# etzinis/sudo_rm_rf

Measured on AMD Instinct MI355X. Metric: separated-seconds/sec (4s@8kHz mixtures), Improved-U16/512, 1->8 MI355X, higher is better.
Workload: dtype f32 (1x1 convs: fp32 operands split into bf16 hi+lo, 3 bf16 MFMAs per product, fp32 accumulate)

## Files before the change

include/sudormrf_hip.h:

```cpp
#ifndef SUDORMRF_HIP_H
#define SUDORMRF_HIP_H

#include <stddef.h>

#ifdef __cplusplus
extern "C" {
#endif

#define SRF_ABI_VERSION 18

#define SRF_STAT_BUCKETS 64

#define SRF_OK 0
#define SRF_EINVAL (-1)
#define SRF_EHIP (-2)
#define SRF_EWORKSPACE (-3)

#define SRF_VARIANT_IMPROVED 0
#define SRF_VARIANT_GROUPCOMM 1
#define SRF_VARIANT_CAUSAL 2

typedef struct srf_config {
  int variant;
  int in_audio_channels;
  int out_channels;
  int in_channels;
  int num_blocks;
  int upsampling_depth;
  int enc_kernel_size;
  int enc_num_basis;
  int num_sources;
  int group_size;
} srf_config;

typedef struct srf_norm {
  const double* sums;
  const float* gamma;
  const float* beta;
  const float* prelu;
} srf_norm;

typedef struct srf_plan srf_plan;

int srf_abi_version(void);
const char* srf_last_error(void);

void srf_set_kernel_mode(int mode);
int srf_get_kernel_mode(void);
int srf_profile_begin(void* stream);
int srf_profile_end(void* stream, int* count);
int srf_profile_get(int i, const char** name, float* ms);
int srf_profile_timeline(int i, const char** name, float* t_ms, int* stream_index);

#ifdef SRF_DIAGNOSTICS
enum srf_debug_flag {
  SRF_DBG_NO_PAIRS = 1,
  SRF_DBG_GEMM_NO_MGROUPS = 2,
  SRF_DBG_NO_GEMM_256 = 4,
  SRF_DBG_NO_PACKED_WEIGHTS = 8,
  SRF_DBG_PYR_PER_LEVEL = 16,
  SRF_DBG_PYR_NO_LDS_TILES = 32,
  SRF_DBG_PYR_NO_REG = 64,
  SRF_DBG_PYR_PASS1_NONPERSISTENT = 128,
  SRF_DBG_GEMM_WHOLE_TAIL_TILES = 256,
  SRF_DBG_GEMM_QUARTER_TILES_LAST = 512,
  SRF_DBG_TAC_ONE_STEP_PER_LANE = 1024,
  SRF_DBG_GEMM_128_ONE_TILE_PER_BLOCK = 2048,
  SRF_DBG_WGRAD_NO_XCD_MAP = 4096,
  SRF_DBG_GEMM_256_SWAP_FORMS = 8192,
  SRF_DBG_TRAIN_BF16X3 = 16384,
  SRF_DBG_NO_FUSED_TAIL = 32768,
  SRF_DBG_BWD_NO_FUSED_HEAD = 1 << 16,
  SRF_DBG_PYR_PASS1_ROWS_PER_WAVE = 1 << 17,
  SRF_DBG_WGRAD_NO_WIDE_TILE = 1 << 18,
  SRF_DBG_WGRAD_128_MASKED = 1 << 19,
  SRF_DBG_WGRAD_SHORT_CHUNKS = 1 << 20,
  SRF_DBG_PAIR_PERSISTENT = 1 << 21,
  SRF_DBG_TAC_VALU = 1 << 22,
  SRF_DBG_PAIR_FULL_DRAIN = 1 << 23,
  SRF_DBG_TAC_GENERIC = 1 << 24,
  SRF_DBG_WGRAD_ONE_CHAIN_FOLD = 1 << 25,
  SRF_DBG_TAC_LANES_4TILES = 1 << 26,
  SRF_DBG_GEMM_128_POINTER_LOADS = 1 << 27,
  SRF_DBG_TRAIN_FWD_SPLIT_BF16 = 1 << 28,
  SRF_DBG_BWD_DW_CHUNKED = 1 << 29,
  SRF_DBG_BWD_GLN_SCALAR = 1 << 30,
  SRF_DBG_TRAIN_FWD_EXACT_MFMA = -2147483647 - 1
};
void srf_set_debug_flags(int flags);
#endif

int srf_plan_create(const srf_config* cfg, int batch, int T, srf_plan** out);
void srf_plan_destroy(srf_plan* plan);
size_t srf_plan_workspace_bytes(const srf_plan* plan);
int srf_plan_num_params(const srf_plan* plan);
int srf_plan_frames(const srf_plan* plan);
int srf_plan_padded_length(const srf_plan* plan);
int srf_plan_num_launches(const srf_plan* plan);

int srf_forward(const srf_plan* plan, const float* const* params, int num_params,
                const float* wav, float* out, void* workspace, size_t workspace_bytes, void* stream);

int srf_separate(const srf_plan* plan, const float* const* params, int num_params, const float* wav, float* out,
                 float* stats, int mixture_consistency, void* workspace, size_t workspace_bytes, void* stream);

int srf_plan_set_block_scales(srf_plan* plan, const float* alpha, const float* beta, int n);

int srf_debug_fetch(const srf_plan* plan, const void* workspace, int what, float* dst, size_t dst_floats,
                    void* stream);



int srf_encoder(const float* wav, const float* w, float* out, double* sums,
                int Bt, int A, int T, int N, int K, int L, void* stream);

int srf_gln_stats(const float* x, double* sums, int groups, long per_group, void* stream);
int srf_gln_apply(const float* x, float* y, const srf_norm* norm, int groups, int channels, int length,
                  void* stream);
int srf_gln_apply_add(const float* x, const float* q, float* y, const srf_norm* norm, int groups,
                      int channels, int length, void* stream);

int srf_pw_conv(const float* x, const float* w, const float* bias, float* y,
                int Bt, int Cin, int Cout, int L, const srf_norm* in_norm, const float* residual,
                double* out_sums, int epilogue_mask, const float* mul, int mul_channels, void* stream);

size_t srf_packed_pw_weight_bytes(int Cout, int Cin);
int srf_pack_pw_weights(const float* const* w, void* const* packed, const int* Cout, const int* Cin, int n,
                        void* stream);
int srf_pw_conv_packed(const float* x, const float* w, const void* w_packed, const float* bias, float* y,
                       int Bt, int Cin, int Cout, int L, const srf_norm* in_norm, const float* residual,
                       double* out_sums, int epilogue_mask, const float* mul, int mul_channels, void* stream);

int srf_pw_conv_pair_supported(int Bt, int Cin1, int Cmid, int Cout2, int L);
int srf_pw_conv_pair(const float* x, const void* w1_packed, const float* bias1, float* y, const srf_norm* in_norm,
                     const float* residual, const void* w2_packed, const float* bias2, float* y2, double* out_sums2,
                     int Bt, int Cin1, int Cmid, int Cout2, int L, void* stream);

size_t srf_packed3_pw_weight_bytes(int Cout, int Cin);
int srf_pack3_pw_weights(const float* const* w, void* const* packed, const int* Cout, const int* Cin, int n, void* stream);
void srf_pack3_forget(const void* packed);
int srf_pw_conv_packed3(const float* x, const float* w, const void* w_packed3, const float* bias, float* y, int Bt, int Cin,
                        int Cout, int L, const srf_norm* in_norm, const float* residual, double* out_sums, void* stream);
int srf_pw_conv_pair_packed3_supported(int Bt, int Cin1, int Cmid, int Cout2, int L);
int srf_pw_conv_pair_packed3(const float* x, const void* w1_packed3, const float* bias1, float* y, const srf_norm* in_norm,
                             const float* residual, const void* w2_packed3, const float* bias2, float* y2, double* out_sums2,
                             int Bt, int Cin1, int Cmid, int Cout2, int L, void* stream);

int srf_dwconv5(const float* x, const float* w, const float* bias, float* y,
                int Bt, int C, int Lin, int stride, const srf_norm* in_norm, double* out_sums,
                void* stream);

int srf_conv1d(const float* x, const float* w, const float* bias, float* y, int Bt, int Cin, int Cout, int Lin, int K,
               int stride, int padding, int dilation, int groups, double* out_sums, void* stream);

int srf_merge(const float* const* levels, const srf_norm* norms, int D, float* y,
              int Bt, int C, int L, double* out_sums, void* stream);

int srf_pyramid_supported(int C, int L, int D);
size_t srf_pyramid_scratch_bytes(int groups, int C, int L, int D);
int srf_pyramid(const float* y1, float* merged, const srf_norm* in_norm, const float* const* w,
                const float* const* bias, const float* const* gamma, const float* const* beta, int groups,
                int C, int L, int D, void* scratch, double* out_sums, void* stream);

int srf_causal_encoder(const float* wav, const float* w, float* out, int Bt, int A, int T, int N, int K, int L, void* stream);
int srf_causal_dwconv(const float* x, const float* w, const float* bias, const float* in_prelu, const float* out_prelu,
                      float* y, int Bt, int C, int Lin, int stride, void* stream);
int srf_causal_merge(const float* const* levels, int D, float* y, int Bt, int C, int L, void* stream);
int srf_causal_pyramid_supported(int C, int L, int D);
int srf_causal_pyramid(const float* y1, float* merged, const float* in_prelu, const float* const* w,
                       const float* const* bias, const float* const* prelu, int Bt, int C, int L, int D, void* stream);
int srf_causal_scale(const float* src, float* dst, long n, const float* dscale, float hscale, void* stream);
int srf_prelu_apply(const float* x, const float* slope, float* y, long n, void* stream);

typedef struct srf_stream srf_stream;
int srf_stream_create(const srf_config* cfg, int batch, int max_chunk_samples, srf_stream** out);
void srf_stream_destroy(srf_stream* s);
int srf_stream_granule(const srf_stream* s);
int srf_stream_delay(const srf_stream* s);
size_t srf_stream_state_bytes(const srf_stream* s);
size_t srf_stream_weights_bytes(const srf_stream* s);
size_t srf_stream_workspace_bytes(const srf_stream* s);
int srf_stream_num_launches(const srf_stream* s);
int srf_stream_set_block_scales(srf_stream* s, const float* alpha, const float* beta, int n);
int srf_stream_prepare(const srf_stream* s, const float* const* params, int num_params, void* weights_buf, void* stream);
int srf_stream_reset(const srf_stream* s, void* state, int row, void* stream);
int srf_stream_push(const srf_stream* s, const void* weights_buf, void* state, const float* wav, int n, float* out,
                    void* workspace, size_t workspace_bytes, void* stream);
int srf_stream_flush(const srf_stream* s, const void* state, float* out_tail, void* stream);
int srf_causal_stream_pyramid(const float* y1, float* merged, float* const* state, const float* in_prelu,
                              const float* const* w, const float* const* bias, const float* const* prelu, int Bt, int C, int Lc,
                              int D, void* stream);

size_t srf_decoder_scratch_floats(int Bt, int Ci, int Co, int K, int L);
int srf_decoder(const float* v, const float* w, float* out, int Bt, int Ci, int Co, int K, int L, int T,
                float* scratch, void* stream);

int srf_tac(const float* x, float* q, const float* const* params, int Bt, int G, int n, int H, int L,
            double* out_sums, void* stream);

int srf_mixture_consistency(const float* pr, const float* mix, float* out, int Bt, int S, int T,
                            void* stream);

int srf_mixture_consistency_magsq(const float* pr, const float* mix, float* out, int Bt, int S, int T, float* work,
                                  void* stream);

int srf_wav_normalize(const float* wav, float* out, float* stats, int rows, int T, void* stream);
int srf_wav_stats(const float* wav, float* stats, int rows, int T, void* stream);
int srf_wav_denormalize(const float* est, const float* stats, const float* mix_norm, float* out, int Bt, int S,
                        int T, void* stream);

size_t srf_pit_sisdr_work_bytes(int Bt, int S);
int srf_pit_sisdr_forward(const float* est, const float* tgt, int Bt, int S, int T, float clamp, void* work,
                          float* pw, float* loss, void* stream);
int srf_pit_sdr_forward(const float* est, const float* tgt, int Bt, int S, int T, float clamp, int sdr_type,
                        int zero_mean, int take_log, void* work, float* pw, float* loss, void* stream);
int srf_pit_sisdr_match(const void* work, int Bt, int S, int* match_out, void* stream);
int srf_pit_sisdr_backward(const float* est, const float* tgt, int Bt, int S, int T, float clamp, const void* work,
                           const float* loss, const float* upstream, float* grad_est, void* stream);

size_t srf_perm_inv_sisdr_work_bytes(int Bt, int S);
int srf_perm_inv_sisdr(const float* pr, const float* tgt, const float* mix, int Bt, int S, int T, int zero_mean,
                       double eps, void* work, float* best, int* best_perm, float* base, void* stream);

size_t srf_zeroref_snr_work_bytes(int Bt, int S, int T);
int srf_zeroref_snr_forward(const float* est, const float* tgt, int Bt, int S, int T, int zero_mean, float threshold_db,
                            float thresh, float eps, void* work, float* values, int* best_perm, float* loss, void* stream);
int srf_zeroref_snr_backward(const float* est, const float* tgt, int Bt, int S, int T, const void* work,
                             const float* upstream, int upstream_per_example, float* grad_est, void* stream);
size_t srf_stab_sisdr_work_bytes(int Bt, int T);
int srf_stab_sisdr(const float* pr, const float* tgt, int Bt, int pr_rows, int n_est, int n_act, int T, int zero_mean,
                   int improvement, double eps, void* work, float* values, int* best_perm, void* stream);
size_t srf_fuss_augment_scratch_bytes(int B, int T);
int srf_fuss_augment(const float* clean, const int* src_b, const int* src_s, const float* gain, int B, int S, int T, float eps,
                     float* out, float* mix, float* stats, void* scratch, void* stream);


size_t srf_pw_wgrad_scratch_bytes(int Bt, int Cout, int Cin, int L);
int srf_pw_wgrad(const float* g, const float* x, const srf_norm* in_norm, int Bt, int Cin, int Cout, int L, float* dw,
                 float* dbias, int accumulate, void* scratch, void* stream);
int srf_pw_wgrad_cols(const float* g, const float* x, const srf_norm* in_norm, int Bt, int Cin, int Cout, int L,
                      float* dw, int dw_cols, float* dbias, int accumulate, void* scratch, void* stream);
int srf_pw_wgrad_ld(const float* g, const float* x, const srf_norm* in_norm, int Bt, int Cin, int Cout, int L,
                    float* dw, int dw_cols, int dw_ld, float* dbias, int accumulate, void* scratch, void* stream);

size_t srf_tac_bwd_scratch_bytes(int Bt, int G, int n, int L);
int srf_tac_bwd(const float* x, const float* go, const float* const* params, float* const* grads, int Bt, int G, int n,
                int H, int L, float* gx, void* scratch, void* stream);

size_t srf_gln_bwd_scratch_bytes(int groups, int C);
int srf_gln_bwd(const float* gout, const float* gout2, const float* x, const srf_norm* norm, int groups, int C, int L,
                float* gx, int accumulate_gx, float* dgamma, float* dbeta, float* dslope, void* scratch, void* stream);

int srf_merge_bwd(const float* g_merged, float* const* g_levels, int D, long rows, int L, void* stream);

size_t srf_dwconv5_bwd_scratch_bytes(int groups, int C);
int srf_dwconv5_bwd(const float* gd, const float* xin, const srf_norm* in_norm, const float* w, int groups, int C,
                    int Lin, int stride, float* gin, float* dw, float* dbias, void* scratch, void* stream);

int srf_mask_apply(const float* m, const float* enc, float* v, int Bt, int SA, int N, int L, void* stream);
int srf_mask_bwd(const float* gv, const float* m, const float* enc, float* gm, float* genc, int accumulate_genc, int Bt,
                 int SA, int N, int L, void* stream);

int srf_prelu_bwd(const float* gout, const float* x, const float* slope, float* gx, float* dslope, long n, void* stream);

int srf_frames_gather(const float* src, float* out, int Bt, int R, int T, int K, int hop, int pad, int L, int rows_out,
                      void* stream);

size_t srf_train_saved_bytes(const srf_plan* plan);
size_t srf_train_scratch_bytes(const srf_plan* plan);
int srf_forward_train(const srf_plan* plan, const float* const* params, int num_params, const float* wav, float* out,
                      void* saved, size_t saved_bytes, void* scratch, size_t scratch_bytes, void* stream);
int srf_backward(const srf_plan* plan, const float* const* params, float* const* grads, int num_params,
                 const float* wav, const float* grad_out, const void* saved, size_t saved_bytes, void* scratch,
                 size_t scratch_bytes, void* stream);
int srf_backward_wav(const srf_plan* plan, const float* const* params, float* const* grads, int num_params,
                     const float* wav, const float* grad_out, const void* saved, size_t saved_bytes, void* scratch,
                     size_t scratch_bytes, float* grad_wav, void* stream);

size_t srf_online_remix_scratch_bytes(int B, int S);
int srf_online_remix(const float* clean, const int* src_b, const int* src_s, int B, int S, int T, float eps, float* mix,
                     float* out, void* scratch, void* stream);

int srf_opt_chunk_size(void);
int srf_clip_adam_step(const void* tensors, const void* chunks, int n_chunks, double* buckets, float max_norm, float lr,
                       float beta1, float beta2, float eps, int step, float* norm_out, void* stream);

typedef struct srf_feeder srf_feeder;
int srf_wav_info(const char* path, int* rate, int* channels, int* bits, long* frames);
int srf_wav_read(const char* path, long start, long n, float* dst, long* frames);
int srf_feeder_create(const char* const* paths, int n_items, int n_streams, int time_samples, int batch, int n_threads,
                      int augment, int shuffle, int drop_last, unsigned long long seed, srf_feeder** out);
int srf_feeder_create_sharded(const char* const* paths, int n_items, int n_streams, int time_samples, int batch,
                              int n_threads, int augment, int shuffle, int drop_last, unsigned long long seed, int normalize,
                              int rank, int world, srf_feeder** out);
void srf_feeder_destroy(srf_feeder* f);
long srf_feeder_epoch_items(srf_feeder* f, int* items, long capacity);
int srf_feeder_read_example(const char* const* paths, int n_streams, int time_samples, long start, int augment, int normalize,
                            float* wave, int* len, float* stat);
long srf_feeder_batches_per_epoch(const srf_feeder* f);
long srf_feeder_item_frames(const srf_feeder* f, int item);
int srf_feeder_start_epoch(srf_feeder* f, int epoch);
int srf_feeder_submit(srf_feeder* f, float* wave, int* len, float* stat);
int srf_feeder_wait(srf_feeder* f, float** wave, int** len, float** stat, int* n_valid);
int srf_feeder_normalize(const float* raw, const int* len, const float* stat, int B, int n_streams, int T, int normalize,
                         float eps, float* mix, float* src, void* stream);

#ifdef __cplusplus
}
#endif
#endif
```

sudo_rm_rf_amd/_lib.py:

```python
import ctypes as C
import os
import threading

import torch

_PKG = os.path.dirname(os.path.abspath(__file__))
LIB_PATH = os.environ.get("SRF_LIB") or os.path.join(_PKG, "libsudormrf_hip.so")
ABI_VERSION = 18
STAT_BUCKETS = 64

SRF_OK = 0
VARIANT_IMPROVED, VARIANT_GROUPCOMM, VARIANT_CAUSAL = 0, 1, 2


class SrfError(RuntimeError):
    pass


class srf_config(C.Structure):
    _fields_ = [(n, C.c_int) for n in (
        "variant", "in_audio_channels", "out_channels", "in_channels", "num_blocks",
        "upsampling_depth", "enc_kernel_size", "enc_num_basis", "num_sources", "group_size")]


class srf_norm(C.Structure):
    _fields_ = [("sums", C.c_void_p), ("gamma", C.c_void_p), ("beta", C.c_void_p), ("prelu", C.c_void_p)]


_vp, _i, _sz, _l = C.c_void_p, C.c_int, C.c_size_t, C.c_long
_PROTOS = {
    "srf_abi_version": (_i, []),
    "srf_last_error": (C.c_char_p, []),
    "srf_set_kernel_mode": (None, [_i]),
    "srf_get_kernel_mode": (_i, []),
    "srf_profile_begin": (_i, [_vp]),
    "srf_profile_end": (_i, [_vp, C.POINTER(_i)]),
    "srf_profile_get": (_i, [_i, C.POINTER(C.c_char_p), C.POINTER(C.c_float)]),
    "srf_profile_timeline": (_i, [_i, C.POINTER(C.c_char_p), C.POINTER(C.c_float), C.POINTER(_i)]),
    "srf_plan_create": (_i, [C.POINTER(srf_config), _i, _i, C.POINTER(_vp)]),
    "srf_plan_destroy": (None, [_vp]),
    "srf_plan_workspace_bytes": (_sz, [_vp]),
    "srf_plan_num_params": (_i, [_vp]),
    "srf_plan_frames": (_i, [_vp]),
    "srf_plan_padded_length": (_i, [_vp]),
    "srf_plan_num_launches": (_i, [_vp]),
    "srf_forward": (_i, [_vp, C.POINTER(_vp), _i, _vp, _vp, _vp, _sz, _vp]),
    "srf_debug_fetch": (_i, [_vp, _vp, _i, _vp, _sz, _vp]),
    "srf_encoder": (_i, [_vp, _vp, _vp, _vp, _i, _i, _i, _i, _i, _i, _vp]),
    "srf_gln_stats": (_i, [_vp, _vp, _i, _l, _vp]),
    "srf_gln_apply": (_i, [_vp, _vp, C.POINTER(srf_norm), _i, _i, _i, _vp]),
    "srf_gln_apply_add": (_i, [_vp, _vp, _vp, C.POINTER(srf_norm), _i, _i, _i, _vp]),
    "srf_pw_conv": (_i, [_vp, _vp, _vp, _vp, _i, _i, _i, _i, C.POINTER(srf_norm), _vp, _vp, _i, _vp, _i, _vp]),
    "srf_set_debug_flags": (None, [_i]),
    "srf_packed_pw_weight_bytes": (_sz, [_i, _i]),
    "srf_pack_pw_weights": (_i, [C.POINTER(_vp), C.POINTER(_vp), C.POINTER(_i), C.POINTER(_i), _i, _vp]),
    "srf_pw_conv_packed": (_i, [_vp, _vp, _vp, _vp, _vp, _i, _i, _i, _i, C.POINTER(srf_norm), _vp, _vp, _i, _vp, _i, _vp]),
    "srf_pw_conv_pair_supported": (_i, [_i, _i, _i, _i, _i]),
    "srf_pw_conv_pair": (_i, [_vp, _vp, _vp, _vp, C.POINTER(srf_norm), _vp, _vp, _vp, _vp, _vp, _i, _i, _i, _i, _i, _vp]),
    "srf_pw_conv_pair_packed3_supported": (_i, [_i, _i, _i, _i, _i]),
    "srf_pw_conv_pair_packed3": (_i, [_vp, _vp, _vp, _vp, C.POINTER(srf_norm), _vp, _vp, _vp, _vp, _vp, _i, _i, _i, _i, _i, _vp]),
    "srf_packed3_pw_weight_bytes": (_sz, [_i, _i]),
    "srf_pack3_pw_weights": (_i, [C.POINTER(_vp), C.POINTER(_vp), C.POINTER(_i), C.POINTER(_i), _i, _vp]),
    "srf_pack3_forget": (None, [_vp]),
    "srf_pw_conv_packed3": (_i, [_vp, _vp, _vp, _vp, _vp, _i, _i, _i, _i, C.POINTER(srf_norm), _vp, _vp, _vp]),
    "srf_pit_sisdr_work_bytes": (_sz, [_i, _i]),
    "srf_perm_inv_sisdr_work_bytes": (_sz, [_i, _i]),
    "srf_perm_inv_sisdr": (_i, [_vp, _vp, _vp, _i, _i, _i, _i, C.c_double, _vp, _vp, _vp, _vp, _vp]),
    "srf_pit_sisdr_forward": (_i, [_vp, _vp, _i, _i, _i, C.c_float, _vp, _vp, _vp, _vp]),
    "srf_pit_sdr_forward": (_i, [_vp, _vp, _i, _i, _i, C.c_float, _i, _i, _i, _vp, _vp, _vp, _vp]),
    "srf_pit_sisdr_match": (_i, [_vp, _i, _i, _vp, _vp]),
    "srf_pit_sisdr_backward": (_i, [_vp, _vp, _i, _i, _i, C.c_float, _vp, _vp, _vp, _vp, _vp]),
    "srf_zeroref_snr_work_bytes": (_sz, [_i, _i, _i]),
    "srf_zeroref_snr_forward": (_i, [_vp, _vp, _i, _i, _i, _i, C.c_float, C.c_float, C.c_float, _vp, _vp, _vp, _vp, _vp]),
    "srf_zeroref_snr_backward": (_i, [_vp, _vp, _i, _i, _i, _vp, _vp, _i, _vp, _vp]),
    "srf_stab_sisdr_work_bytes": (_sz, [_i, _i]),
    "srf_stab_sisdr": (_i, [_vp, _vp, _i, _i, _i, _i, _i, _i, _i, C.c_double, _vp, _vp, _vp, _vp]),
    "srf_fuss_augment_scratch_bytes": (_sz, [_i, _i]),
    "srf_fuss_augment": (_i, [_vp, _vp, _vp, _vp, _i, _i, _i, C.c_float, _vp, _vp, _vp, _vp, _vp]),
    "srf_pw_wgrad_scratch_bytes": (_sz, [_i, _i, _i, _i]),
    "srf_pw_wgrad_cols": (_i, [_vp, _vp, C.POINTER(srf_norm), _i, _i, _i, _i, _vp, _i, _vp, _i, _vp, _vp]),
    "srf_pw_wgrad_ld": (_i, [_vp, _vp, C.POINTER(srf_norm), _i, _i, _i, _i, _vp, _i, _i, _vp, _i, _vp, _vp]),
    "srf_pw_wgrad": (_i, [_vp, _vp, C.POINTER(srf_norm), _i, _i, _i, _i, _vp, _vp, _i, _vp, _vp]),
    "srf_gln_bwd_scratch_bytes": (_sz, [_i, _i]),
    "srf_gln_bwd": (_i, [_vp, _vp, _vp, C.POINTER(srf_norm), _i, _i, _i, _vp, _i, _vp, _vp, _vp, _vp, _vp]),
    "srf_merge_bwd": (_i, [_vp, C.POINTER(_vp), _i, C.c_long, _i, _vp]),
    "srf_dwconv5_bwd_scratch_bytes": (_sz, [_i, _i]),
    "srf_dwconv5_bwd": (_i, [_vp, _vp, C.POINTER(srf_norm), _vp, _i, _i, _i, _i, _vp, _vp, _vp, _vp, _vp]),
    "srf_mask_apply": (_i, [_vp, _vp, _vp, _i, _i, _i, _i, _vp]),
    "srf_mask_bwd": (_i, [_vp, _vp, _vp, _vp, _vp, _i, _i, _i, _i, _i, _vp]),
    "srf_prelu_bwd": (_i, [_vp, _vp, _vp, _vp, _vp, C.c_long, _vp]),
    "srf_frames_gather": (_i, [_vp, _vp, _i, _i, _i, _i, _i, _i, _i, _i, _vp]),
    "srf_train_saved_bytes": (_sz, [_vp]),
    "srf_train_scratch_bytes": (_sz, [_vp]),
    "srf_forward_train": (_i, [_vp, C.POINTER(_vp), _i, _vp, _vp, _vp, _sz, _vp, _sz, _vp]),
    "srf_backward": (_i, [_vp, C.POINTER(_vp), C.POINTER(_vp), _i, _vp, _vp, _vp, _sz, _vp, _sz, _vp]),
    "srf_backward_wav": (_i, [_vp, C.POINTER(_vp), C.POINTER(_vp), _i, _vp, _vp, _vp, _sz, _vp, _sz, _vp, _vp]),
    "srf_tac_bwd_scratch_bytes": (_sz, [_i, _i, _i, _i]),
    "srf_tac_bwd": (_i, [_vp, _vp, C.POINTER(_vp), C.POINTER(_vp), _i, _i, _i, _i, _i, _vp, _vp, _vp]),
    "srf_online_remix_scratch_bytes": (_sz, [_i, _i]),
    "srf_online_remix": (_i, [_vp, _vp, _vp, _i, _i, _i, C.c_float, _vp, _vp, _vp, _vp]),
    "srf_opt_chunk_size": (_i, []),
    "srf_clip_adam_step": (_i, [_vp, _vp, _i, _vp, C.c_float, C.c_float, C.c_float, C.c_float, C.c_float, _i, _vp, _vp]),
    "srf_wav_normalize": (_i, [_vp, _vp, _vp, _i, _i, _vp]),
    "srf_wav_stats": (_i, [_vp, _vp, _i, _i, _vp]),
    "srf_separate": (_i, [_vp, C.POINTER(_vp), _i, _vp, _vp, _vp, _i, _vp, _sz, _vp]),
    "srf_wav_denormalize": (_i, [_vp, _vp, _vp, _vp, _i, _i, _i, _vp]),
    "srf_dwconv5": (_i, [_vp, _vp, _vp, _vp, _i, _i, _i, _i, C.POINTER(srf_norm), _vp, _vp]),
    "srf_conv1d": (_i, [_vp, _vp, _vp, _vp, _i, _i, _i, _i, _i, _i, _i, _i, _i, _vp, _vp]),
    "srf_pyramid_supported": (_i, [_i, _i, _i]),
    "srf_pyramid_scratch_bytes": (_sz, [_i, _i, _i, _i]),
    "srf_pyramid": (_i, [_vp, _vp, C.POINTER(srf_norm), C.POINTER(_vp), C.POINTER(_vp), C.POINTER(_vp),
                        C.POINTER(_vp), _i, _i, _i, _i, _vp, _vp, _vp]),
    "srf_merge": (_i, [C.POINTER(_vp), C.POINTER(srf_norm), _i, _vp, _i, _i, _i, _vp, _vp]),
    "srf_decoder_scratch_floats": (_sz, [_i, _i, _i, _i, _i]),
    "srf_decoder": (_i, [_vp, _vp, _vp, _i, _i, _i, _i, _i, _i, _vp, _vp]),
    "srf_tac": (_i, [_vp, _vp, C.POINTER(_vp), _i, _i, _i, _i, _i, _vp, _vp]),
    "srf_mixture_consistency": (_i, [_vp, _vp, _vp, _i, _i, _i, _vp]),
    "srf_mixture_consistency_magsq": (_i, [_vp, _vp, _vp, _i, _i, _i, _vp, _vp]),
    "srf_wav_info": (_i, [C.c_char_p, C.POINTER(_i), C.POINTER(_i), C.POINTER(_i), C.POINTER(_l)]),
    "srf_wav_read": (_i, [C.c_char_p, _l, _l, _vp, C.POINTER(_l)]),
    "srf_feeder_create": (_i, [C.POINTER(C.c_char_p), _i, _i, _i, _i, _i, _i, _i, _i, C.c_ulonglong, C.POINTER(_vp)]),
    "srf_feeder_create_sharded": (_i, [C.POINTER(C.c_char_p), _i, _i, _i, _i, _i, _i, _i, _i, C.c_ulonglong, _i, _i, _i,
                                       C.POINTER(_vp)]),
    "srf_feeder_destroy": (None, [_vp]),
    "srf_feeder_epoch_items": (_l, [_vp, _vp, _l]),
    "srf_feeder_read_example": (_i, [C.POINTER(C.c_char_p), _i, _i, _l, _i, _i, _vp, _vp, _vp]),
    "srf_feeder_batches_per_epoch": (_l, [_vp]),
    "srf_feeder_item_frames": (_l, [_vp, _i]),
    "srf_feeder_start_epoch": (_i, [_vp, _i]),
    "srf_feeder_submit": (_i, [_vp, _vp, _vp, _vp]),
    "srf_feeder_wait": (_i, [_vp, C.POINTER(_vp), C.POINTER(_vp), C.POINTER(_vp), C.POINTER(_i)]),
    "srf_feeder_normalize": (_i, [_vp, _vp, _vp, _i, _i, _i, _i, C.c_float, _vp, _vp, _vp]),
    "srf_plan_set_block_scales": (_i, [_vp, C.POINTER(C.c_float), C.POINTER(C.c_float), _i]),
    "srf_causal_encoder": (_i, [_vp, _vp, _vp, _i, _i, _i, _i, _i, _i, _vp]),
    "srf_causal_dwconv": (_i, [_vp, _vp, _vp, _vp, _vp, _vp, _i, _i, _i, _i, _vp]),
    "srf_causal_merge": (_i, [C.POINTER(_vp), _i, _vp, _i, _i, _i, _vp]),
    "srf_causal_pyramid_supported": (_i, [_i, _i, _i]),
    "srf_causal_pyramid": (_i, [_vp, _vp, _vp, C.POINTER(_vp), C.POINTER(_vp), C.POINTER(_vp), _i, _i, _i, _i, _vp]),
    "srf_causal_scale": (_i, [_vp, _vp, _l, _vp, C.c_float, _vp]),
    "srf_prelu_apply": (_i, [_vp, _vp, _vp, _l, _vp]),
    "srf_stream_create": (_i, [C.POINTER(srf_config), _i, _i, C.POINTER(_vp)]),
    "srf_stream_destroy": (None, [_vp]),
    "srf_stream_granule": (_i, [_vp]),
    "srf_stream_delay": (_i, [_vp]),
    "srf_stream_state_bytes": (_sz, [_vp]),
    "srf_stream_weights_bytes": (_sz, [_vp]),
    "srf_stream_workspace_bytes": (_sz, [_vp]),
    "srf_stream_num_launches": (_i, [_vp]),
    "srf_stream_set_block_scales": (_i, [_vp, C.POINTER(C.c_float), C.POINTER(C.c_float), _i]),
    "srf_stream_prepare": (_i, [_vp, C.POINTER(_vp), _i, _vp, _vp]),
    "srf_stream_reset": (_i, [_vp, _vp, _i, _vp]),
    "srf_stream_push": (_i, [_vp, _vp, _vp, _vp, _i, _vp, _vp, _sz, _vp]),
    "srf_stream_flush": (_i, [_vp, _vp, _vp, _vp]),
    "srf_causal_stream_pyramid": (_i, [_vp, _vp, C.POINTER(_vp), _vp, C.POINTER(_vp), C.POINTER(_vp), C.POINTER(_vp), _i, _i, _i,
                                       _i, _vp]),
}
EXPORTED_SYMBOLS = tuple(_PROTOS)

_lib = None
_lock = threading.Lock()


def load():
    global _lib
    if _lib is not None:
        return _lib
    with _lock:
        if _lib is not None:
            return _lib
        if not os.path.exists(LIB_PATH):
            raise SrfError(
                "libsudormrf_hip.so not found at %s -- build it with `python -m sudo_rm_rf_amd.build` "
                "(or __graft_entry__.build()).  There is no CPU / PyTorch fallback." % LIB_PATH)
        lib = C.CDLL(LIB_PATH)
        for name, (res, args) in _PROTOS.items():
            try:
                fn = getattr(lib, name)
            except AttributeError as e:
                raise SrfError("libsudormrf_hip.so lacks symbol %s (stale build?)" % name) from e
            fn.restype = res
            fn.argtypes = args
        if lib.srf_abi_version() != ABI_VERSION:
            raise SrfError("libsudormrf_hip.so ABI version %d != expected %d" %
                           (lib.srf_abi_version(), ABI_VERSION))
        _lib = lib
    return _lib


def check(rc, what="libsudormrf_hip"):
    if rc != SRF_OK:
        msg = load().srf_last_error()
        raise SrfError("%s failed (%d): %s" % (what, rc, msg.decode() if msg else "?"))


def ptr(t):
    return None if t is None else C.c_void_p(t.data_ptr())


def current_stream(device):
    return C.c_void_p(torch.cuda.current_stream(device).cuda_stream)


def make_norm(sums=None, gamma=None, beta=None, prelu=None):
    n = srf_norm()
    n.sums = sums.data_ptr() if sums is not None else None
    n.gamma = gamma.data_ptr() if gamma is not None else None
    n.beta = beta.data_ptr() if beta is not None else None
    n.prelu = prelu.data_ptr() if prelu is not None else None
    return n
```

sudo_rm_rf_amd/build.py:

```python
import hashlib
import os
import re
import shutil
import subprocess
import sys
from concurrent.futures import ThreadPoolExecutor

PKG = os.path.dirname(os.path.abspath(__file__))
CSRC = os.path.join(PKG, "csrc")
OBJ = os.path.join(CSRC, "build")
LIB = os.path.join(PKG, "libsudormrf_hip.so")
SOURCES = ["srf_api.hip", "srf_encoder.hip", "srf_elementwise.hip", "srf_dwconv.hip", "srf_pyramid.hip", "srf_pyramid_reg.hip", "srf_pwconv.hip", "srf_pwconv_bf16x3.hip", "srf_pwconv_x3w.hip", "srf_pwconv_x3p.hip", "srf_pwconv_x3f.hip", "srf_pwconv_w4.hip", "srf_pwconv_small.hip",
           "srf_tac.hip", "srf_loss.hip", "srf_pwconv_wgrad.hip", "srf_backward.hip", "srf_train.hip", "srf_augment.hip", "srf_optim.hip", "srf_feeder.hip",
           "srf_causal.hip", "srf_causal_stream.hip", "srf_loss_fuss.hip"]
HEADERS = [os.path.join(CSRC, "srf_common.h"), os.path.join(CSRC, "srf_internal.h"), os.path.join(CSRC, "srf_pw.h"), os.path.join(CSRC, "srf_plan.h"), os.path.join(CSRC, "srf_pyr.h"),
           os.path.join(os.path.dirname(PKG), "include", "sudormrf_hip.h")]
FLAGS = ["-O3", "-std=c++17", "--offload-arch=gfx950", "-fPIC", "-munsafe-fp-atomics",
         "-Wall", "-Wno-unused-function"]
FILE_FLAGS = {
    "srf_pwconv_bf16x3.hip": ["-fno-slp-vectorize"],
    "srf_pwconv_x3w.hip": ["-fno-slp-vectorize"],
    "srf_pwconv_x3p.hip": ["-fno-slp-vectorize"],
    "srf_pwconv_x3f.hip": ["-fno-slp-vectorize"],
    "srf_pwconv_w4.hip": ["-fno-slp-vectorize"],
    "srf_pwconv_wgrad.hip": ["-fno-slp-vectorize"],
    "srf_pwconv.hip": ["-fno-slp-vectorize"],
    "srf_pyramid_reg.hip": ["-fno-slp-vectorize"],
}

_HAZARD = re.compile(r"^\s*(v_pk_\w+)\s.*op_sel:\[[01],1[,\]]", re.M)


def isa_lint(asm_path):
    hits = []
    with open(asm_path, errors="replace") as f:
        for i, line in enumerate(f, 1):
            if _HAZARD.match(line):
                hits.append((i, line.strip()))
    return hits


def hipcc():
    for c in (os.environ.get("HIPCC"), shutil.which("hipcc"), "/opt/rocm/bin/hipcc"):
        if c and os.path.exists(c):
            return c
    raise RuntimeError("hipcc not found (set HIPCC=...)")


def _digest(paths, extra=""):
    h = hashlib.sha1(extra.encode())
    for p in paths:
        with open(p, "rb") as f:
            h.update(f.read())
    return h.hexdigest()


def _compile(cc, src, extra_flags):
    path = os.path.join(CSRC, src)
    obj = os.path.join(OBJ, os.path.basename(src).replace(".hip", ".o"))
    stamp = obj + ".sha1"
    flags = FLAGS + FILE_FLAGS.get(src, []) + extra_flags
    dig = _digest([path, os.path.abspath(__file__)] + HEADERS, " ".join(flags))
    if os.path.exists(obj) and os.path.exists(stamp) and open(stamp).read() == dig:
        return obj, False
    cmd = [cc] + flags + ["-save-temps=obj", "-c", path, "-o", obj]
    r = subprocess.run(cmd, capture_output=True, text=True)
    if r.returncode != 0:
        raise RuntimeError("hipcc failed: %s\n%s\n%s" % (" ".join(cmd), r.stdout, r.stderr))
    warn = "\n".join(l for l in r.stderr.splitlines() if "argument unused during compilation" not in l)
    if warn.strip():
        sys.stderr.write(warn + "\n")
    base = os.path.basename(src).replace(".hip", "")
    asm = os.path.join(OBJ, base + "-hip-amdgcn-amd-amdhsa-gfx950.s")
    if not os.path.exists(asm):
        raise RuntimeError("ISA lint: device assembly %s was not produced" % asm)
    hits = isa_lint(asm)
    for f in os.listdir(OBJ):
        if f.startswith(base + "-h") or f.startswith(base + ".hip-"):
            os.remove(os.path.join(OBJ, f))
    if hits:
        os.remove(obj)
        raise RuntimeError(
            "ISA lint: %s contains %d packed-fp32 instruction(s) with op_sel = 1 on src1 (wrong low result in lanes 48..63 "
            "next to another wavefront's bf16 MFMA on gfx950, see build.py); first: line %d: %s"
            % (src, len(hits), hits[0][0], hits[0][1]))
    with open(stamp, "w") as f:
        f.write(dig)
    return obj, True


def build(force=False, verbose=True, extra_flags=()):
    cc = hipcc()
    os.makedirs(OBJ, exist_ok=True)
    extra_flags = list(extra_flags)
    if force:
        for f in os.listdir(OBJ):
            os.remove(os.path.join(OBJ, f))
    sources = SOURCES
    with ThreadPoolExecutor(max_workers=min(len(sources), os.cpu_count() or 4)) as ex:
        res = list(ex.map(lambda s: _compile(cc, s, extra_flags), sources))
    objs = [o for o, _ in res]
    changed = any(c for _, c in res)
    if changed or not os.path.exists(LIB):
        cmd = [cc, "-shared", "-fPIC", "--offload-arch=gfx950", "-o", LIB] + objs
        r = subprocess.run(cmd, capture_output=True, text=True)
        if r.returncode != 0:
            raise RuntimeError("link failed: %s\n%s\n%s" % (" ".join(cmd), r.stdout, r.stderr))
        if verbose:
            print("built", LIB)
    elif verbose:
        print("up to date:", LIB)
    return LIB


if __name__ == "__main__":
    build(force="--force" in sys.argv)
```

sudo_rm_rf_amd/csrc/srf_api.hip:

```cpp
#include <string.h>

#include <atomic>
#include <mutex>
#include <new>
#include <vector>

#include "srf_plan.h"

static thread_local char g_err[512] = "";
static std::atomic<int> g_kernel_mode{0};

void srf_set_error(const char* fmt, ...) {
  va_list ap;
  va_start(ap, fmt);
  vsnprintf(g_err, sizeof(g_err), fmt, ap);
  va_end(ap);
}
static thread_local int g_kernel_mode_override = -1;
int srf_kernel_mode() { return g_kernel_mode_override >= 0 ? g_kernel_mode_override : g_kernel_mode.load(std::memory_order_relaxed); }
int srf_kernel_mode_override(int mode) {
  const int prev = g_kernel_mode_override;
  g_kernel_mode_override = mode;
  return prev;
}
static std::atomic<int> g_debug_flags{0};
int srf_debug_flags() { return g_debug_flags.load(std::memory_order_relaxed); }
extern "C" void srf_set_debug_flags(int f) { g_debug_flags.store(f, std::memory_order_relaxed); }

static std::mutex g_dev_mu;
static int g_dev_cus[SRF_MAX_DEVICES];
static long g_dev_occ[SRF_MAX_DEVICES][SRF_OCC_SLOTS];
static bool g_dev_occ_set[SRF_MAX_DEVICES][SRF_OCC_SLOTS];

int srf_current_device() {
  int dev = 0;
  return hipGetDevice(&dev) == hipSuccess ? dev : -1;
}
int srf_device_cus() {
  const int dev = srf_current_device();
  if (dev < 0 || dev >= SRF_MAX_DEVICES) return 256;
  std::lock_guard<std::mutex> lk(g_dev_mu);
  if (!g_dev_cus[dev]) {
    hipDeviceProp_t prop;
    g_dev_cus[dev] = hipGetDeviceProperties(&prop, dev) == hipSuccess ? prop.multiProcessorCount : 256;
  }
  return g_dev_cus[dev];
}
long srf_device_cached(int slot, long (*compute)(void*), void* arg) {
  const int dev = srf_current_device();
  if (dev < 0 || dev >= SRF_MAX_DEVICES || slot < 0 || slot >= SRF_OCC_SLOTS) return compute(arg);
  {
    std::lock_guard<std::mutex> lk(g_dev_mu);
    if (g_dev_occ_set[dev][slot]) return g_dev_occ[dev][slot];
  }
  const long v = compute(arg);
  std::lock_guard<std::mutex> lk(g_dev_mu);
  g_dev_occ[dev][slot] = v;
  g_dev_occ_set[dev][slot] = true;
  return v;
}

struct ProfMark {
  const char* name;
  hipEvent_t ev;
  hipStream_t st;
};
static bool g_prof = false;
static std::vector<ProfMark> g_marks;
static std::vector<hipEvent_t> g_pool;
static std::vector<float> g_ms;

static thread_local int g_prof_hold = 0;
bool srf_profiling() { return g_prof && g_prof_hold == 0; }
void srf_prof_hold(int delta) { g_prof_hold += delta; }
void srf_prof_mark(const char* name, hipStream_t st) {
  hipEvent_t ev;
  if (!g_pool.empty()) {
    ev = g_pool.back();
    g_pool.pop_back();
  } else if (hipEventCreate(&ev) != hipSuccess) {
    return;
  }
  (void)hipEventRecord(ev, st);
  g_marks.push_back(ProfMark{name, ev, st});
}

extern "C" int srf_profile_begin(void* stream) {
  for (auto& m : g_marks) g_pool.push_back(m.ev);
  g_marks.clear();
  g_ms.clear();
  g_prof = true;
  srf_prof_mark("begin", (hipStream_t)stream);
  return SRF_OK;
}

extern "C" int srf_profile_end(void* stream, int* count) {
  g_prof = false;
  SRF_CHECK_HIP(hipStreamSynchronize((hipStream_t)stream));
  g_ms.assign(g_marks.size(), 0.f);
  for (size_t i = 1; i < g_marks.size(); ++i) {
    float ms = 0.f;
    SRF_CHECK_HIP(hipEventElapsedTime(&ms, g_marks[i - 1].ev, g_marks[i].ev));
    g_ms[i] = ms;
  }
  if (count) *count = g_marks.empty() ? 0 : (int)g_marks.size() - 1;
  return SRF_OK;
}

extern "C" int srf_profile_timeline(int i, const char** name, float* t_ms, int* stream_index) {
  SRF_CHECK_ARG(i >= 0 && (size_t)(i + 1) < g_marks.size() && name && t_ms && stream_index, "srf_profile_timeline: bad index %d", i);
  float ms = 0.f;
  SRF_CHECK_HIP(hipEventElapsedTime(&ms, g_marks[0].ev, g_marks[i + 1].ev));
  int idx = 0;
  std::vector<hipStream_t> seen;
  for (size_t j = 1; j <= (size_t)(i + 1); ++j) {
    bool known = false;
    for (size_t k = 0; k < seen.size(); ++k)
      if (seen[k] == g_marks[j].st) {
        known = true;
        if (j == (size_t)(i + 1)) idx = (int)k;
      }
    if (!known) {
      if (j == (size_t)(i + 1)) idx = (int)seen.size();
      seen.push_back(g_marks[j].st);
    }
  }
  *name = g_marks[i + 1].name;
  *t_ms = ms;
  *stream_index = idx;
  return SRF_OK;
}

extern "C" int srf_profile_get(int i, const char** name, float* ms) {
  SRF_CHECK_ARG(i >= 0 && (size_t)(i + 1) < g_marks.size() && name && ms, "srf_profile_get: bad index %d", i);
  *name = g_marks[i + 1].name;
  *ms = g_ms[i + 1];
  return SRF_OK;
}

extern "C" const char* srf_last_error(void) { return g_err; }
extern "C" int srf_abi_version(void) { return SRF_ABI_VERSION; }
extern "C" void srf_set_kernel_mode(int mode) { g_kernel_mode.store((mode == 1 || mode == 2) ? mode : 0, std::memory_order_relaxed); }
extern "C" int srf_get_kernel_mode(void) { return g_kernel_mode.load(std::memory_order_relaxed); }

__global__ __launch_bounds__(256) void srf_zero_kernel(uint4* __restrict__ p, size_t n16) {
  for (size_t i = (size_t)blockIdx.x * 256 + threadIdx.x; i < n16; i += (size_t)gridDim.x * 256) p[i] = make_uint4(0, 0, 0, 0);
}
static int srf_zero_launch(void* p, size_t bytes, hipStream_t st) {
  SRF_CHECK_ARG(srf_aligned16(p) && bytes % 16 == 0, "internal: zero fill needs 16-byte granules");
  const size_t n16 = bytes / 16;
  if (!n16) return SRF_OK;
  const size_t blocks = (n16 + 255) / 256;
  hipLaunchKernelGGL(srf_zero_kernel, dim3((unsigned)(blocks < 2048 ? blocks : 2048)), dim3(256), 0, st, (uint4*)p, n16);
  SRF_CHECK_LAUNCH("zero_fill", st);
  return SRF_OK;
}

extern "C" size_t srf_decoder_scratch_floats(int Bt, int Ci, int Co, int K, int L) {
  const size_t M = (size_t)Co * K;
  return srf_align_up(M * Ci, 64) + srf_align_up(M, 64) + srf_align_up((size_t)Bt * M * L, 64);
}

static int srf_decoder_impl(const float* v, const float* w, float* out, int Bt, int Ci, int Co, int K, int L, int T,
                            float* scratch, const float* post_stats, const float* post_wav, int post_mc, void* stream,
                            const float* in_prelu = nullptr);
extern "C" int srf_decoder(const float* v, const float* w, float* out, int Bt, int Ci, int Co, int K,
                           int L, int T, float* scratch, void* stream) {
  return srf_decoder_impl(v, w, out, Bt, Ci, Co, K, L, T, scratch, nullptr, nullptr, 0, stream);
}
static int srf_decoder_impl(const float* v, const float* w, float* out, int Bt, int Ci, int Co, int K, int L, int T,
                            float* scratch, const float* post_stats, const float* post_wav, int post_mc, void* stream,
                            const float* in_prelu) {
  SRF_CHECK_ARG(v && w && out && scratch, "srf_decoder: null pointer");
  SRF_CHECK_ARG(Bt > 0 && Ci > 0 && Co > 0 && L > 0 && T > 0, "srf_decoder: bad sizes");
  SRF_CHECK_ARG(K >= 3 && (K & 1), "srf_decoder: kernel size must be odd (got %d)", K);
  SRF_CHECK_ARG(T <= (K / 2) * L, "srf_decoder: T=%d exceeds hop*L=%d", T, (K / 2) * L);
  SRF_CHECK_ARG(Co <= 65535 && Bt <= 65535, "srf_decoder: too many channels / batch");
  SRF_CHECK_ALIGNED16("srf_decoder", {"scratch", scratch});
  hipStream_t st = (hipStream_t)stream;
  const int M = Co * K;
  float* wt = scratch;
  float* zb = wt + srf_align_up((size_t)M * Ci, 64);
  float* z = zb + srf_align_up((size_t)M, 64);
  int rc = srf_transpose_launch(w, wt, Ci, M, st);
  if (rc) return rc;
  rc = srf_zero_launch(zb, sizeof(float) * srf_align_up((size_t)M, 64), st);
  if (rc) return rc;
  const srf_norm act{nullptr, nullptr, nullptr, in_prelu};
  rc = srf_pw_conv(v, wt, zb, z, Bt, Ci, M, L, in_prelu ? &act : nullptr, nullptr, nullptr, 0, nullptr, 0, stream);
  if (rc) return rc;
  return srf_overlap_add_launch(z, out, Bt, Co, K, L, T, 1, post_stats, post_wav, post_mc, st);
}

static long plan_padded_length(int T, int h, int D) {
  const long nls = (long)h << D;
  return (T < nls) ? nls : ((T / nls) + (T % nls ? 1 : 0)) * nls;
}
static void plan_add_pack(srf_plan* p, size_t* off, int param, int cout, int cin) {
  const size_t bytes = srf_packed_pw_weight_bytes(cout, cin);
  if (!bytes) return;
  const size_t o = *off;
  *off = srf_align_up(*off + bytes, 256);
  p->pk_param.push_back(param);
  p->pk_cout.push_back(cout);
  p->pk_cin.push_back(cin);
  p->pk_off.push_back(o);
  p->pk_of_param[param] = o;
}

static int plan_fail(srf_plan* p, int rc) {
  delete p;
  return rc;
}

static int causal_plan_create(const srf_config* c, int batch, int T, srf_plan** out);
extern "C" int srf_plan_create(const srf_config* c, int batch, int T, srf_plan** out) {
  SRF_CHECK_ARG(c && out, "srf_plan_create: null pointer");
  *out = nullptr;
  SRF_CHECK_ARG(c->variant == SRF_VARIANT_IMPROVED || c->variant == SRF_VARIANT_GROUPCOMM || c->variant == SRF_VARIANT_CAUSAL,
                "srf_plan_create: unknown variant %d", c->variant);
  if (c->variant == SRF_VARIANT_CAUSAL) return causal_plan_create(c, batch, T, out);
  SRF_CHECK_ARG(batch > 0 && T > 0, "srf_plan_create: batch and T must be positive");
  SRF_CHECK_ARG(c->out_channels > 0 && c->in_channels > 0 && c->num_blocks > 0 && c->enc_num_basis > 0 &&
                    c->num_sources > 0,
                "srf_plan_create: non-positive model dimension");
  SRF_CHECK_ARG(c->upsampling_depth >= 1 && c->upsampling_depth <= SRF_MAX_DEPTH,
                "srf_plan_create: upsampling_depth %d unsupported (1..%d)", c->upsampling_depth,
                SRF_MAX_DEPTH);
  SRF_CHECK_ARG(c->enc_kernel_size >= 3 && (c->enc_kernel_size & 1),
                "srf_plan_create: enc_kernel_size must be odd (the reference's mask multiply breaks "
                "for even sizes)");
  srf_plan* p = new (std::nothrow) srf_plan();
  SRF_CHECK_ARG(p != nullptr, "srf_plan_create: out of host memory");
  p->cfg = *c;
  const bool gc = c->variant == SRF_VARIANT_GROUPCOMM;
  const int G = gc ? c->group_size : 1;
  p->A = gc ? c->in_audio_channels : 1;
  if (G <= 0 || p->A <= 0) {
    srf_set_error("srf_plan_create: group_size / in_audio_channels must be positive");
    return plan_fail(p, SRF_EINVAL);
  }
  if (gc && (c->out_channels % G || c->in_channels % G)) {
    srf_set_error("srf_plan_create: channels (%d,%d) not divisible by group_size %d", c->out_channels,
                  c->in_channels, G);
    return plan_fail(p, SRF_EINVAL);
  }
  if (gc) {
    const int n = c->out_channels / G;
    if (!(n == 2 || n == 4 || n == 8 || n == 16 || n == 32)) {
      srf_set_error("srf_plan_create: out_channels/group_size = %d unsupported (2,4,8,16,32)", n);
      return plan_fail(p, SRF_EINVAL);
    }
  }
  const int D = c->upsampling_depth, U = c->num_blocks, K = c->enc_kernel_size;
  const int h = K / 2;
  const long Tp = plan_padded_length(T, h, D);
  p->Bt = batch;
  p->T = T;
  p->Tp = (int)Tp;
  p->L = (int)((Tp + 2 * h - K) / h + 1);
  p->SA = c->num_sources * p->A;
  p->Bg = batch * G;
  p->nB = c->out_channels / G;
  p->nC = c->in_channels / G;
  if (p->L % (1 << (D - 1)) != 0) {
    srf_set_error("srf_plan_create: internal: L=%d not divisible by 2^(D-1)", p->L);
    return plan_fail(p, SRF_EINVAL);
  }
  if ((long)p->Bg > 65535) {
    srf_set_error("srf_plan_create: batch*group_size=%d too large (max 65535 per call)", p->Bg);
    return plan_fail(p, SRF_EINVAL);
  }
  const int ublock_params = 10 + 4 * D;
  p->p_block0 = 5;
  p->p_ublock_off = gc ? 11 : 0;
  p->p_block_stride = ublock_params + p->p_ublock_off;
  p->p_tail = 5 + U * p->p_block_stride;
  p->n_params = p->p_tail + 4;
  p->slots_per_block = D + 2 + (gc ? 1 : 0);
  p->n_slots = 1 + U * p->slots_per_block;
  const size_t F = sizeof(float);
  const size_t L = p->L;
  size_t off = 0;
  auto take = [&](size_t bytes) {
    const size_t o = off;
    off = srf_align_up(off + bytes, 256);
    return o;
  };
  p->stats_bytes = (size_t)p->n_slots * p->Bg * SRF_STAT_BUCKETS * 2 * sizeof(double);
  p->off_stats = take(p->stats_bytes);
  p->off_enc = take(F * batch * c->enc_num_basis * L);
  p->off_xa = take(F * batch * c->out_channels * L);
  p->off_xb = take(F * batch * c->out_channels * L);
  p->off_xq = gc ? take(F * batch * c->out_channels * L) : 0;
  p->off_xu = gc ? take(F * batch * c->out_channels * L) : 0;
  p->off_y1 = take(F * batch * c->in_channels * L);
  for (int k = 0; k < D; ++k) p->off_lv[k] = take(F * batch * c->in_channels * (L >> k));
  p->off_masked = take(F * batch * p->SA * c->enc_num_basis * L);
  p->off_dec = take(F * srf_decoder_scratch_floats(batch, p->SA * c->enc_num_basis, p->SA, K, p->L));
  p->fused_pyramid = srf_pyramid_supported(p->nC, p->L, D);
  p->off_pyr = p->fused_pyramid ? take(srf_pyramid_scratch_bytes(p->Bg, p->nC, p->L, D)) : 0;
  p->pk_of_param.assign(p->n_params, 0);
  plan_add_pack(p, &off, 3, c->out_channels, c->enc_num_basis);
  for (int i = 0; i < U; ++i) {
    const int pu = p->p_block0 + i * p->p_block_stride + p->p_ublock_off;
    plan_add_pack(p, &off, pu + 0, p->nC, p->nB);
    plan_add_pack(p, &off, pu + 5 + 4 * D + 3, p->nB, p->nC);
  }
  plan_add_pack(p, &off, p->p_tail + 1, p->SA * c->enc_num_basis, c->out_channels);
  p->off_wdpack = (p->SA * K <= 64 && p->pk_of_param[p->p_tail + 1]) ? take(srf_mask_decode_pack_bytes(p->SA * c->enc_num_basis)) : 0;
  p->total_bytes = off;
  p->n_launches = 1  + 2 + U * (D + 3 + (gc ? 2 : 0)) + 1 + 4;
  *out = p;
  return SRF_OK;
}

static int causal_plan_create(const srf_config* c, int batch, int T, srf_plan** out) {
  SRF_CHECK_ARG(batch > 0 && T > 0, "srf_plan_create: batch and T must be positive");
  SRF_CHECK_ARG(c->in_audio_channels > 0 && c->out_channels > 0 && c->in_channels > 0 && c->num_blocks > 0 &&
                    c->enc_num_basis > 0 && c->num_sources > 0,
                "srf_plan_create: non-positive model dimension (causal variant)");
  SRF_CHECK_ARG(c->group_size == 1, "srf_plan_create: the causal variant has no groups (group_size must be 1, got %d)",
                c->group_size);
  SRF_CHECK_ARG(c->upsampling_depth >= 1 && c->upsampling_depth <= SRF_MAX_DEPTH,
                "srf_plan_create: upsampling_depth %d unsupported (1..%d)", c->upsampling_depth, SRF_MAX_DEPTH);
  SRF_CHECK_ARG(c->enc_kernel_size >= 3 && (c->enc_kernel_size & 1),
                "srf_plan_create: enc_kernel_size must be odd for the causal variant (got %d)", c->enc_kernel_size);
  srf_plan* p = new (std::nothrow) srf_plan();
  SRF_CHECK_ARG(p != nullptr, "srf_plan_create: out of host memory");
  p->cfg = *c;
// ... 447 lines not shown
```

sudo_rm_rf_amd/csrc/srf_common.h:

```cpp
#pragma once
#include <hip/hip_runtime.h>
#include <stdarg.h>
#include <stdio.h>
#include <initializer_list>
#define SRF_DIAGNOSTICS 1
#include "../../include/sudormrf_hip.h"

#define SRF_WAVE 64
#define SRF_MAX_DEPTH 8

void srf_set_error(const char* fmt, ...);
int srf_kernel_mode();
int srf_kernel_mode_override(int mode);
int srf_debug_flags();
static inline bool srf_dbg(int mask) { return (srf_debug_flags() & mask) != 0; }
bool srf_profiling();
void srf_prof_hold(int delta);
void srf_prof_mark(const char* name, hipStream_t st);
#define SRF_MAX_DEVICES 64
int srf_current_device();
int srf_device_cus();
#define SRF_OCC_SLOTS 16
long srf_device_cached(int slot, long (*compute)(void*), void* arg);

#define SRF_CHECK_ARG(cond, ...)          \
  do {                                    \
    if (!(cond)) {                        \
      srf_set_error(__VA_ARGS__);         \
      return SRF_EINVAL;                  \
    }                                     \
  } while (0)

#define SRF_CHECK_LAUNCH(name, st)                                                    \
  do {                                                                                \
    hipError_t e__ = hipGetLastError();                                               \
    if (e__ != hipSuccess) {                                                          \
      srf_set_error("%s: kernel launch failed: %s", name, hipGetErrorString(e__));    \
      return SRF_EHIP;                                                                \
    }                                                                                 \
    if (srf_profiling()) srf_prof_mark(name, (hipStream_t)(st));                      \
  } while (0)

#define SRF_CHECK_HIP(expr)                                                            \
  do {                                                                                \
    hipError_t e__ = (expr);                                                          \
    if (e__ != hipSuccess) {                                                          \
      srf_set_error("%s failed: %s", #expr, hipGetErrorString(e__));                  \
      return SRF_EHIP;                                                                \
    }                                                                                 \
  } while (0)

static inline bool srf_aligned16(const void* p) { return (((size_t)p) & 15) == 0; }
static inline size_t srf_align_up(size_t v, size_t a) { return (v + a - 1) / a * a; }

struct SrfNamedPtr {
  const char* name;
  const void* p;
};
static inline const char* srf_first_unaligned16(std::initializer_list<SrfNamedPtr> ops) {
  for (const SrfNamedPtr& o : ops)
    if (o.p && !srf_aligned16(o.p)) return o.name;
  return nullptr;
}
#define SRF_CHECK_ALIGNED16(fn, ...)                                                                        \
  do {                                                                                                      \
    if (const char* u__ = srf_first_unaligned16({__VA_ARGS__})) {                                           \
      srf_set_error("%s: operand '%s' is not 16-byte aligned (this entry point has no unaligned form)", fn, u__); \
      return SRF_EINVAL;                                                                                    \
    }                                                                                                       \
  } while (0)

struct SrfNormDev {
  const double* sums;
  const float* gamma;
  const float* beta;
  const float* prelu;
};

static inline SrfNormDev srf_norm_dev(const srf_norm* n) {
  SrfNormDev d{nullptr, nullptr, nullptr, nullptr};
  if (n) {
    d.sums = n->sums;
    d.gamma = n->gamma;
    d.beta = n->beta;
    d.prelu = n->prelu;
  }
  return d;
}

__device__ __forceinline__ double srf_wave_sum(double v);
__device__ __forceinline__ void srf_finalize_stats(const double* sums, long g, double inv_count,
                                                   float& mean, float& rstd) {
  const double2 bk =
      reinterpret_cast<const double2*>(sums)[g * SRF_STAT_BUCKETS + (threadIdx.x & (SRF_STAT_BUCKETS - 1))];
  const double s = srf_wave_sum(bk.x), q = srf_wave_sum(bk.y);
  const double m = s * inv_count;
  double v = q * inv_count - m * m;
  v = v < 0.0 ? 0.0 : v;
  mean = (float)m;
  rstd = (float)(1.0 / sqrt(v + 1e-8));
}

__device__ __forceinline__ double srf_wave_sum(double v) {
#pragma unroll
  for (int o = 32; o > 0; o >>= 1) v += __shfl_xor(v, o, 64);
  return v;
}

__device__ __forceinline__ double* srf_stat_slot(double* sums, long g, long bucket) {
  return sums + 2 * (g * SRF_STAT_BUCKETS + (bucket & (SRF_STAT_BUCKETS - 1)));
}

template <int NWAVES>
__device__ __forceinline__ void srf_block_stats_atomic(double s, double q, double* dst, double* sh) {
  s = srf_wave_sum(s);
  q = srf_wave_sum(q);
  const int lane = threadIdx.x & 63, w = threadIdx.x >> 6;
  if (lane == 0) {
    sh[w] = s;
    sh[NWAVES + w] = q;
  }
  __syncthreads();
  if (threadIdx.x == 0) {
    double a = 0.0, b = 0.0;
#pragma unroll
    for (int i = 0; i < NWAVES; ++i) {
      a += sh[i];
      b += sh[NWAVES + i];
    }
    atomicAdd(dst, a);
    atomicAdd(dst + 1, b);
  }
}

__device__ __forceinline__ float srf_lane_up(float v) {
  return __int_as_float(__builtin_amdgcn_update_dpp(0, __float_as_int(v), 0x138, 0xf, 0xf, true));
}
__device__ __forceinline__ float srf_lane_down(float v) {
  return __int_as_float(__builtin_amdgcn_update_dpp(0, __float_as_int(v), 0x130, 0xf, 0xf, true));
}

__device__ __forceinline__ float srf_dpp_wave_sum(float v) {
  auto dpp = [](float x, int ctrl_id) {
    const int xi = __float_as_int(x);
    int r;
    switch (ctrl_id) {
      case 0: r = __builtin_amdgcn_update_dpp(0, xi, 0x111, 0xf, 0xf, true); break;
      case 1: r = __builtin_amdgcn_update_dpp(0, xi, 0x112, 0xf, 0xf, true); break;
      case 2: r = __builtin_amdgcn_update_dpp(0, xi, 0x114, 0xf, 0xf, true); break;
      case 3: r = __builtin_amdgcn_update_dpp(0, xi, 0x118, 0xf, 0xf, true); break;
      case 4: r = __builtin_amdgcn_update_dpp(0, xi, 0x142, 0xa, 0xf, true); break;
      default: r = __builtin_amdgcn_update_dpp(0, xi, 0x143, 0xc, 0xf, true); break;
    }
    return __int_as_float(r);
  };
  v += dpp(v, 0);
  v += dpp(v, 1);
  v += dpp(v, 2);
  v += dpp(v, 3);
  v += dpp(v, 4);
  v += dpp(v, 5);
  return v;
}

__device__ __forceinline__ double srf_dpp_wave_sum(double v) {
  auto step = [](double x, auto ctrl_tag) {
    constexpr int CTRL = decltype(ctrl_tag)::ctrl, RMASK = decltype(ctrl_tag)::rmask;
    const long long xi = __double_as_longlong(x);
    const int lo = __builtin_amdgcn_update_dpp(0, (int)(xi & 0xffffffffLL), CTRL, RMASK, 0xf, true);
    const int hi = __builtin_amdgcn_update_dpp(0, (int)(xi >> 32), CTRL, RMASK, 0xf, true);
    return __longlong_as_double(((long long)hi << 32) | (unsigned int)lo);
  };
  struct T1 { enum { ctrl = 0x111, rmask = 0xf }; };
  struct T2 { enum { ctrl = 0x112, rmask = 0xf }; };
  struct T4 { enum { ctrl = 0x114, rmask = 0xf }; };
  struct T8 { enum { ctrl = 0x118, rmask = 0xf }; };
  struct B15 { enum { ctrl = 0x142, rmask = 0xa }; };
  struct B31 { enum { ctrl = 0x143, rmask = 0xc }; };
  v += step(v, T1{});
  v += step(v, T2{});
  v += step(v, T4{});
  v += step(v, T8{});
  v += step(v, B15{});
  v += step(v, B31{});
  return v;
}

__device__ __forceinline__ void srf_finalize_stats_dpp(const double* sums, long g, double inv_count, float& mean,
                                                       float& rstd) {
  const double2 bk = reinterpret_cast<const double2*>(sums)[g * SRF_STAT_BUCKETS + (threadIdx.x & (SRF_STAT_BUCKETS - 1))];
  auto bcast63 = [](double x) {
    const long long xi = __double_as_longlong(x);
    const int lo = __builtin_amdgcn_readlane((int)(xi & 0xffffffffLL), 63);
    const int hi = __builtin_amdgcn_readlane((int)(xi >> 32), 63);
    return __longlong_as_double(((long long)hi << 32) | (unsigned int)lo);
  };
  const double s = bcast63(srf_dpp_wave_sum(bk.x)), q = bcast63(srf_dpp_wave_sum(bk.y));
  const double m = s * inv_count;
  double v = q * inv_count - m * m;
  v = v < 0.0 ? 0.0 : v;
  mean = (float)m;
  rstd = (float)(1.0 / sqrt(v + 1e-8));
}

template <bool NT>
__device__ __forceinline__ float4 srf_ld4(const float* p) {
  if constexpr (NT) {
    typedef float srf_f4v __attribute__((ext_vector_type(4)));
    const srf_f4v t = __builtin_nontemporal_load(reinterpret_cast<const srf_f4v*>(p));
    return make_float4(t[0], t[1], t[2], t[3]);
  } else {
    return *reinterpret_cast<const float4*>(p);
  }
}
template <bool NT>
__device__ __forceinline__ float2 srf_ld2(const float* p) {
  if constexpr (NT) {
    typedef float srf_f2v __attribute__((ext_vector_type(2)));
    const srf_f2v t = __builtin_nontemporal_load(reinterpret_cast<const srf_f2v*>(p));
    return make_float2(t[0], t[1]);
  } else {
    return *reinterpret_cast<const float2*>(p);
  }
}

__device__ __forceinline__ float srf_prelu(float x, float a) {
  return __builtin_amdgcn_fmed3f(x, a * x, a <= 1.f ? __builtin_inff() : -__builtin_inff());
}
```

sudo_rm_rf_amd/csrc/srf_pyr.h:

```cpp
#pragma once
#include "srf_internal.h"

struct PyrRegArgs {
  const float* y1;
  float* d0;
  float* merged;
  SrfNormDev in_norm;
  const float* in_mr;
  double in_inv_count;
  const float* w[SRF_MAX_DEPTH];
  const float* bias[SRF_MAX_DEPTH];
  const float* gamma[SRF_MAX_DEPTH];
  const float* beta[SRF_MAX_DEPTH];
  const float* lvl;
  double* mom;
  double* out_sums;
  int rows;
  int rpw;
  int C, L, D, tiles, own;
  float* lv_out[SRF_MAX_DEPTH];
  int save = 0;
};

int srf_pyramid_reg_launch(PyrRegArgs a, bool moments, long rows, hipStream_t st);
```

sudo_rm_rf_amd/csrc/srf_pyramid.hip:

```cpp
#include "srf_pyr.h"

struct PyrArgs {
  const float* y1;
  float* merged;
  SrfNormDev in_norm;
  double in_inv_count;
  const float* w[SRF_MAX_DEPTH];
  const float* bias[SRF_MAX_DEPTH];
  const float* gamma[SRF_MAX_DEPTH];
  const float* beta[SRF_MAX_DEPTH];
  const float* lvl;
  const float* in_mr;
  float* d0;
  double* mom;
  double* out_sums;
  long rows;
  int C, L, D;
};

__device__ __forceinline__ float srf_dot5(const float* w, float x0, float x1, float x2, float x3, float x4,
                                          float init) {
  return fmaf(w[4], x4, fmaf(w[3], x3, fmaf(w[2], x2, fmaf(w[1], x1, fmaf(w[0], x0, init)))));
}

// ... 231 lines not shown
    }
    if (a.out_sums) srf_block_stats_atomic<4>(ms, mq, srf_stat_slot(a.out_sums, g, row), red);
  }
  __syncthreads();
  }
}

struct PyrTile {
  int TS, tiles;
  int h[SRF_MAX_DEPTH];
  int wave_floats;
  long tasks;
};

template <bool MOMENTS>
__global__ __launch_bounds__(256) void srf_pyramid_tile_kernel(PyrArgs a, PyrTile t) {
  extern __shared__ __attribute__((aligned(16))) float lds[];
  const int L = a.L, D = a.D, C = a.C;
  const int lane = threadIdx.x & 63;
  const int wave = __builtin_amdgcn_readfirstlane(threadIdx.x >> 6);
  const long task = (long)blockIdx.x * 4 + wave;
  if (task >= t.tasks) return;
  const long row = task / t.tiles;
  const int tile = (int)(task - row * t.tiles);
  const int c = (int)(row % C);
  const long g = row / C;
  const int j0 = tile * t.TS;

  float* bufB = lds + wave * t.wave_floats;
  const int len0 = t.TS + 2 * t.h[0] + 8;
  float* bufA = bufB + len0;
  int offA[SRF_MAX_DEPTH];
  {
    int o = 0;
    offA[0] = 0;
#pragma unroll
    for (int k = 1; k < SRF_MAX_DEPTH; ++k) {
      offA[k] = o;
      if (k < D) o += (t.TS >> k) + 2 * t.h[k] + 8;
    }
  }

  float* coef = bufB + t.wave_floats - 8 * SRF_MAX_DEPTH;
  {
    const int k = lane >> 3, j = lane & 7;
    float v = 0.f;
    if (k < D) {
      if (j < 5) {
        v = a.w[k][c * 5 + j];
      } else if (j == 5) {
        v = (MOMENTS && k > 0) ? 0.f : a.bias[k][c];
      } else if (MOMENTS) {
        v = (j == 6) ? 1.f : 0.f;
      } else {
        const float m = a.lvl[(g * D + k) * 2 + 0], r = a.lvl[(g * D + k) * 2 + 1];
        const float aa = a.gamma[k][c] * r;
        v = (j == 6) ? aa : (a.beta[k][c] - m * aa);
      }
    }
    coef[lane] = v;
  }
  __builtin_amdgcn_fence(__ATOMIC_RELEASE, "wavefront");
  __builtin_amdgcn_wave_barrier();
  __builtin_amdgcn_fence(__ATOMIC_ACQUIRE, "wavefront");
  float sc = 1.f, sh = 0.f;
  if (a.in_norm.sums) {
    const float mean = a.in_mr[2 * g], rstd = a.in_mr[2 * g + 1];
    sc = a.in_norm.gamma[c] * rstd;
    sh = a.in_norm.beta[c] - mean * sc;
  }
  const bool act = a.in_norm.prelu != nullptr;
  const float slope = act ? a.in_norm.prelu[0] : 1.f;
  struct Lv {
    float w[5], b, a, c;
  };
  auto level_coef = [&](int k) {
    const float4 c0 = *reinterpret_cast<const float4*>(coef + 8 * k);
    const float4 c1 = *reinterpret_cast<const float4*>(coef + 8 * k + 4);
    Lv lv;
    lv.w[0] = c0.x;
    lv.w[1] = c0.y;
    lv.w[2] = c0.z;
    lv.w[3] = c0.w;
    lv.w[4] = c1.x;
    lv.b = c1.y;
    lv.a = c1.z;
    lv.c = c1.w;
    return lv;
  };
  auto wave_sync = [&]() {
    __builtin_amdgcn_fence(__ATOMIC_RELEASE, "wavefront");
    __builtin_amdgcn_wave_barrier();
    __builtin_amdgcn_fence(__ATOMIC_ACQUIRE, "wavefront");
  };

  const int lo0 = j0 - t.h[0];
  const int n4 = L >> 2;
  float s1[SRF_MAX_DEPTH], s2[SRF_MAX_DEPTH];
#pragma unroll
  for (int k = 0; k < SRF_MAX_DEPTH; ++k) s1[k] = s2[k] = 0.f;

  if (MOMENTS) {
    const float4* yrow = reinterpret_cast<const float4*>(a.y1 + (size_t)row * L);
    for (int q = lane; q < (len0 >> 2); q += 64) {
      const int p4 = ((lo0 - 4) >> 2) + q;
      const bool ok = p4 >= 0 && p4 < n4;
      float4 v = yrow[min(max(p4, 0), n4 - 1)];
      v.x = fmaf(v.x, sc, sh);
      v.y = fmaf(v.y, sc, sh);
      v.z = fmaf(v.z, sc, sh);
      v.w = fmaf(v.w, sc, sh);
      if (act) {
        v.x = srf_prelu(v.x, slope);
        v.y = srf_prelu(v.y, slope);
        v.z = srf_prelu(v.z, slope);
        v.w = srf_prelu(v.w, slope);
      }
      if (!ok) v = make_float4(0.f, 0.f, 0.f, 0.f);
      *reinterpret_cast<float4*>(bufA + 4 * q) = v;
    }
    wave_sync();
    const Lv l0 = level_coef(0);
    float4* drow = reinterpret_cast<float4*>(a.d0 + (size_t)row * L);
    const int nq = (t.TS + 2 * t.h[0]) >> 2;
    for (int q = lane; q < nq; q += 64) {
      const float* p = bufA + 4 + 4 * q;
      const float2 lo = *reinterpret_cast<const float2*>(p - 2);
      const float4 mi = *reinterpret_cast<const float4*>(p);
      const float2 hi = *reinterpret_cast<const float2*>(p + 4);
      float4 d;
      d.x = srf_dot5(l0.w, lo.x, lo.y, mi.x, mi.y, mi.z, l0.b);
      d.y = srf_dot5(l0.w, lo.y, mi.x, mi.y, mi.z, mi.w, l0.b);
      d.z = srf_dot5(l0.w, mi.x, mi.y, mi.z, mi.w, hi.x, l0.b);
      d.w = srf_dot5(l0.w, mi.y, mi.z, mi.w, hi.x, hi.y, l0.b);
      const int pos = lo0 + 4 * q;
      if (pos >= j0 && pos < j0 + t.TS) {
        drow[pos >> 2] = d;
        s1[0] += (d.x + d.y) + (d.z + d.w);
        s2[0] += fmaf(d.x, d.x, fmaf(d.y, d.y, fmaf(d.z, d.z, d.w * d.w)));
        if (pos == 0) {
          a.mom[(row * D + 0) * 5 + 2] = (double)d.x;
          a.mom[(row * D + 0) * 5 + 3] = (double)d.y;
        }
        if (pos == L - 4) a.mom[(row * D + 0) * 5 + 4] = (double)d.w;
      }
      if (pos < 0 || pos >= L) d = make_float4(0.f, 0.f, 0.f, 0.f);
      *reinterpret_cast<float4*>(bufB + 4 + 4 * q) = d;
    }
  } else {
    const Lv l0 = level_coef(0);
    const float4* drow = reinterpret_cast<const float4*>(a.d0 + (size_t)row * L);
    const int nq = (t.TS + 2 * t.h[0]) >> 2;
    for (int q = lane; q < nq; q += 64) {
      const int p4 = (lo0 >> 2) + q;
      const bool ok = p4 >= 0 && p4 < n4;
      float4 d = drow[min(max(p4, 0), n4 - 1)];
      d.x = fmaf(d.x, l0.a, l0.c);
      d.y = fmaf(d.y, l0.a, l0.c);
      d.z = fmaf(d.z, l0.a, l0.c);
      d.w = fmaf(d.w, l0.a, l0.c);
      if (!ok) d = make_float4(0.f, 0.f, 0.f, 0.f);
      *reinterpret_cast<float4*>(bufB + 4 + 4 * q) = d;
    }
  }
  wave_sync();

#pragma unroll
  for (int k = 1; k < SRF_MAX_DEPTH; ++k) {
    if (k < D) {
      const int Lk = L >> k;
      const Lv lk = level_coef(k);
      const float* src = (k == 1) ? bufB : (bufA + offA[k - 1]);
      float* dst = bufA + offA[k];
      const int own_lo = j0 >> k, own_len = t.TS >> k;
      const int lo = own_lo - t.h[k];
      const int nq = (own_len + 2 * t.h[k]) >> 2;
      for (int q = lane; q < nq; q += 64) {
        const float* p = src + 8 + 8 * q;
        const float2 l2 = *reinterpret_cast<const float2*>(p - 2);
        const float4 A = *reinterpret_cast<const float4*>(p);
        const float4 B = *reinterpret_cast<const float4*>(p + 4);
        const float r = p[8];
        float4 d;
        d.x = srf_dot5(lk.w, l2.x, l2.y, A.x, A.y, A.z, lk.b);
        d.y = srf_dot5(lk.w, A.x, A.y, A.z, A.w, B.x, lk.b);
        d.z = srf_dot5(lk.w, A.z, A.w, B.x, B.y, B.z, lk.b);
        d.w = srf_dot5(lk.w, B.x, B.y, B.z, B.w, r, lk.b);
        const int pos = lo + 4 * q;
        if (MOMENTS) {
          if (pos >= own_lo && pos < own_lo + own_len) {
            s1[k] += (d.x + d.y) + (d.z + d.w);
            s2[k] += fmaf(d.x, d.x, fmaf(d.y, d.y, fmaf(d.z, d.z, d.w * d.w)));
            if (pos == 0) {
              a.mom[(row * D + k) * 5 + 2] = (double)d.x;
              a.mom[(row * D + k) * 5 + 3] = (double)d.y;
            }
            if (pos == Lk - 4) a.mom[(row * D + k) * 5 + 4] = (double)d.w;
          }
        } else {
          d.x = fmaf(d.x, lk.a, lk.c);
          d.y = fmaf(d.y, lk.a, lk.c);
          d.z = fmaf(d.z, lk.a, lk.c);
          d.w = fmaf(d.w, lk.a, lk.c);
        }
        if (pos < 0 || pos >= Lk) d = make_float4(0.f, 0.f, 0.f, 0.f);
        *reinterpret_cast<float4*>(dst + 4 + 4 * q) = d;
      }
      wave_sync();
    }
  }

  if (MOMENTS) {
#pragma unroll
    for (int k = 0; k < SRF_MAX_DEPTH; ++k) {
      if (k < D) {
        float r1 = s1[k], r2 = s2[k];
#pragma unroll
        for (int o = 32; o > 0; o >>= 1) {
          r1 += __shfl_xor(r1, o, 64);
          r2 += __shfl_xor(r2, o, 64);
        }
        if (lane == 0) {
          atomicAdd(&a.mom[(row * D + k) * 5 + 0], (double)r1);
          atomicAdd(&a.mom[(row * D + k) * 5 + 1], (double)r2);
        }
      }
    }
  } else {
    float4* mrow = reinterpret_cast<float4*>(a.merged + (size_t)row * L + j0);
    float ms = 0.f, mq = 0.f;
    for (int q = lane; q < (t.TS >> 2); q += 64) {
      float tt = 0.f;
      bool have = false;
#pragma unroll
      for (int k = SRF_MAX_DEPTH - 1; k >= 2; --k) {
        if (k < D) {
          const float nk = bufA[offA[k] + 4 + t.h[k] + ((4 * q) >> k)];
          tt = have ? nk + tt : nk;
          have = true;
        }
      }
      float4 o = *reinterpret_cast<const float4*>(bufB + 4 + t.h[0] + 4 * q);
      if (D > 1) {
        const float2 e = *reinterpret_cast<const float2*>(bufA + offA[1] + 4 + t.h[1] + 2 * q);
        const float ta = have ? e.x + tt : e.x, tb = have ? e.y + tt : e.y;
        o.x += ta;
        o.y += ta;
        o.z += tb;
        o.w += tb;
      }
      mrow[q] = o;
      ms += (o.x + o.y) + (o.z + o.w);
      mq += fmaf(o.x, o.x, fmaf(o.y, o.y, fmaf(o.z, o.z, o.w * o.w)));
    }
    if (a.out_sums) {
      const double ds = srf_wave_sum((double)ms), dq = srf_wave_sum((double)mq);
      if (lane == 0) {
        double* dst = srf_stat_slot(a.out_sums, g, task);
        atomicAdd(dst, ds);
        atomicAdd(dst + 1, dq);
      }
    }
  }
}

__global__ __launch_bounds__(64) void srf_stats_finalize_kernel(const double* sums, double inv_count,
                                                                float* out) {
  float mean, rstd;
  srf_finalize_stats(sums, blockIdx.x, inv_count, mean, rstd);
  if (threadIdx.x == 0) {
    out[2 * blockIdx.x] = mean;
    out[2 * blockIdx.x + 1] = rstd;
  }
}

struct PyrFinArgs {
  const double* mom;
  const float* w[SRF_MAX_DEPTH];
  const float* bias[SRF_MAX_DEPTH];
  const float* gamma[SRF_MAX_DEPTH];
  const float* beta[SRF_MAX_DEPTH];
  float* lvl;
  const double* in_sums;
  double in_inv_count;
  float* in_mr;
  int C, L, D;
  double* lv_sums[SRF_MAX_DEPTH];
};

#define SRF_FIN_CPT 8
template <int CPT>
__global__ __launch_bounds__(256) void srf_pyramid_finalize_kernel(PyrFinArgs a) {
  __shared__ double red[16];
  const long g = blockIdx.x;
  const int tid = threadIdx.x, C = a.C, D = a.D;
  if (a.in_sums && tid < 64) {
    float m, r;
    srf_finalize_stats(a.in_sums, g, a.in_inv_count, m, r);
    if (tid == 0) {
      a.in_mr[2 * g] = m;
      a.in_mr[2 * g + 1] = r;
    }
  }
  double alpha[CPT], kap[CPT], g0[CPT], g1[CPT], gl[CPT];
#pragma unroll
  for (int i = 0; i < CPT; ++i) {
    alpha[i] = 1.0;
    kap[i] = g0[i] = g1[i] = gl[i] = 0.0;
  }
  constexpr bool PRE = CPT <= 2;
  double mo[PRE ? SRF_MAX_DEPTH : 1][CPT][5];
  auto load_level = [&](int slot, int k) {
#pragma unroll
    for (int i = 0; i < CPT; ++i) {
      const int c = min(tid + 256 * i, C - 1);
      const double* m = a.mom + ((g * C + c) * D + k) * 5;
#pragma unroll
      for (int e = 0; e < 5; ++e) mo[slot][i][e] = m[e];
    }
  };
  if (PRE) {
#pragma unroll
    for (int k = 0; k < SRF_MAX_DEPTH; ++k) load_level(PRE ? k : 0, k < D ? k : 0);
  }
#pragma unroll
  for (int k = 0; k < SRF_MAX_DEPTH; ++k) {
    if (k >= D) break;
    const int Lk = a.L >> k;
    const int slot = PRE ? k : 0;
    if (!PRE) load_level(0, k);
    float gam_[CPT], bet_[CPT], w_[CPT][5], bias_[CPT];
    if (k + 1 < D) {
#pragma unroll
      for (int i = 0; i < CPT; ++i) {
        const int c = min(tid + 256 * i, C - 1);
        gam_[i] = a.gamma[k][c];
        bet_[i] = a.beta[k][c];
        bias_[i] = a.bias[k + 1][c];
#pragma unroll
        for (int t = 0; t < 5; ++t) w_[i][t] = a.w[k + 1][c * 5 + t];
      }
    }
    double s = 0.0, q = 0.0;
#pragma unroll
    for (int i = 0; i < CPT; ++i) {
      const int c = tid + 256 * i;
      if (c < C) {
        const double S1 = mo[slot][i][0], S2 = mo[slot][i][1], e0 = mo[slot][i][2], e1 = mo[slot][i][3], el = mo[slot][i][4];
        s += alpha[i] * S1 + (Lk - 3) * kap[i] + g0[i] + g1[i] + gl[i];
        q += alpha[i] * alpha[i] * S2 +
             2.0 * alpha[i] * (kap[i] * (S1 - e0 - e1 - el) + g0[i] * e0 + g1[i] * e1 + gl[i] * el) +
             (Lk - 3) * kap[i] * kap[i] + g0[i] * g0[i] + g1[i] * g1[i] + gl[i] * gl[i];
      }
    }
    s = srf_dpp_wave_sum(s);
    q = srf_dpp_wave_sum(q);
    if ((tid & 63) == 63) {
      red[(tid >> 6) * 2] = s;
      red[(tid >> 6) * 2 + 1] = q;
    }
    __syncthreads();
    float mean_f, rstd_f;
    {
      double ts = 0.0, tq = 0.0;
      for (int w = 0; w < 4; ++w) {
        ts += red[2 * w];
        tq += red[2 * w + 1];
      }
      const double n = (double)C * (double)Lk;
      const double mean = ts / n;
      double var = tq / n - mean * mean;
      var = var < 0.0 ? 0.0 : var;
      mean_f = (float)mean;
      rstd_f = (float)(1.0 / sqrt(var + 1e-8));
      if (tid == 0) {
        a.lvl[(g * D + k) * 2 + 0] = mean_f;
        a.lvl[(g * D + k) * 2 + 1] = rstd_f;
        if (a.lv_sums[k]) {
          double* dst = a.lv_sums[k] + (size_t)g * SRF_STAT_BUCKETS * 2;
          dst[0] = ts;
          dst[1] = tq;
        }
      }
    }
    if (k + 1 < D) {
#pragma unroll
      for (int i = 0; i < CPT; ++i) {
        const int c = tid + 256 * i;
        if (c < C) {
          const float af = gam_[i] * rstd_f;
          const float bf = bet_[i] - mean_f * af;
          const double A = (double)af, B = (double)bf;
          const double w0 = w_[i][0], w1 = w_[i][1], w2 = w_[i][2], w3 = w_[i][3], w4 = w_[i][4];
          const double bs = (double)bias_[i];
          const double sw = w0 + w1 + w2 + w3 + w4;
          const double nk = bs + A * kap[i] * sw + B * sw;
          const double n0 = bs + A * (w2 * g0[i] + w3 * g1[i] + w4 * kap[i]) + B * (w2 + w3 + w4);
          const double n1 = bs + A * (w0 * g0[i] + w1 * g1[i] + (w2 + w3 + w4) * kap[i]) + B * sw;
          const double nl = bs + A * ((w0 + w1 + w2) * kap[i] + w3 * gl[i]) + B * (w0 + w1 + w2 + w3);
          kap[i] = nk;
          g0[i] = n0;
          g1[i] = n1;
          gl[i] = nl;
          alpha[i] *= A;
        }
      }
    }
    __syncthreads();
  }
}

static size_t pyr_lds_bytes(int L, int D) {
  size_t sizeA = (size_t)L + 8, lv = 0;
  for (int k = 1; k < D; ++k) lv += (size_t)(L >> k) + 8;
  if (lv > sizeA) sizeA = lv;
  sizeA = (sizeA + 3) & ~(size_t)3;
  return sizeof(float) * ((size_t)L + 8 + sizeA) + sizeof(double) * (4 * SRF_MAX_DEPTH * 2 + 8);
}

static void srf_pyramid_finalize_launch(const PyrFinArgs& f, int groups, int C, hipStream_t st) {
  if (C <= 512)
    hipLaunchKernelGGL(srf_pyramid_finalize_kernel<2>, dim3((unsigned)groups), dim3(256), 0, st, f);
  else
    hipLaunchKernelGGL((srf_pyramid_finalize_kernel<SRF_FIN_CPT>), dim3((unsigned)groups), dim3(256), 0, st, f);
}

extern "C" int srf_pyramid_supported(int C, int L, int D) {
  if (D < 1 || D > SRF_MAX_DEPTH || C > 256 * SRF_FIN_CPT) return 0;
  if ((L >> (D - 1)) < 8 || (L % (1 << (D - 1))) != 0) return 0;
  if (!srf_dbg(SRF_DBG_PYR_NO_REG) && srf_pyramid_reg_supported(L, D)) return 1;
  if (L % (4 << (D - 1)) != 0) return 0;
  return pyr_lds_bytes(L, D) <= 160 * 1024 - 1024;
}

static size_t pyr_small_bytes(int groups, int C, int D) {
  const size_t b = sizeof(double) * (size_t)groups * C * D * 5 + sizeof(float) * (size_t)groups * (D * 2 + 2);
  return (b + 255) & ~(size_t)255;
}
extern "C" size_t srf_pyramid_scratch_bytes(int groups, int C, int L, int D) {
  return pyr_small_bytes(groups, C, D) + sizeof(float) * (size_t)groups * C * L;
}

static bool pyr_pick_tile(int L, int D, PyrTile* t) {
  const int unit = 4 << (D - 1);
  const int m = L / unit;
  int best = 0;
  for (int q = 1; q <= m; ++q) {
    if (m % q) continue;
    const int ts = q * unit;
    if (ts >= 384 && ts <= 1024) {
      if (!best || abs(ts - 640) < abs(best - 640)) best = ts;
    }
  }
  if (!best || best == L) return false;
  t->TS = best;
  t->tiles = L / best;
  int h = 0;
  for (int k = SRF_MAX_DEPTH - 1; k >= 0; --k) {
    if (k >= D) {
      t->h[k] = 0;
      continue;
    }
    t->h[k] = (k == D - 1) ? 0 : 2 * h + 4;
    h = t->h[k];
  }
  const int len0 = best + 2 * t->h[0] + 8;
  int lv = 0;
  for (int k = 1; k < D; ++k) lv += (best >> k) + 2 * t->h[k] + 8;
  const int lenA = lv > len0 ? lv : len0;
  t->wave_floats = len0 + ((lenA + 3) & ~3) + 8 * SRF_MAX_DEPTH;
  return (size_t)t->wave_floats * 4 * sizeof(float) <= 64 * 1024;
}


int srf_pyramid_impl(const float* y1, float* merged, const srf_norm* in_norm, const float* const* w,
                     const float* const* bias, const float* const* gamma, const float* const* beta, int groups, int C,
                     int L, int D, void* scratch, double* out_sums, float* const* lv_out, double* const* lv_sums,
                     void* stream);

extern "C" int srf_pyramid(const float* y1, float* merged, const srf_norm* in_norm,
                           const float* const* w, const float* const* bias, const float* const* gamma,
                           const float* const* beta, int groups, int C, int L, int D, void* scratch,
                           double* out_sums, void* stream) {
  return srf_pyramid_impl(y1, merged, in_norm, w, bias, gamma, beta, groups, C, L, D, scratch, out_sums, nullptr, nullptr,
                          stream);
}

int srf_pyramid_impl(const float* y1, float* merged, const srf_norm* in_norm, const float* const* w,
                     const float* const* bias, const float* const* gamma, const float* const* beta, int groups, int C,
                     int L, int D, void* scratch, double* out_sums, float* const* lv_out, double* const* lv_sums,
                     void* stream) {
  SRF_CHECK_ARG((lv_out == nullptr) == (lv_sums == nullptr), "srf_pyramid: level outputs and level sums come together");
  SRF_CHECK_ARG(y1 && merged && w && bias && gamma && beta && scratch, "srf_pyramid: null pointer");
  SRF_CHECK_ARG(groups > 0 && C > 0 && L > 0, "srf_pyramid: bad sizes");
  SRF_CHECK_ARG(srf_pyramid_supported(C, L, D), "srf_pyramid: unsupported shape C=%d L=%d D=%d", C, L, D);
  SRF_CHECK_ALIGNED16("srf_pyramid", {"in_norm.sums", in_norm ? in_norm->sums : nullptr}, {"y1", y1}, {"merged", merged}, {"scratch", scratch});
  hipStream_t st = (hipStream_t)stream;
  const long rows = (long)groups * C;
  SRF_CHECK_ARG(rows < (1L << 31), "srf_pyramid: too many rows");
  double* mom = reinterpret_cast<double*>(scratch);
  float* lvl = reinterpret_cast<float*>(mom + (size_t)rows * D * 5);
  PyrArgs a;
  PyrFinArgs f;
  a.y1 = y1;
  a.merged = merged;
  a.in_norm = srf_norm_dev(in_norm);
  a.in_inv_count = 1.0 / ((double)C * (double)L);
  for (int k = 0; k < SRF_MAX_DEPTH; ++k) {
    const int kk = k < D ? k : 0;
    SRF_CHECK_ARG(w[kk] && bias[kk] && gamma[kk] && beta[kk], "srf_pyramid: null level parameter %d", kk);
    a.w[k] = f.w[k] = w[kk];
    a.bias[k] = f.bias[k] = bias[kk];
    a.gamma[k] = f.gamma[k] = gamma[kk];
    a.beta[k] = f.beta[k] = beta[kk];
  }
  a.lvl = lvl;
  a.in_mr = lvl + (size_t)groups * D * 2;
  a.d0 = reinterpret_cast<float*>(reinterpret_cast<char*>(scratch) + pyr_small_bytes(groups, C, D));
  a.mom = mom;
  a.out_sums = out_sums;
  a.rows = rows;
  a.C = C;
  a.L = L;
  a.D = D;
  f.mom = mom;
  f.lvl = lvl;
  f.in_sums = nullptr;
  f.in_inv_count = a.in_inv_count;
  f.in_mr = const_cast<float*>(a.in_mr);
  f.C = C;
  f.L = L;
  f.D = D;
  for (int k = 0; k < SRF_MAX_DEPTH; ++k) f.lv_sums[k] = (lv_sums && k < D) ? lv_sums[k] : nullptr;
  SRF_CHECK_ARG(!lv_out || (!srf_dbg(SRF_DBG_PYR_NO_REG | SRF_DBG_PYR_PASS1_NONPERSISTENT) && srf_pyramid_reg_supported(L, D)),
                "srf_pyramid: level outputs need the register-resident kernels");
  if (!srf_dbg(SRF_DBG_PYR_NO_REG) && srf_pyramid_reg_supported(L, D)) {
    PyrRegArgs r;
    for (int k = 0; k < SRF_MAX_DEPTH; ++k) r.lv_out[k] = (lv_out && k < D) ? lv_out[k] : nullptr;
    r.save = lv_out != nullptr;
    r.y1 = y1;
    r.d0 = a.d0;
    r.merged = merged;
    r.in_norm = a.in_norm;
    r.in_mr = a.in_mr;
    r.in_inv_count = a.in_inv_count;
    for (int k = 0; k < SRF_MAX_DEPTH; ++k) {
      r.w[k] = a.w[k];
      r.bias[k] = a.bias[k];
      r.gamma[k] = a.gamma[k];
      r.beta[k] = a.beta[k];
    }
    r.lvl = lvl;
    r.mom = mom;
    r.out_sums = out_sums;
    r.C = C;
    r.L = L;
    r.D = D;
    r.rows = r.rpw = 0;
    r.tiles = r.own = 0;
    if (srf_dbg(SRF_DBG_PYR_PASS1_NONPERSISTENT)) {
      SRF_CHECK_HIP(hipMemsetAsync(mom, 0, sizeof(double) * (size_t)rows * D * 5, st));
      if (a.in_norm.sums) {
        hipLaunchKernelGGL(srf_stats_finalize_kernel, dim3((unsigned)groups), dim3(64), 0, st, a.in_norm.sums,
                           a.in_inv_count, const_cast<float*>(a.in_mr));
        SRF_CHECK_LAUNCH("stats_finalize", st);
      }
    }
    SRF_CHECK_ARG(merged != y1, "srf_pyramid: merged must not alias y1 (pass 2 re-reads y1 with halos)");
    int rc = srf_pyramid_reg_launch(r, true, rows, st);
    if (rc) return rc;
    if (!srf_dbg(SRF_DBG_PYR_PASS1_NONPERSISTENT)) f.in_sums = a.in_norm.sums;
    srf_pyramid_finalize_launch(f, groups, C, st);
    SRF_CHECK_LAUNCH("pyramid_finalize", st);
    return srf_pyramid_reg_launch(r, false, rows, st);
  }
  PyrTile tile;
  if (!srf_dbg(SRF_DBG_PYR_NO_LDS_TILES) && pyr_pick_tile(L, D, &tile)) {
    tile.tasks = rows * tile.tiles;
    const size_t tl = (size_t)tile.wave_floats * 4 * sizeof(float);
    const unsigned nb = (unsigned)((tile.tasks + 3) / 4);
    SRF_CHECK_HIP(hipMemsetAsync(mom, 0, sizeof(double) * (size_t)rows * D * 5, st));
    if (a.in_norm.sums) {
      hipLaunchKernelGGL(srf_stats_finalize_kernel, dim3((unsigned)groups), dim3(64), 0, st, a.in_norm.sums,
                         a.in_inv_count, const_cast<float*>(a.in_mr));
      SRF_CHECK_LAUNCH("stats_finalize", st);
    }
    hipLaunchKernelGGL(srf_pyramid_tile_kernel<true>, dim3(nb), dim3(256), tl, st, a, tile);
    SRF_CHECK_LAUNCH("pyramid_moments", st);
    srf_pyramid_finalize_launch(f, groups, C, st);
    SRF_CHECK_LAUNCH("pyramid_finalize", st);
    hipLaunchKernelGGL(srf_pyramid_tile_kernel<false>, dim3(nb), dim3(256), tl, st, a, tile);
    SRF_CHECK_LAUNCH("pyramid_merge", st);
    return SRF_OK;
  }
  const size_t ldsb = pyr_lds_bytes(L, D);
  if (ldsb > 64 * 1024) {
    SRF_CHECK_HIP(hipFuncSetAttribute(reinterpret_cast<const void*>(&srf_pyramid_kernel<true>),
                                      hipFuncAttributeMaxDynamicSharedMemorySize, 160 * 1024));
    SRF_CHECK_HIP(hipFuncSetAttribute(reinterpret_cast<const void*>(&srf_pyramid_kernel<false>),
                                      hipFuncAttributeMaxDynamicSharedMemorySize, 160 * 1024));
  }
  auto resident_blocks = [&](const void* fn) -> long {
    int per_cu = 0;
    if (hipOccupancyMaxActiveBlocksPerMultiprocessor(&per_cu, fn, 256, ldsb) != hipSuccess || per_cu < 1)
      per_cu = 1;
    const long n = (long)per_cu * srf_device_cus();
    return n < rows ? n : rows;
  };
  const long nblk1 = resident_blocks(reinterpret_cast<const void*>(&srf_pyramid_kernel<true>));
  const long nblk2 = resident_blocks(reinterpret_cast<const void*>(&srf_pyramid_kernel<false>));
  hipLaunchKernelGGL(srf_pyramid_kernel<true>, dim3((unsigned)nblk1), dim3(256), ldsb, st, a);
  SRF_CHECK_LAUNCH("pyramid_moments", st);
  srf_pyramid_finalize_launch(f, groups, C, st);
  SRF_CHECK_LAUNCH("pyramid_finalize", st);
  hipLaunchKernelGGL(srf_pyramid_kernel<false>, dim3((unsigned)nblk2), dim3(256), ldsb, st, a);
  SRF_CHECK_LAUNCH("pyramid_merge", st);
  return SRF_OK;
}
```

sudo_rm_rf_amd/csrc/srf_pyramid_reg.hip:

```cpp
#include "srf_pyr.h"


template <int N>
__device__ __forceinline__ void srf_zero(float (&v)[N]) {
#pragma unroll
  for (int i = 0; i < N; ++i) v[i] = 0.f;
}

template <int N>
__device__ __forceinline__ void srf_conv_s1(const float (&x)[N], float (&out)[N], const float* w, float b) {
  const float l2 = srf_lane_up(x[N - 2]), l1 = srf_lane_up(x[N - 1]);
  const float r0 = srf_lane_down(x[0]), r1 = srf_lane_down(x[1]);
  float e[N + 4];
  e[0] = l2;
  e[1] = l1;
#pragma unroll
  for (int i = 0; i < N; ++i) e[i + 2] = x[i];
  e[N + 2] = r0;
  e[N + 3] = r1;
#pragma unroll
  for (int i = 0; i < N; ++i)
    out[i] = fmaf(w[4], e[i + 4], fmaf(w[3], e[i + 3], fmaf(w[2], e[i + 2], fmaf(w[1], e[i + 1], fmaf(w[0], e[i], b)))));
}

template <int N>
__device__ __forceinline__ void srf_conv_s2(const float (&x)[N], float (&out)[N / 2], const float* w, float b) {
  const float l2 = srf_lane_up(x[N - 2]), l1 = srf_lane_up(x[N - 1]);
  const float r0 = srf_lane_down(x[0]);
  float e[N + 3];
  e[0] = l2;
  e[1] = l1;
#pragma unroll
  for (int i = 0; i < N; ++i) e[i + 2] = x[i];
  e[N + 2] = r0;
#pragma unroll
  for (int j = 0; j < N / 2; ++j)
    out[j] = fmaf(w[4], e[2 * j + 4],
                  fmaf(w[3], e[2 * j + 3], fmaf(w[2], e[2 * j + 2], fmaf(w[1], e[2 * j + 1], fmaf(w[0], e[2 * j], b)))));
}

template <int N>
__device__ __forceinline__ void srf_affine_mask(float (&v)[N], float a, float c, bool valid) {
  const float am = valid ? a : 0.f, cm = valid ? c : 0.f;
#pragma unroll
  for (int i = 0; i < N; ++i) v[i] = fmaf(v[i], am, cm);
}

template <int N>
__device__ __forceinline__ void srf_acc_moments(const float (&v)[N], float& s, float& q) {
#pragma unroll
  for (int i = 0; i < N; ++i) {
    s += v[i];
    q = fmaf(v[i], v[i], q);
  }
}

struct LvCoef {
  float w[5], b, a, c;
};

template <int N>
__device__ __forceinline__ void srf_pyr_edges(double* m5, const float (&v)[N], int ci, int nchunks) {
  if (ci == 0) {
    m5[2] = (double)v[0];
    if (N >= 2) m5[3] = (double)v[N >= 2 ? 1 : 0];
  }
  if (N == 1 && ci == 1) m5[3] = (double)v[0];
  if (ci == nchunks - 1) m5[4] = (double)v[N - 1];
}

template <int CH>
__device__ __forceinline__ void srf_pyr_store_chunks(float4* strip, const float (&v)[CH], bool own, float* row_base,
                                                     int first_chunk, int cnt, int lane) {
  constexpr int NF = CH / 4, PF = NF + 1;
  const int j = lane - 2;
  if (own) {
#pragma unroll
    for (int i = 0; i < NF; ++i) strip[j * PF + i] = make_float4(v[4 * i], v[4 * i + 1], v[4 * i + 2], v[4 * i + 3]);
  }
  __builtin_amdgcn_fence(__ATOMIC_RELEASE, "wavefront");
  __builtin_amdgcn_wave_barrier();
  __builtin_amdgcn_fence(__ATOMIC_ACQUIRE, "wavefront");
  float4* dst = reinterpret_cast<float4*>(row_base + (size_t)first_chunk * CH);
#pragma unroll
  for (int it = 0; it < (60 * NF + 63) / 64; ++it) {
    const int f = it * 64 + lane;
    if (f < cnt * NF) dst[f] = strip[(f / NF) * PF + (f % NF)];
  }
  __builtin_amdgcn_fence(__ATOMIC_RELEASE, "wavefront");
  __builtin_amdgcn_wave_barrier();
  __builtin_amdgcn_fence(__ATOMIC_ACQUIRE, "wavefront");
}

template <int N>
__device__ __forceinline__ void srf_pyr_store_level(float* dst, const float (&v)[N]) {
  if constexpr (N >= 4) {
#pragma unroll
    for (int i = 0; i < N / 4; ++i)
      reinterpret_cast<float4*>(dst)[i] = make_float4(v[4 * i], v[4 * i + 1], v[4 * i + 2], v[4 * i + 3]);
  } else if constexpr (N == 2) {
    *reinterpret_cast<float2*>(dst) = make_float2(v[0], v[1]);
  } else {
    dst[0] = v[0];
  }
}

template <bool MOMENTS, int CH, bool PERSIST = MOMENTS, bool SAVE = false>
__global__ __launch_bounds__(256) void srf_pyramid_reg_kernel(PyrRegArgs a) {
  __shared__ float4 pyr_strip[MOMENTS ? 1 : 4 * 60 * (CH / 4 + 1)];
  const int lane = threadIdx.x & 63;
  const int L = a.L, D = a.D, C = a.C;
  const int nchunks = L / CH;
  const int wave = __builtin_amdgcn_readfirstlane(threadIdx.x >> 6);
  int row, row_end, tile, g, c;
  if (PERSIST) {
    row = (blockIdx.x * 4 + wave) * a.rpw;
    if (row >= a.rows) return;
    row_end = min(row + a.rpw, a.rows);
    g = row / C;
    c = row - g * C;
    tile = 0;
  } else {
    c = blockIdx.x;
    g = blockIdx.z;
    row = g * C + c;
    row_end = row + 1;
    tile = blockIdx.y * 4 + wave;
    if (tile >= a.tiles) return;
  }
  const float* in_base = a.y1;
  auto chunk_src = [&](int row_, int tile_) {
    const int ci_ = min(max(tile_ * a.own - 2 + lane, 0), nchunks - 1);
    return reinterpret_cast<const float4*>(in_base + (size_t)row_ * L + ci_ * CH);
  };
  float s1[6], s2[6];
  int cur_g = -1;
  float in_mean = 0.f, in_rstd = 1.f;
  float4 pre[CH / 4];
  {
    const float4* src = chunk_src(row, tile);
#pragma unroll
    for (int i = 0; i < CH / 4; ++i) pre[i] = src[i];
  }
  for (;;) {
  int nrow = row, ntile = tile + 1;
  if (ntile == a.tiles) {
    ntile = 0;
    nrow = row + 1;
  }
  const bool last_task = !PERSIST || nrow >= row_end;
  const int ci = tile * a.own - 2 + lane;
  const bool valid = ci >= 0 && ci < nchunks;
  const bool own = valid && lane >= 2 && lane < 2 + a.own;

  LvCoef lc[SRF_MAX_DEPTH];
#pragma unroll
  for (int k = 0; k < SRF_MAX_DEPTH; ++k) {
    if (k < D && (CH >> k) >= 1) {
#pragma unroll
      for (int t = 0; t < 5; ++t) lc[k].w[t] = a.w[k][c * 5 + t];
      lc[k].b = (MOMENTS && k > 0) ? 0.f : a.bias[k][c];
      if (MOMENTS) {
        lc[k].a = 1.f;
        lc[k].c = 0.f;
      } else {
        const float m = a.lvl[(g * D + k) * 2 + 0], r = a.lvl[(g * D + k) * 2 + 1];
        lc[k].a = a.gamma[k][c] * r;
        lc[k].c = a.beta[k][c] - m * lc[k].a;
      }
    }
  }

  float x0[CH];
  {
    float sc = 1.f, sh = 0.f;
    if (a.in_norm.sums) {
      if (PERSIST) {
        if (g != cur_g) {
          srf_finalize_stats(a.in_norm.sums, g, a.in_inv_count, in_mean, in_rstd);
          cur_g = g;
        }
      } else {
        in_mean = a.in_mr[2 * g];
        in_rstd = a.in_mr[2 * g + 1];
      }
      sc = a.in_norm.gamma[c] * in_rstd;
      sh = a.in_norm.beta[c] - in_mean * sc;
    }
    const bool act = a.in_norm.prelu != nullptr;
    const float slope = act ? a.in_norm.prelu[0] : 1.f;
    float o[CH];
#pragma unroll
    for (int i = 0; i < CH / 4; ++i) {
      const float4 v = pre[i];
      o[4 * i + 0] = v.x;
      o[4 * i + 1] = v.y;
      o[4 * i + 2] = v.z;
      o[4 * i + 3] = v.w;
    }
    const float scm = valid ? sc : 0.f, shm = valid ? sh : 0.f;
#pragma unroll
    for (int i = 0; i < CH; ++i) {
      float v = fmaf(o[i], scm, shm);
      if (act) v = srf_prelu(v, slope);
      o[i] = v;
    }
    srf_conv_s1<CH>(o, x0, lc[0].w, lc[0].b);
    if (SAVE && a.lv_out[0])
      srf_pyr_store_chunks<CH>(pyr_strip + (threadIdx.x >> 6) * (60 * (CH / 4 + 1)), x0, own, a.lv_out[0] + (size_t)row * L,
                               tile * a.own, min(a.own, nchunks - tile * a.own), lane);
    const float vmask = valid ? 1.f : 0.f;
    if (MOMENTS) {
#pragma unroll
      for (int i = 0; i < CH; ++i) x0[i] *= vmask;
    } else {
      srf_affine_mask<CH>(x0, lc[0].a, lc[0].c, valid);
    }
  }

  if (PERSIST) {
    const float4* src = chunk_src(last_task ? row : nrow, last_task ? tile : ntile);
#pragma unroll
    for (int i = 0; i < CH / 4; ++i) pre[i] = src[i];
  }

  float x1[CH / 2], x2[CH / 4], x3[CH / 8], x4[CH / 16], x5[CH / 32 > 0 ? CH / 32 : 1];
  srf_zero(x1);
  srf_zero(x2);
  srf_zero(x3);
  srf_zero(x4);
  srf_zero(x5);
  if (!PERSIST || tile == 0) {
#pragma unroll
    for (int k = 0; k < 6; ++k) s1[k] = s2[k] = 0.f;
  }
  double* mrow = a.mom + (size_t)row * D * 5;
  if (MOMENTS && own) {
    srf_acc_moments<CH>(x0, s1[0], s2[0]);
    srf_pyr_edges<CH>(mrow, x0, ci, nchunks);
  }
  if (D > 1) {
    srf_conv_s2<CH>(x0, x1, lc[1].w, lc[1].b);
    if (SAVE && own) srf_pyr_store_level<CH / 2>(a.lv_out[1] + (size_t)row * (L >> 1) + (size_t)ci * (CH / 2), x1);
    srf_affine_mask<CH / 2>(x1, lc[1].a, lc[1].c, valid);
    if (MOMENTS && own) {
      srf_acc_moments<CH / 2>(x1, s1[1], s2[1]);
      srf_pyr_edges<CH / 2>(mrow + 5, x1, ci, nchunks);
    }
  }
  if (D > 2) {
    srf_conv_s2<CH / 2>(x1, x2, lc[2].w, lc[2].b);
    if (SAVE && own) srf_pyr_store_level<CH / 4>(a.lv_out[2] + (size_t)row * (L >> 2) + (size_t)ci * (CH / 4), x2);
    srf_affine_mask<CH / 4>(x2, lc[2].a, lc[2].c, valid);
    if (MOMENTS && own) {
      srf_acc_moments<CH / 4>(x2, s1[2], s2[2]);
      srf_pyr_edges<CH / 4>(mrow + 10, x2, ci, nchunks);
    }
  }
  if (D > 3) {
    srf_conv_s2<CH / 4>(x2, x3, lc[3].w, lc[3].b);
    if (SAVE && own) srf_pyr_store_level<CH / 8>(a.lv_out[3] + (size_t)row * (L >> 3) + (size_t)ci * (CH / 8), x3);
    srf_affine_mask<CH / 8>(x3, lc[3].a, lc[3].c, valid);
    if (MOMENTS && own) {
      srf_acc_moments<CH / 8>(x3, s1[3], s2[3]);
      srf_pyr_edges<CH / 8>(mrow + 15, x3, ci, nchunks);
    }
  }
  if (D > 4) {
    srf_conv_s2<CH / 8>(x3, x4, lc[4].w, lc[4].b);
    if (SAVE && own) srf_pyr_store_level<CH / 16>(a.lv_out[4] + (size_t)row * (L >> 4) + (size_t)ci * (CH / 16), x4);
    srf_affine_mask<CH / 16>(x4, lc[4].a, lc[4].c, valid);
    if (MOMENTS && own) {
      srf_acc_moments<CH / 16>(x4, s1[4], s2[4]);
      srf_pyr_edges<CH / 16>(mrow + 20, x4, ci, nchunks);
    }
  }
  if constexpr (CH >= 32) {
    if (D > 5) {
      srf_conv_s2<CH / 16>(x4, x5, lc[5].w, lc[5].b);
      if (SAVE && own) srf_pyr_store_level<CH / 32>(a.lv_out[5] + (size_t)row * (L >> 5) + (size_t)ci * (CH / 32), x5);
      srf_affine_mask<CH / 32>(x5, lc[5].a, lc[5].c, valid);
      if (MOMENTS && own) {
        srf_acc_moments<CH / 32>(x5, s1[5], s2[5]);
        srf_pyr_edges<CH / 32>(mrow + 25, x5, ci, nchunks);
      }
    }
  }

  if (MOMENTS) {
#pragma unroll
    for (int k = 0; k < 6; ++k) {
      if (PERSIST && tile != a.tiles - 1) break;
      if (k < D) {
        const float r1 = srf_dpp_wave_sum(s1[k]);
        const float r2 = srf_dpp_wave_sum(s2[k]);
        if (lane == 63) {
          if (PERSIST) {
            mrow[k * 5 + 0] = (double)r1;
            mrow[k * 5 + 1] = (double)r2;
          } else {
            atomicAdd(&mrow[k * 5 + 0], (double)r1);
            atomicAdd(&mrow[k * 5 + 1], (double)r2);
          }
        }
      }
    }
  } else {
    float ms = 0.f, mq = 0.f;
    float outv[CH];
#pragma unroll
    for (int i = 0; i < CH; ++i) {
      float t = 0.f;
      bool have = false;
      if (D > 5 && CH >= 32) {
        t = x5[i >> 5];
        have = true;
      }
      if (D > 4) {
        const float v = x4[i >> 4];
        t = have ? v + t : v;
        have = true;
      }
      if (D > 3) {
        const float v = x3[i >> 3];
        t = have ? v + t : v;
        have = true;
      }
      if (D > 2) {
        const float v = x2[i >> 2];
        t = have ? v + t : v;
        have = true;
      }
      if (D > 1) {
        const float v = x1[i >> 1];
        t = have ? v + t : v;
        have = true;
      }
      const float v = have ? x0[i] + t : x0[i];
      outv[i] = v;
      ms += v;
      mq = fmaf(v, v, mq);
    }
    if (!own) {
      ms = 0.f;
      mq = 0.f;
    }
    srf_pyr_store_chunks<CH>(pyr_strip + wave * (60 * (CH / 4 + 1)), outv, own, a.merged + (size_t)row * L, tile * a.own,
                             min(a.own, nchunks - tile * a.own), lane);
    if (a.out_sums) {
      const double ds = srf_dpp_wave_sum((double)ms), dq = srf_dpp_wave_sum((double)mq);
      if (lane == 63) {
        double* dst = srf_stat_slot(a.out_sums, g, c * a.tiles + tile);
        atomicAdd(dst, ds);
        atomicAdd(dst + 1, dq);
      }
    }
  }
  if (last_task) break;
  if (ntile == 0 && ++c == C) {
    c = 0;
    ++g;
  }
  row = nrow;
  tile = ntile;
  }
}

bool srf_pyramid_reg_supported(int L, int D) {
  if (D <= 5) return L % 16 == 0 && L / 16 >= 4;
  if (D == 6) return L % 32 == 0 && L / 32 >= 4;
  return false;
}

int srf_pyramid_reg_launch(PyrRegArgs a, bool moments, long rows, hipStream_t st) {
  const int CH = a.D <= 5 ? 16 : 32;
  const int nchunks = a.L / CH;
  a.tiles = (nchunks + 59) / 60;
  a.own = (nchunks + a.tiles - 1) / a.tiles;
  SRF_CHECK_ARG(rows * a.tiles < (1L << 31) && rows / a.C <= 65535, "srf_pyramid: too many rows");
  a.rows = (int)rows;
  const bool persist = moments && !srf_dbg(SRF_DBG_PYR_PASS1_NONPERSISTENT);
  long cw = 0;
  if (persist) {
    struct Q { int ch; } q{CH};
    cw = srf_device_cached(CH == 16 ? 0 : 1, [](void* p) -> long {
      const int ch = static_cast<Q*>(p)->ch;
      int per_cu = 0;
      const void* fn = ch == 16 ? (const void*)&srf_pyramid_reg_kernel<true, 16, true>
                                : (const void*)&srf_pyramid_reg_kernel<true, 32, true>;
      if (hipOccupancyMaxActiveBlocksPerMultiprocessor(&per_cu, fn, 256, 0) != hipSuccess || per_cu < 1) per_cu = 2;
      return (long)srf_device_cus() * per_cu * 4;
    }, &q);
  }
  dim3 grid;
  if (persist) {
    long nwaves = cw < rows ? cw : rows;
    a.rpw = srf_dbg(SRF_DBG_PYR_PASS1_ROWS_PER_WAVE) ? (int)((rows + nwaves - 1) / nwaves) : 1;
    nwaves = (rows + a.rpw - 1) / a.rpw;
    grid = dim3((unsigned)((nwaves + 3) / 4));
  } else {
    a.rpw = 1;
    grid = dim3((unsigned)a.C, (unsigned)((a.tiles + 3) / 4), (unsigned)(rows / a.C));
  }
  const bool save = !moments && a.save != 0;
  if (save)
    for (int k = 0; k < a.D; ++k)
      SRF_CHECK_ARG((a.lv_out[k] || (k == 0 && a.D > 1)) && srf_aligned16(a.lv_out[k]), "srf_pyramid: level output %d missing / unaligned", k);
  if (CH == 16) {
    if (moments && persist)
      hipLaunchKernelGGL((srf_pyramid_reg_kernel<true, 16, true>), grid, dim3(256), 0, st, a);
    else if (moments)
      hipLaunchKernelGGL((srf_pyramid_reg_kernel<true, 16, false>), grid, dim3(256), 0, st, a);
    else if (save)
      hipLaunchKernelGGL((srf_pyramid_reg_kernel<false, 16, false, true>), grid, dim3(256), 0, st, a);
    else
      hipLaunchKernelGGL((srf_pyramid_reg_kernel<false, 16, false>), grid, dim3(256), 0, st, a);
  } else {
    if (moments && persist)
      hipLaunchKernelGGL((srf_pyramid_reg_kernel<true, 32, true>), grid, dim3(256), 0, st, a);
    else if (moments)
      hipLaunchKernelGGL((srf_pyramid_reg_kernel<true, 32, false>), grid, dim3(256), 0, st, a);
    else if (save)
      hipLaunchKernelGGL((srf_pyramid_reg_kernel<false, 32, false, true>), grid, dim3(256), 0, st, a);
    else
      hipLaunchKernelGGL((srf_pyramid_reg_kernel<false, 32, false>), grid, dim3(256), 0, st, a);
  }
  SRF_CHECK_LAUNCH(moments ? "pyramid_moments" : (save ? "pyramid_merge_save" : "pyramid_merge"), st);
  return SRF_OK;
}
```

sudo_rm_rf_amd/ops.py:

```python
import contextlib
import ctypes as C
import enum
import weakref

import torch

from . import _lib


def _chk(*ts):
    dev = None
    for t in ts:
        if t is None:
            continue
        if t.device.type != "cuda":
            raise _lib.SrfError("sudo_rm_rf_amd ops need CUDA (ROCm) tensors; got %s" % t.device)
        if not t.is_contiguous():
            raise _lib.SrfError("tensor must be contiguous")
        dev = t.device
    return dev


def new_sums(groups, device):
    return torch.zeros((groups, _lib.STAT_BUCKETS, 2), dtype=torch.float64, device=device)


def _norm(sums, gamma, beta, prelu):
    if sums is None and gamma is None and beta is None and prelu is None:
        return None
    return C.byref(_lib.make_norm(sums, gamma, beta, prelu))


def encoder(wav, weight, L, sums=None):
    dev = _chk(wav, weight, sums)
    Bt, A, T = wav.shape
    N, A2, K = weight.shape
    assert A == A2
    out = torch.empty((Bt, N, L), dtype=torch.float32, device=dev)
    _lib.check(_lib.load().srf_encoder(_lib.ptr(wav), _lib.ptr(weight), _lib.ptr(out), _lib.ptr(sums),
                                       Bt, A, T, N, K, L, _lib.current_stream(dev)), "srf_encoder")
    return out


def gln_stats(x, groups):
    dev = _chk(x)
    sums = new_sums(groups, dev)
    per_group = x.numel() // groups
    _lib.check(_lib.load().srf_gln_stats(_lib.ptr(x), _lib.ptr(sums), groups, per_group,
                                         _lib.current_stream(dev)), "srf_gln_stats")
    return sums


def gln_apply(x, sums, gamma, beta, prelu=None, residual=None):
    dev = _chk(x, sums, gamma, beta, prelu, residual)
    groups, channels = x.shape[0], x.shape[1]
    length = x.numel() // (groups * channels)
    y = torch.empty_like(x)
    n = _lib.make_norm(sums, gamma, beta, prelu)
    lib = _lib.load()
    if residual is None:
        rc = lib.srf_gln_apply(_lib.ptr(x), _lib.ptr(y), C.byref(n), groups, channels, length,
                               _lib.current_stream(dev))
    else:
        rc = lib.srf_gln_apply_add(_lib.ptr(residual), _lib.ptr(x), _lib.ptr(y), C.byref(n), groups,
                                   channels, length, _lib.current_stream(dev))
    _lib.check(rc, "srf_gln_apply")
    return y


def glob_ln(x, gamma, beta):
    x = x.contiguous()
    return gln_apply(x, gln_stats(x, x.shape[0]), gamma, beta)


def pack_pw_weight(weight):
    dev = _chk(weight)
    Cout = weight.shape[0]
    Cin = weight.numel() // Cout
    lib = _lib.load()
    nbytes = lib.srf_packed_pw_weight_bytes(Cout, Cin)
    if not nbytes:
        return None
    packed = torch.empty(nbytes, dtype=torch.uint8, device=dev)
    _lib.check(lib.srf_pack_pw_weights((C.c_void_p * 1)(weight.data_ptr()), (C.c_void_p * 1)(packed.data_ptr()),
                                       (C.c_int * 1)(Cout), (C.c_int * 1)(Cin), 1, _lib.current_stream(dev)),
               "srf_pack_pw_weights")
    return packed


def pack3_pw_weight(weight):
    dev = _chk(weight)
    Cout = weight.shape[0]
    Cin = weight.numel() // Cout
    lib = _lib.load()
    nbytes = lib.srf_packed3_pw_weight_bytes(Cout, Cin)
    if not nbytes:
        return None
    packed = torch.empty(nbytes, dtype=torch.uint8, device=dev)
    _lib.check(lib.srf_pack3_pw_weights((C.c_void_p * 1)(weight.data_ptr()), (C.c_void_p * 1)(packed.data_ptr()),
                                        (C.c_int * 1)(Cout), (C.c_int * 1)(Cin), 1, _lib.current_stream(dev)),
               "srf_pack3_pw_weights")
    weakref.finalize(packed, lib.srf_pack3_forget, packed.data_ptr())
    return packed


def pw_conv3(x, weight, bias, packed3, in_sums=None, in_gamma=None, in_beta=None, in_prelu=None, residual=None, out_sums=None):
    dev = _chk(x, weight, bias, in_sums, in_gamma, in_beta, in_prelu, residual, out_sums)
    Bt, Cin, L = x.shape
    Cout = weight.shape[0]
    y = torch.empty((Bt, Cout, L), dtype=torch.float32, device=dev)
    rc = _lib.load().srf_pw_conv_packed3(_lib.ptr(x), _lib.ptr(weight), _lib.ptr(packed3), _lib.ptr(bias), _lib.ptr(y), Bt, Cin,
                                         Cout, L, _norm(in_sums, in_gamma, in_beta, in_prelu), _lib.ptr(residual),
                                         _lib.ptr(out_sums), _lib.current_stream(dev))
    _lib.check(rc, "srf_pw_conv_packed3")
    return y


def pw_conv(x, weight, bias, in_sums=None, in_gamma=None, in_beta=None, in_prelu=None, residual=None,
            out_sums=None, mask_mul=None, packed=None):
    dev = _chk(x, weight, bias, in_sums, in_gamma, in_beta, in_prelu, residual, out_sums, mask_mul)
    Bt, Cin, L = x.shape
    Cout = weight.shape[0]
    assert weight.numel() == Cout * Cin
    y = torch.empty((Bt, Cout, L), dtype=torch.float32, device=dev)
    lib = _lib.load()
    rc = lib.srf_pw_conv_packed(
        _lib.ptr(x), _lib.ptr(weight), _lib.ptr(packed), _lib.ptr(bias), _lib.ptr(y), Bt, Cin, Cout, L,
        _norm(in_sums, in_gamma, in_beta, in_prelu), _lib.ptr(residual), _lib.ptr(out_sums),
        1 if mask_mul is not None else 0, _lib.ptr(mask_mul),
        mask_mul.shape[1] if mask_mul is not None else 0, _lib.current_stream(dev))
    _lib.check(rc, "srf_pw_conv")
    return y


def pw_conv_pair_supported(Bt, Cin1, Cmid, Cout2, L):
    return bool(_lib.load().srf_pw_conv_pair_supported(Bt, Cin1, Cmid, Cout2, L))


def pw_conv_pair(x, packed1, bias1, in_sums, in_gamma, in_beta, in_prelu, residual, packed2, bias2, Cmid, Cout2, out_sums2=None):
    dev = _chk(x, packed1, bias1, in_sums, in_gamma, in_beta, in_prelu, residual, packed2, bias2, out_sums2)
    Bt, Cin1, L = x.shape
    y = torch.empty((Bt, Cmid, L), dtype=torch.float32, device=dev)
    y2 = torch.empty((Bt, Cout2, L), dtype=torch.float32, device=dev)
    rc = _lib.load().srf_pw_conv_pair(_lib.ptr(x), _lib.ptr(packed1), _lib.ptr(bias1), _lib.ptr(y),
                                      _norm(in_sums, in_gamma, in_beta, in_prelu), _lib.ptr(residual), _lib.ptr(packed2),
                                      _lib.ptr(bias2), _lib.ptr(y2), _lib.ptr(out_sums2), Bt, Cin1, Cmid, Cout2, L,
                                      _lib.current_stream(dev))
    _lib.check(rc, "srf_pw_conv_pair")
    return y, y2


def pw_conv_pair3_supported(Bt, Cin1, Cmid, Cout2, L):
    return bool(_lib.load().srf_pw_conv_pair_packed3_supported(Bt, Cin1, Cmid, Cout2, L))


def pw_conv_pair3(x, packed3_1, bias1, in_sums, in_gamma, in_beta, in_prelu, residual, packed3_2, bias2, Cmid, Cout2, out_sums2=None):
    dev = _chk(x, packed3_1, bias1, in_sums, in_gamma, in_beta, in_prelu, residual, packed3_2, bias2, out_sums2)
    Bt, Cin1, L = x.shape
    y = torch.empty((Bt, Cmid, L), dtype=torch.float32, device=dev)
    y2 = torch.empty((Bt, Cout2, L), dtype=torch.float32, device=dev)
    rc = _lib.load().srf_pw_conv_pair_packed3(_lib.ptr(x), _lib.ptr(packed3_1), _lib.ptr(bias1), _lib.ptr(y),
                                              _norm(in_sums, in_gamma, in_beta, in_prelu), _lib.ptr(residual), _lib.ptr(packed3_2),
                                              _lib.ptr(bias2), _lib.ptr(y2), _lib.ptr(out_sums2), Bt, Cin1, Cmid, Cout2, L,
                                              _lib.current_stream(dev))
    _lib.check(rc, "srf_pw_conv_pair_packed3")
    return y, y2


def dwconv5(x, weight, bias, stride, in_sums=None, in_gamma=None, in_beta=None, in_prelu=None,
            out_sums=None):
    dev = _chk(x, weight, bias, in_sums, in_gamma, in_beta, in_prelu, out_sums)
    Bt, Cc, Lin = x.shape
    Lout = (Lin - 1) // stride + 1
    y = torch.empty((Bt, Cc, Lout), dtype=torch.float32, device=dev)
    rc = _lib.load().srf_dwconv5(_lib.ptr(x), _lib.ptr(weight), _lib.ptr(bias), _lib.ptr(y), Bt, Cc, Lin,
                                 stride, _norm(in_sums, in_gamma, in_beta, in_prelu), _lib.ptr(out_sums),
                                 _lib.current_stream(dev))
    _lib.check(rc, "srf_dwconv5")
    return y


def conv1d(x, weight, bias, stride=1, padding=0, dilation=1, groups=1, out_sums=None):
    dev = _chk(x, weight, bias, out_sums)
    Bt, Cin, Lin = x.shape
    Cout, cpg, K = weight.shape
    if cpg * groups != Cin:
        raise RuntimeError("weight %s does not match %d input channels in %d groups" % (tuple(weight.shape), Cin, groups))
    Lout = (Lin + 2 * padding - dilation * (K - 1) - 1) // stride + 1
    if Lout <= 0:
        raise RuntimeError("kernel size %d (dilation %d) exceeds the padded input length %d" % (K, dilation, Lin + 2 * padding))
    y = torch.empty((Bt, Cout, Lout), dtype=torch.float32, device=dev)
    rc = _lib.load().srf_conv1d(_lib.ptr(x), _lib.ptr(weight), _lib.ptr(bias), _lib.ptr(y), Bt, Cin, Cout, Lin, K, stride,
                                padding, dilation, groups, _lib.ptr(out_sums), _lib.current_stream(dev))
    _lib.check(rc, "srf_conv1d")
    return y


def merge(levels, sums, gammas, betas, out_sums=None):
    dev = _chk(*levels, *sums, *gammas, *betas, out_sums)
    D = len(levels)
    Bt, Cc, L = levels[0].shape
    y = torch.empty((Bt, Cc, L), dtype=torch.float32, device=dev)
    lv = (C.c_void_p * D)(*[t.data_ptr() for t in levels])
    norms = (_lib.srf_norm * D)(*[_lib.make_norm(s, g, b, None) for s, g, b in zip(sums, gammas, betas)])
    rc = _lib.load().srf_merge(lv, norms, D, _lib.ptr(y), Bt, Cc, L, _lib.ptr(out_sums),
                               _lib.current_stream(dev))
    _lib.check(rc, "srf_merge")
    return y


def pyramid(y1, in_sums, in_gamma, in_beta, in_prelu, weights, biases, gammas, betas, out_sums=None):
    dev = _chk(y1, in_sums, in_gamma, in_beta, in_prelu, *weights, *biases, *gammas, *betas, out_sums)
    groups, Cc, L = y1.shape
    D = len(weights)
    lib = _lib.load()
    if not lib.srf_pyramid_supported(Cc, L, D):
        raise _lib.SrfError("srf_pyramid: unsupported shape C=%d L=%d D=%d" % (Cc, L, D))
    merged = torch.empty_like(y1)
    scratch = torch.empty(lib.srf_pyramid_scratch_bytes(groups, Cc, L, D), dtype=torch.uint8, device=dev)
    arr = lambda ts: (C.c_void_p * D)(*[t.data_ptr() for t in ts])
    n = _lib.make_norm(in_sums, in_gamma, in_beta, in_prelu)
    rc = lib.srf_pyramid(_lib.ptr(y1), _lib.ptr(merged), C.byref(n), arr(weights), arr(biases), arr(gammas),
                         arr(betas), groups, Cc, L, D, _lib.ptr(scratch), _lib.ptr(out_sums),
                         _lib.current_stream(dev))
    _lib.check(rc, "srf_pyramid")
    return merged


def decoder(v, weight, T):
    dev = _chk(v, weight)
    Bt, Ci, L = v.shape
    Ci2, Co, K = weight.shape
    assert Ci == Ci2
    lib = _lib.load()
    scratch = torch.empty(lib.srf_decoder_scratch_floats(Bt, Ci, Co, K, L), dtype=torch.float32, device=dev)
    out = torch.empty((Bt, Co, T), dtype=torch.float32, device=dev)
    rc = lib.srf_decoder(_lib.ptr(v), _lib.ptr(weight), _lib.ptr(out), Bt, Ci, Co, K, L, T,
                         _lib.ptr(scratch), _lib.current_stream(dev))
    _lib.check(rc, "srf_decoder")
    return out


def tac(x4, params, out_sums=None):
    dev = _chk(x4, *params, out_sums)
    Bt, G, n, L = x4.shape
    H = params[0].shape[0]
    q = torch.empty_like(x4)
    pp = (C.c_void_p * 9)(*[p.data_ptr() for p in params])
    rc = _lib.load().srf_tac(_lib.ptr(x4), _lib.ptr(q), pp, Bt, G, n, H, L, _lib.ptr(out_sums),
                             _lib.current_stream(dev))
    _lib.check(rc, "srf_tac")
    return q


def mixture_consistency(pr_batch, input_mixture, mix_weights_type="uniform"):
    dev = _chk(pr_batch, input_mixture)
    Bt, S, T = pr_batch.shape
    out = torch.empty_like(pr_batch)
    if mix_weights_type == "magsq":
        work = torch.empty(Bt * S, dtype=torch.float32, device=pr_batch.device)
        rc = _lib.load().srf_mixture_consistency_magsq(_lib.ptr(pr_batch), _lib.ptr(input_mixture), _lib.ptr(out),
                                                       Bt, S, T, _lib.ptr(work), _lib.current_stream(dev))
        _lib.check(rc, "srf_mixture_consistency_magsq")
        return out
    rc = _lib.load().srf_mixture_consistency(_lib.ptr(pr_batch), _lib.ptr(input_mixture), _lib.ptr(out),
                                             Bt, S, T, _lib.current_stream(dev))
    _lib.check(rc, "srf_mixture_consistency")
    return out


def pw_wgrad(g, x, in_sums=None, in_gamma=None, in_beta=None, in_prelu=None, dw=None, dbias=None, want_bias=True):
    dev = _chk(g, x, in_sums, in_gamma, in_beta, in_prelu, dw, dbias)
    Bt, Cout, L = g.shape
    Cin = x.shape[1]
    assert x.shape == (Bt, Cin, L)
    lib = _lib.load()
    acc = dw is not None
    if dw is None:
        dw = torch.empty((Cout, Cin), dtype=torch.float32, device=dev)
    if dbias is None and want_bias:
        assert not acc
        dbias = torch.empty((Cout,), dtype=torch.float32, device=dev)
    scratch = torch.empty(lib.srf_pw_wgrad_scratch_bytes(Bt, Cout, Cin, L), dtype=torch.uint8, device=dev)
    rc = lib.srf_pw_wgrad(_lib.ptr(g), _lib.ptr(x), _norm(in_sums, in_gamma, in_beta, in_prelu), Bt, Cin, Cout, L,
                          _lib.ptr(dw), _lib.ptr(dbias), 1 if acc else 0, _lib.ptr(scratch),
                          _lib.current_stream(dev))
    _lib.check(rc, "srf_pw_wgrad")
    return dw, dbias


def gln_bwd(gout, x, sums, gamma, beta, prelu=None, gout2=None, gx=None, dgamma=None, dbeta=None, dslope=None):
    dev = _chk(gout, x, sums, gamma, beta, prelu, gout2, gx, dgamma, dbeta, dslope)
    groups, Cc, L = x.shape
    lib = _lib.load()
    acc = gx is not None
    if gx is None:
        gx = torch.empty_like(x)
    dgamma = torch.zeros(Cc, dtype=torch.float32, device=dev) if dgamma is None else dgamma
    dbeta = torch.zeros(Cc, dtype=torch.float32, device=dev) if dbeta is None else dbeta
    if prelu is not None and dslope is None:
        dslope = torch.zeros(1, dtype=torch.float32, device=dev)
    scratch = torch.empty(lib.srf_gln_bwd_scratch_bytes(groups, Cc), dtype=torch.uint8, device=dev)
    n = _norm(sums, gamma, beta, prelu)
    rc = lib.srf_gln_bwd(_lib.ptr(gout), _lib.ptr(gout2), _lib.ptr(x), n, groups, Cc, L, _lib.ptr(gx),
                         1 if acc else 0, _lib.ptr(dgamma), _lib.ptr(dbeta), _lib.ptr(dslope), _lib.ptr(scratch),
                         _lib.current_stream(dev))
    _lib.check(rc, "srf_gln_bwd")
    return gx, dgamma, dbeta, dslope


def merge_bwd(g_merged, D):
    dev = _chk(g_merged)
    groups, Cc, L = g_merged.shape
    outs = [g_merged] + [torch.empty((groups, Cc, L >> k), dtype=torch.float32, device=dev) for k in range(1, D)]
    arr = (C.c_void_p * D)(*[t.data_ptr() for t in outs])
    rc = _lib.load().srf_merge_bwd(_lib.ptr(g_merged), arr, D, groups * Cc, L, _lib.current_stream(dev))
    _lib.check(rc, "srf_merge_bwd")
    return outs


def dwconv5_bwd(gd, xin, weight, stride, in_sums=None, in_gamma=None, in_beta=None, in_prelu=None, dw=None,
                dbias=None, want_gin=True):
    dev = _chk(gd, xin, weight, in_sums, in_gamma, in_beta, in_prelu, dw, dbias)
    groups, Cc, Lin = xin.shape
    lib = _lib.load()
    gin = torch.empty_like(xin) if want_gin else None
    dw = torch.zeros((Cc, 1, 5), dtype=torch.float32, device=dev) if dw is None else dw
    dbias = torch.zeros((Cc,), dtype=torch.float32, device=dev) if dbias is None else dbias
    scratch = torch.empty(lib.srf_dwconv5_bwd_scratch_bytes(groups, Cc), dtype=torch.uint8, device=dev)
    rc = lib.srf_dwconv5_bwd(_lib.ptr(gd), _lib.ptr(xin), _norm(in_sums, in_gamma, in_beta, in_prelu), _lib.ptr(weight),
                             groups, Cc, Lin, stride, _lib.ptr(gin), _lib.ptr(dw), _lib.ptr(dbias), _lib.ptr(scratch),
                             _lib.current_stream(dev))
    _lib.check(rc, "srf_dwconv5_bwd")
    return gin, dw, dbias


def mask_apply(m, enc):
    dev = _chk(m, enc)
    Bt, SN, L = m.shape
    N = enc.shape[1]
    v = torch.empty_like(m)
    _lib.check(_lib.load().srf_mask_apply(_lib.ptr(m), _lib.ptr(enc), _lib.ptr(v), Bt, SN // N, N, L,
                                          _lib.current_stream(dev)), "srf_mask_apply")
    return v


def mask_bwd(gv, m, enc, genc=None):
    dev = _chk(gv, m, enc, genc)
    Bt, SN, L = m.shape
    N = enc.shape[1]
    acc = genc is not None
    genc = torch.empty_like(enc) if genc is None else genc
    gm = torch.empty_like(gv)
    _lib.check(_lib.load().srf_mask_bwd(_lib.ptr(gv), _lib.ptr(m), _lib.ptr(enc), _lib.ptr(gm), _lib.ptr(genc),
                                        1 if acc else 0, Bt, SN // N, N, L, _lib.current_stream(dev)), "srf_mask_bwd")
    return gm, genc


def prelu_bwd(gout, x, slope, dslope=None):
    dev = _chk(gout, x, slope, dslope)
    gx = torch.empty_like(gout)
    dslope = torch.zeros(1, dtype=torch.float32, device=dev) if dslope is None else dslope
    _lib.check(_lib.load().srf_prelu_bwd(_lib.ptr(gout), _lib.ptr(x), _lib.ptr(slope), _lib.ptr(gx), _lib.ptr(dslope),
                                         gout.numel(), _lib.current_stream(dev)), "srf_prelu_bwd")
    return gx, dslope


def frames_gather(src, K, hop, pad, L, rows_out=None):
    dev = _chk(src)
    Bt, R, T = src.shape
    rows_out = R * K if rows_out is None else rows_out
    out = torch.empty((Bt, rows_out, L), dtype=torch.float32, device=dev)
    _lib.check(_lib.load().srf_frames_gather(_lib.ptr(src), _lib.ptr(out), Bt, R, T, K, hop, pad, L, rows_out,
                                             _lib.current_stream(dev)), "srf_frames_gather")
    return out


def tac_bwd(x, go, params, grads=None):
    dev = _chk(x, go, *params)
    Bt, G, n, L = x.shape
    lib = _lib.load()
    if grads is None:
        grads = [torch.zeros_like(p) for p in params]
    gx = torch.empty_like(x)
    scratch = torch.empty(lib.srf_tac_bwd_scratch_bytes(Bt, G, n, L), dtype=torch.uint8, device=dev)
    parr = (C.c_void_p * 9)(*[p.data_ptr() for p in params])
    garr = (C.c_void_p * 9)(*[g.data_ptr() for g in grads])
    rc = lib.srf_tac_bwd(_lib.ptr(x), _lib.ptr(go), parr, garr, Bt, G, n, 3 * n, L, _lib.ptr(gx), _lib.ptr(scratch),
                         _lib.current_stream(dev))
    _lib.check(rc, "srf_tac_bwd")
    return gx, grads


def wav_normalize(wav):
    dev = _chk(wav)
    T = wav.shape[-1]
    rows = wav.numel() // T
    out = torch.empty_like(wav)
    stats = torch.empty((rows, 2), dtype=torch.float32, device=dev)
    rc = _lib.load().srf_wav_normalize(_lib.ptr(wav), _lib.ptr(out), _lib.ptr(stats), rows, T,
                                       _lib.current_stream(dev))
    _lib.check(rc, "srf_wav_normalize")
    return out, stats


def wav_denormalize(est, stats, mix_norm=None):
    dev = _chk(est, stats, mix_norm)
    Bt, S, T = est.shape
    assert stats.shape == (Bt, 2)
    out = torch.empty_like(est)
    rc = _lib.load().srf_wav_denormalize(_lib.ptr(est), _lib.ptr(stats), _lib.ptr(mix_norm), _lib.ptr(out),
                                         Bt, S, T, _lib.current_stream(dev))
    _lib.check(rc, "srf_wav_denormalize")
    return out


def causal_encoder(wav, weight, L):
    dev = _chk(wav, weight)
    Bt, A, T = wav.shape
    N, A2, KW = weight.shape
    if A != A2 or KW % 2 == 0:
        raise _lib.SrfError("causal_encoder: weight %s does not fit input %s" % (tuple(weight.shape), tuple(wav.shape)))
    K = (KW + 1) // 2
    out = torch.empty((Bt, N, L), dtype=torch.float32, device=dev)
    _lib.check(_lib.load().srf_causal_encoder(_lib.ptr(wav), _lib.ptr(weight), _lib.ptr(out), Bt, A, T, N, K, L,
                                              _lib.current_stream(dev)), "srf_causal_encoder")
    return out


def causal_dwconv(x, weight, bias, stride, in_prelu=None, out_prelu=None):
    dev = _chk(x, weight, bias, in_prelu, out_prelu)
    Bt, Cc, Lin = x.shape
    if weight.shape != (Cc, 1, 21):
        raise _lib.SrfError("causal_dwconv: weight must be [%d, 1, 21], got %s" % (Cc, tuple(weight.shape)))
    y = torch.empty((Bt, Cc, (Lin - 1) // stride + 1), dtype=torch.float32, device=dev)
    rc = _lib.load().srf_causal_dwconv(_lib.ptr(x), _lib.ptr(weight), _lib.ptr(bias), _lib.ptr(in_prelu), _lib.ptr(out_prelu),
                                       _lib.ptr(y), Bt, Cc, Lin, stride, _lib.current_stream(dev))
    _lib.check(rc, "srf_causal_dwconv")
    return y


def causal_merge(levels):
    dev = _chk(*levels)
    Bt, Cc, L = levels[0].shape
    D = len(levels)
    y = torch.empty_like(levels[0])
    arr = (C.c_void_p * D)(*[t.data_ptr() for t in levels])
    _lib.check(_lib.load().srf_causal_merge(arr, D, _lib.ptr(y), Bt, Cc, L, _lib.current_stream(dev)), "srf_causal_merge")
    return y


def causal_pyramid_supported(C_, L, D):
    return bool(_lib.load().srf_causal_pyramid_supported(C_, L, D))


def causal_pyramid(y1, in_prelu, weights, biases, prelus):
    dev = _chk(y1, in_prelu, *weights, *biases, *prelus)
    Bt, Cc, L = y1.shape
    D = len(weights)
    lib = _lib.load()
    if not lib.srf_causal_pyramid_supported(Cc, L, D):
        raise _lib.SrfError("srf_causal_pyramid: unsupported shape C=%d L=%d D=%d" % (Cc, L, D))
    merged = torch.empty_like(y1)
    arr = lambda ts: (C.c_void_p * D)(*[t.data_ptr() for t in ts])
    rc = lib.srf_causal_pyramid(_lib.ptr(y1), _lib.ptr(merged), _lib.ptr(in_prelu), arr(weights), arr(biases), arr(prelus),
                                Bt, Cc, L, D, _lib.current_stream(dev))
    _lib.check(rc, "srf_causal_pyramid")
    return merged


def causal_stream_pyramid(y1, state, in_prelu, weights, biases, prelus):
    dev = _chk(y1, in_prelu, *state, *weights, *biases, *prelus)
    Bt, Cc, Lc = y1.shape
    D = len(weights)
    if len(state) != D or any(tuple(s.shape) != (Bt, Cc, 10) for s in state):
        raise _lib.SrfError("causal_stream_pyramid: state must be %d tensors of shape [%d, %d, 10]" % (D, Bt, Cc))
    merged = torch.empty_like(y1)
    arr = lambda ts: (C.c_void_p * D)(*[t.data_ptr() for t in ts])
    rc = _lib.load().srf_causal_stream_pyramid(_lib.ptr(y1), _lib.ptr(merged), arr(state), _lib.ptr(in_prelu), arr(weights),
                                               arr(biases), arr(prelus), Bt, Cc, Lc, D, _lib.current_stream(dev))
    _lib.check(rc, "srf_causal_stream_pyramid")
    return merged


def causal_scale(src, dscale=None, hscale=1.0):
    dev = _chk(src, dscale)
    dst = torch.empty_like(src)
    rc = _lib.load().srf_causal_scale(_lib.ptr(src), _lib.ptr(dst), src.numel(), _lib.ptr(dscale), float(hscale),
                                      _lib.current_stream(dev))
    _lib.check(rc, "srf_causal_scale")
    return dst


def prelu(x, slope):
    dev = _chk(x, slope)
    y = torch.empty_like(x)
    _lib.check(_lib.load().srf_prelu_apply(_lib.ptr(x), _lib.ptr(slope), _lib.ptr(y), x.numel(), _lib.current_stream(dev)),
               "srf_prelu_apply")
    return y


class DebugFlag(enum.IntFlag):
    NO_PAIRS = 1
    GEMM_NO_MGROUPS = 2
    NO_GEMM_256 = 4
    NO_PACKED_WEIGHTS = 8
    PYR_PER_LEVEL = 16
    PYR_NO_LDS_TILES = 32
    PYR_NO_REG = 64
    PYR_PASS1_NONPERSISTENT = 128
    GEMM_WHOLE_TAIL_TILES = 256
    GEMM_QUARTER_TILES_LAST = 512
    TAC_ONE_STEP_PER_LANE = 1024
    GEMM_128_ONE_TILE_PER_BLOCK = 2048
    WGRAD_NO_XCD_MAP = 4096
    GEMM_256_SWAP_FORMS = 8192
    TRAIN_BF16X3 = 16384
    NO_FUSED_TAIL = 32768
    BWD_NO_FUSED_HEAD = 1 << 16
    PYR_PASS1_ROWS_PER_WAVE = 1 << 17
    WGRAD_NO_WIDE_TILE = 1 << 18
    WGRAD_128_MASKED = 1 << 19
    WGRAD_SHORT_CHUNKS = 1 << 20
    PAIR_PERSISTENT = 1 << 21
    TAC_VALU = 1 << 22
    PAIR_FULL_DRAIN = 1 << 23
    TAC_GENERIC = 1 << 24
    WGRAD_ONE_CHAIN_FOLD = 1 << 25
    TAC_LANES_4TILES = 1 << 26
    GEMM_128_POINTER_LOADS = 1 << 27
    TRAIN_FWD_SPLIT_BF16 = 1 << 28
    BWD_DW_CHUNKED = 1 << 29
    BWD_GLN_SCALAR = 1 << 30
    TRAIN_FWD_EXACT_MFMA = 1 << 31


_debug_flags = 0


def set_debug_flags(flags):
    global _debug_flags
    bits = int(flags) & 0xFFFFFFFF
    _lib.load().srf_set_debug_flags(bits - (1 << 32) if bits >> 31 else bits)
    _debug_flags = bits


@contextlib.contextmanager
def debug_flags(flags):
    prev = _debug_flags
    set_debug_flags(flags)
    try:
        yield
    finally:
        set_debug_flags(prev)


def set_kernel_mode(mode):
    _lib.load().srf_set_kernel_mode(int(mode))


def get_kernel_mode():
    return int(_lib.load().srf_get_kernel_mode())


class kernel_trace:

    def __init__(self, device):
        self.device = torch.device(device)
        self.launches, self.names = [], set()

    def __enter__(self):
        self._stream = _lib.current_stream(self.device)
        _lib.check(_lib.load().srf_profile_begin(self._stream), "srf_profile_begin")
        return self

    def __exit__(self, *exc):
        lib = _lib.load()
        cnt = C.c_int(0)
        _lib.check(lib.srf_profile_end(self._stream, C.byref(cnt)), "srf_profile_end")
        name, ms = C.c_char_p(), C.c_float()
        for i in range(cnt.value):
            lib.srf_profile_get(i, C.byref(name), C.byref(ms))
            if not name.value.startswith(b"("):
                self.launches.append((name.value.decode(), ms.value))
        self.names = {n for n, _ in self.launches}
        return False
```

Baseline: 22420.

## Fuse pyramid moments, finalize and merge into one persistent kernel launch

```diff
diff --git a/include/sudormrf_hip.h b/include/sudormrf_hip.h
--- a/include/sudormrf_hip.h
+++ b/include/sudormrf_hip.h
@@ -7,7 +7,7 @@
 extern "C" {
 #endif
 
-#define SRF_ABI_VERSION 18
+#define SRF_ABI_VERSION 19
 
 #define SRF_STAT_BUCKETS 64
 
@@ -88,6 +88,17 @@
   SRF_DBG_TRAIN_FWD_EXACT_MFMA = -2147483647 - 1
 };
 void srf_set_debug_flags(int flags);
+enum srf_debug_flag2 {
+  SRF_DBG2_PYR_THREE_LAUNCHES = 1,
+  SRF_DBG2_PYR_ASCENDING = 2,
+  SRF_DBG2_PROFILE_KEEPS_FUSED = 4,
+  SRF_DBG2_PYR_PREREAD_HANDOFF = 8,
+  SRF_DBG2_PYR_ONE_LAUNCH = 16,
+  SRF_DBG2_PYR_LAG_SHIFT = 8,
+  SRF_DBG2_PYR_LAG_MASK = 0xff00
+};
+void srf_set_debug_flags2(int flags);
+int srf_debug_flags2(void);
 #endif
 
 int srf_plan_create(const srf_config* cfg, int batch, int T, srf_plan** out);
diff --git a/sudo_rm_rf_amd/_diag.py b/sudo_rm_rf_amd/_diag.py
--- /dev/null
+++ b/sudo_rm_rf_amd/_diag.py
@@ -0,0 +1,32 @@
+import contextlib
+import enum
+
+from . import _lib
+
+
+class DebugFlag2(enum.IntFlag):
+    PYR_THREE_LAUNCHES = 1
+    PYR_ASCENDING = 2
+    PROFILE_KEEPS_FUSED = 4
+    PYR_PREREAD_HANDOFF = 8
+    PYR_ONE_LAUNCH = 16
+
+    @staticmethod
+    def pyr_lag(k):
+        if not 0 <= int(k) <= 255:
+            raise ValueError("lag %r outside 0..255" % (k,))
+        return int(k) << 8
+
+
+def set_debug_flags2(flags):
+    _lib.load().srf_set_debug_flags2(int(flags))
+
+
+@contextlib.contextmanager
+def debug_flags2(flags):
+    prev = _lib.load().srf_debug_flags2()
+    set_debug_flags2(flags)
+    try:
+        yield
+    finally:
+        set_debug_flags2(prev)
diff --git a/sudo_rm_rf_amd/_lib.py b/sudo_rm_rf_amd/_lib.py
--- a/sudo_rm_rf_amd/_lib.py
+++ b/sudo_rm_rf_amd/_lib.py
@@ -6,7 +6,7 @@
 
 _PKG = os.path.dirname(os.path.abspath(__file__))
 LIB_PATH = os.environ.get("SRF_LIB") or os.path.join(_PKG, "libsudormrf_hip.so")
-ABI_VERSION = 18
+ABI_VERSION = 19
 STAT_BUCKETS = 64
 
 SRF_OK = 0
@@ -52,6 +52,8 @@
     "srf_gln_apply_add": (_i, [_vp, _vp, _vp, C.POINTER(srf_norm), _i, _i, _i, _vp]),
     "srf_pw_conv": (_i, [_vp, _vp, _vp, _vp, _i, _i, _i, _i, C.POINTER(srf_norm), _vp, _vp, _i, _vp, _i, _vp]),
     "srf_set_debug_flags": (None, [_i]),
+    "srf_set_debug_flags2": (None, [_i]),
+    "srf_debug_flags2": (_i, []),
     "srf_packed_pw_weight_bytes": (_sz, [_i, _i]),
     "srf_pack_pw_weights": (_i, [C.POINTER(_vp), C.POINTER(_vp), C.POINTER(_i), C.POINTER(_i), _i, _vp]),
     "srf_pw_conv_packed": (_i, [_vp, _vp, _vp, _vp, _vp, _i, _i, _i, _i, C.POINTER(srf_norm), _vp, _vp, _i, _vp, _i, _vp]),
diff --git a/sudo_rm_rf_amd/build.py b/sudo_rm_rf_amd/build.py
--- a/sudo_rm_rf_amd/build.py
+++ b/sudo_rm_rf_amd/build.py
@@ -13,7 +13,7 @@
 SOURCES = ["srf_api.hip", "srf_encoder.hip", "srf_elementwise.hip", "srf_dwconv.hip", "srf_pyramid.hip", "srf_pyramid_reg.hip", "srf_pwconv.hip", "srf_pwconv_bf16x3.hip", "srf_pwconv_x3w.hip", "srf_pwconv_x3p.hip", "srf_pwconv_x3f.hip", "srf_pwconv_w4.hip", "srf_pwconv_small.hip",
            "srf_tac.hip", "srf_loss.hip", "srf_pwconv_wgrad.hip", "srf_backward.hip", "srf_train.hip", "srf_augment.hip", "srf_optim.hip", "srf_feeder.hip",
            "srf_causal.hip", "srf_causal_stream.hip", "srf_loss_fuss.hip"]
-HEADERS = [os.path.join(CSRC, "srf_common.h"), os.path.join(CSRC, "srf_internal.h"), os.path.join(CSRC, "srf_pw.h"), os.path.join(CSRC, "srf_plan.h"), os.path.join(CSRC, "srf_pyr.h"),
+HEADERS = [os.path.join(CSRC, "srf_common.h"), os.path.join(CSRC, "srf_internal.h"), os.path.join(CSRC, "srf_pw.h"), os.path.join(CSRC, "srf_plan.h"), os.path.join(CSRC, "srf_pyr.h"), os.path.join(CSRC, "srf_pyramid_reg_body.inc"),
            os.path.join(os.path.dirname(PKG), "include", "sudormrf_hip.h")]
 FLAGS = ["-O3", "-std=c++17", "--offload-arch=gfx950", "-fPIC", "-munsafe-fp-atomics",
          "-Wall", "-Wno-unused-function"]
@@ -75,6 +75,11 @@
     if not os.path.exists(asm):
         raise RuntimeError("ISA lint: device assembly %s was not produced" % asm)
     hits = isa_lint(asm)
+    with open(asm, errors="replace") as f:
+        text = f.read()
+    m = re.search(r"^amdhsa\.kernels:.*?^amdhsa\.target:", text, re.S | re.M)
+    with open(os.path.join(OBJ, base + ".kernels.yaml"), "w") as f:
+        f.write(m.group(0) if m else "")
     for f in os.listdir(OBJ):
         if f.startswith(base + "-h") or f.startswith(base + ".hip-"):
             os.remove(os.path.join(OBJ, f))
diff --git a/sudo_rm_rf_amd/csrc/srf_api.hip b/sudo_rm_rf_amd/csrc/srf_api.hip
--- a/sudo_rm_rf_amd/csrc/srf_api.hip
+++ b/sudo_rm_rf_amd/csrc/srf_api.hip
@@ -1,3 +1,4 @@
+#include <stdlib.h>
 #include <string.h>
 
 #include <atomic>
@@ -26,6 +27,12 @@
 static std::atomic<int> g_debug_flags{0};
 int srf_debug_flags() { return g_debug_flags.load(std::memory_order_relaxed); }
 extern "C" void srf_set_debug_flags(int f) { g_debug_flags.store(f, std::memory_order_relaxed); }
+static std::atomic<int> g_debug_flags2{[] {
+  const char* e = getenv("SUDORMRF_DEBUG_FLAGS2");
+  return e ? (int)strtol(e, nullptr, 0) : 0;
+}()};
+extern "C" int srf_debug_flags2(void) { return g_debug_flags2.load(std::memory_order_relaxed); }
+extern "C" void srf_set_debug_flags2(int f) { g_debug_flags2.store(f, std::memory_order_relaxed); }
 
 static std::mutex g_dev_mu;
 static int g_dev_cus[SRF_MAX_DEVICES];
diff --git a/sudo_rm_rf_amd/csrc/srf_common.h b/sudo_rm_rf_amd/csrc/srf_common.h
--- a/sudo_rm_rf_amd/csrc/srf_common.h
+++ b/sudo_rm_rf_amd/csrc/srf_common.h
@@ -14,6 +14,7 @@
 int srf_kernel_mode_override(int mode);
 int srf_debug_flags();
 static inline bool srf_dbg(int mask) { return (srf_debug_flags() & mask) != 0; }
+static inline bool srf_dbg2(int mask) { return (srf_debug_flags2() & mask) != 0; }
 bool srf_profiling();
 void srf_prof_hold(int delta);
 void srf_prof_mark(const char* name, hipStream_t st);
diff --git a/sudo_rm_rf_amd/csrc/srf_pyr.h b/sudo_rm_rf_amd/csrc/srf_pyr.h
--- a/sudo_rm_rf_amd/csrc/srf_pyr.h
+++ b/sudo_rm_rf_amd/csrc/srf_pyr.h
@@ -23,3 +23,79 @@
 };
 
 int srf_pyramid_reg_launch(PyrRegArgs a, bool moments, long rows, hipStream_t st);
+
+#define SRF_PYR_CTL_TICKET 0
+#define SRF_PYR_CTL_TIMEOUT 3
+#define SRF_PYR_CTL_COUNTERS 4
+#define SRF_PYR_GRANULES 16
+#define SRF_PYR_GRANULE_IN 10
+#define SRF_PYR_FUSED_MAX_D 5
+#define SRF_PYR_FUSED_MAX_C 512
+static inline size_t srf_pyr_ctl_granule_off(int groups) {
+  return srf_align_up(sizeof(unsigned) * (SRF_PYR_CTL_COUNTERS + (size_t)groups), 128);
+}
+static inline size_t srf_pyr_ctl_bytes(int groups) {
+  return srf_pyr_ctl_granule_off(groups) + (size_t)groups * SRF_PYR_GRANULES * 8;
+}
+
+struct PyrFusedArgs {
+  unsigned* ctl;
+  unsigned long long* gran;
+  int ticket_word;
+  int G, K;
+  int descending;
+  int preread;
+  unsigned a1, aF, a2;
+  unsigned TA, TB, TC;
+  unsigned long long mA, mB, m2, mC;
+};
+
+bool srf_pyramid_fused_supported(int groups, int C, int L, int D);
+int srf_pyramid_fused_launch(PyrRegArgs a, void* ctl, int groups, int role_mask, bool zero_ctl, hipStream_t st);
+
+struct PyrFinState {
+  double alpha, kap, g0, g1, gl;
+};
+
+__device__ __forceinline__ void srf_pyr_fin_accum(const PyrFinState& t, const double (&mo)[5], int Lk, double& s, double& q) {
+  const double S1 = mo[0], S2 = mo[1], e0 = mo[2], e1 = mo[3], el = mo[4];
+  s += t.alpha * S1 + (Lk - 3) * t.kap + t.g0 + t.g1 + t.gl;
+  q += t.alpha * t.alpha * S2 +
+       2.0 * t.alpha * (t.kap * (S1 - e0 - e1 - el) + t.g0 * e0 + t.g1 * e1 + t.gl * el) +
+       (Lk - 3) * t.kap * t.kap + t.g0 * t.g0 + t.g1 * t.g1 + t.gl * t.gl;
+}
+
+__device__ __forceinline__ void srf_pyr_fin_level(const double* red, int C, int Lk, float& mean_f, float& rstd_f, double& ts,
+                                                  double& tq) {
+  ts = 0.0;
+  tq = 0.0;
+  for (int w = 0; w < 4; ++w) {
+    ts += red[2 * w];
+    tq += red[2 * w + 1];
+  }
+  const double n = (double)C * (double)Lk;
+  const double mean = ts / n;
+  double var = tq / n - mean * mean;
+  var = var < 0.0 ? 0.0 : var;
+  mean_f = (float)mean;
+  rstd_f = (float)(1.0 / sqrt(var + 1e-8));
+}
+
+__device__ __forceinline__ void srf_pyr_fin_advance(PyrFinState& t, float gam, float bet, const float (&w)[5], float bias,
+                                                    float mean_f, float rstd_f) {
+  const float af = gam * rstd_f;
+  const float bf = bet - mean_f * af;
+  const double A = (double)af, B = (double)bf;
+  const double w0 = w[0], w1 = w[1], w2 = w[2], w3 = w[3], w4 = w[4];
+  const double bs = (double)bias;
+  const double sw = w0 + w1 + w2 + w3 + w4;
+  const double nk = bs + A * t.kap * sw + B * sw;
+  const double n0 = bs + A * (w2 * t.g0 + w3 * t.g1 + w4 * t.kap) + B * (w2 + w3 + w4);
+  const double n1 = bs + A * (w0 * t.g0 + w1 * t.g1 + (w2 + w3 + w4) * t.kap) + B * sw;
+  const double nl = bs + A * ((w0 + w1 + w2) * t.kap + w3 * t.gl) + B * (w0 + w1 + w2 + w3);
+  t.kap = nk;
+  t.g0 = n0;
+  t.g1 = n1;
+  t.gl = nl;
+  t.alpha *= A;
+}
diff --git a/sudo_rm_rf_amd/csrc/srf_pyramid.hip b/sudo_rm_rf_amd/csrc/srf_pyramid.hip
--- a/sudo_rm_rf_amd/csrc/srf_pyramid.hip
+++ b/sudo_rm_rf_amd/csrc/srf_pyramid.hip
@@ -557,11 +557,11 @@
       a.in_mr[2 * g + 1] = r;
     }
   }
-  double alpha[CPT], kap[CPT], g0[CPT], g1[CPT], gl[CPT];
+  PyrFinState fs[CPT];
 #pragma unroll
   for (int i = 0; i < CPT; ++i) {
-    alpha[i] = 1.0;
-    kap[i] = g0[i] = g1[i] = gl[i] = 0.0;
+    fs[i].alpha = 1.0;
+    fs[i].kap = fs[i].g0 = fs[i].g1 = fs[i].gl = 0.0;
   }
   constexpr bool PRE = CPT <= 2;
   double mo[PRE ? SRF_MAX_DEPTH : 1][CPT][5];
@@ -600,13 +600,7 @@
 #pragma unroll
     for (int i = 0; i < CPT; ++i) {
       const int c = tid + 256 * i;
-      if (c < C) {
-        const double S1 = mo[slot][i][0], S2 = mo[slot][i][1], e0 = mo[slot][i][2], e1 = mo[slot][i][3], el = mo[slot][i][4];
-        s += alpha[i] * S1 + (Lk - 3) * kap[i] + g0[i] + g1[i] + gl[i];
-        q += alpha[i] * alpha[i] * S2 +
-             2.0 * alpha[i] * (kap[i] * (S1 - e0 - e1 - el) + g0[i] * e0 + g1[i] * e1 + gl[i] * el) +
-             (Lk - 3) * kap[i] * kap[i] + g0[i] * g0[i] + g1[i] * g1[i] + gl[i] * gl[i];
-      }
+      if (c < C) srf_pyr_fin_accum(fs[i], mo[slot][i], Lk, s, q);
     }
     s = srf_dpp_wave_sum(s);
     q = srf_dpp_wave_sum(q);
@@ -617,17 +611,8 @@
     __syncthreads();
     float mean_f, rstd_f;
     {
-      double ts = 0.0, tq = 0.0;
-      for (int w = 0; w < 4; ++w) {
-        ts += red[2 * w];
-        tq += red[2 * w + 1];
-      }
-      const double n = (double)C * (double)Lk;
-      const double mean = ts / n;
-      double var = tq / n - mean * mean;
-      var = var < 0.0 ? 0.0 : var;
-      mean_f = (float)mean;
-      rstd_f = (float)(1.0 / sqrt(var + 1e-8));
+      double ts, tq;
+      srf_pyr_fin_level(red, C, Lk, mean_f, rstd_f, ts, tq);
       if (tid == 0) {
         a.lvl[(g * D + k) * 2 + 0] = mean_f;
         a.lvl[(g * D + k) * 2 + 1] = rstd_f;
@@ -642,23 +627,7 @@
 #pragma unroll
       for (int i = 0; i < CPT; ++i) {
         const int c = tid + 256 * i;
-        if (c < C) {
-          const float af = gam_[i] * rstd_f;
-          const float bf = bet_[i] - mean_f * af;
-          const double A = (double)af, B = (double)bf;
-          const double w0 = w_[i][0], w1 = w_[i][1], w2 = w_[i][2], w3 = w_[i][3], w4 = w_[i][4];
-          const double bs = (double)bias_[i];
-          const double sw = w0 + w1 + w2 + w3 + w4;
-          const double nk = bs + A * kap[i] * sw + B * sw;
-          const double n0 = bs + A * (w2 * g0[i] + w3 * g1[i] + w4 * kap[i]) + B * (w2 + w3 + w4);
-          const double n1 = bs + A * (w0 * g0[i] + w1 * g1[i] + (w2 + w3 + w4) * kap[i]) + B * sw;
-          const double nl = bs + A * ((w0 + w1 + w2) * kap[i] + w3 * gl[i]) + B * (w0 + w1 + w2 + w3);
-          kap[i] = nk;
-          g0[i] = n0;
-          g1[i] = n1;
-          gl[i] = nl;
-          alpha[i] *= A;
-        }
+        if (c < C) srf_pyr_fin_advance(fs[i], gam_[i], bet_[i], w_[i], bias_[i], mean_f, rstd_f);
       }
     }
     __syncthreads();
@@ -689,7 +658,8 @@
 }
 
 static size_t pyr_small_bytes(int groups, int C, int D) {
-  const size_t b = sizeof(double) * (size_t)groups * C * D * 5 + sizeof(float) * (size_t)groups * (D * 2 + 2);
+  const size_t b = srf_pyr_ctl_bytes(groups) + sizeof(double) * (size_t)groups * C * D * 5 +
+                   sizeof(float) * (size_t)groups * (D * 2 + 2);
   return (b + 255) & ~(size_t)255;
 }
 extern "C" size_t srf_pyramid_scratch_bytes(int groups, int C, int L, int D) {
@@ -753,7 +723,7 @@
   hipStream_t st = (hipStream_t)stream;
   const long rows = (long)groups * C;
   SRF_CHECK_ARG(rows < (1L << 31), "srf_pyramid: too many rows");
-  double* mom = reinterpret_cast<double*>(scratch);
+  double* mom = reinterpret_cast<double*>(reinterpret_cast<char*>(scratch) + srf_pyr_ctl_bytes(groups));
   float* lvl = reinterpret_cast<float*>(mom + (size_t)rows * D * 5);
   PyrArgs a;
   PyrFinArgs f;
@@ -822,6 +792,24 @@
       }
     }
     SRF_CHECK_ARG(merged != y1, "srf_pyramid: merged must not alias y1 (pass 2 re-reads y1 with halos)");
+    if (!lv_out && srf_pyramid_fused_supported(groups, C, L, D)) {
+      if (srf_profiling() && !srf_dbg2(SRF_DBG2_PROFILE_KEEPS_FUSED)) {
+        int rc = srf_pyramid_fused_launch(r, scratch, groups, 1, true, st);
+        if (rc) return rc;
+        SRF_CHECK_LAUNCH("pyramid_moments", st);
+        rc = srf_pyramid_fused_launch(r, scratch, groups, 2, false, st);
+        if (rc) return rc;
+        SRF_CHECK_LAUNCH("pyramid_finalize", st);
+        rc = srf_pyramid_fused_launch(r, scratch, groups, 4, false, st);
+        if (rc) return rc;
+        SRF_CHECK_LAUNCH("pyramid_merge", st);
+        return SRF_OK;
+      }
+      const int rc = srf_pyramid_fused_launch(r, scratch, groups, 7, true, st);
+      if (rc) return rc;
+      SRF_CHECK_LAUNCH("pyramid_fused", st);
+      return SRF_OK;
+    }
     int rc = srf_pyramid_reg_launch(r, true, rows, st);
     if (rc) return rc;
     if (!srf_dbg(SRF_DBG_PYR_PASS1_NONPERSISTENT)) f.in_sums = a.in_norm.sums;
diff --git a/sudo_rm_rf_amd/csrc/srf_pyramid_reg.hip b/sudo_rm_rf_amd/csrc/srf_pyramid_reg.hip
--- a/sudo_rm_rf_amd/csrc/srf_pyramid_reg.hip
+++ b/sudo_rm_rf_amd/csrc/srf_pyramid_reg.hip
@@ -59,14 +59,14 @@
   float w[5], b, a, c;
 };
 
-template <int N>
+template <int N, class Hand>
 __device__ __forceinline__ void srf_pyr_edges(double* m5, const float (&v)[N], int ci, int nchunks) {
   if (ci == 0) {
-    m5[2] = (double)v[0];
-    if (N >= 2) m5[3] = (double)v[N >= 2 ? 1 : 0];
-  }
-  if (N == 1 && ci == 1) m5[3] = (double)v[0];
-  if (ci == nchunks - 1) m5[4] = (double)v[N - 1];
+    Hand::store_mom(m5 + 2, (double)v[0]);
+    if (N >= 2) Hand::store_mom(m5 + 3, (double)v[N >= 2 ? 1 : 0]);
+  }
+  if (N == 1 && ci == 1) Hand::store_mom(m5 + 3, (double)v[0]);
+  if (ci == nchunks - 1) Hand::store_mom(m5 + 4, (double)v[N - 1]);
 }
 
 template <int CH>
@@ -105,12 +105,29 @@
   }
 }
 
+template <class T>
+__device__ __forceinline__ T srf_ldc(const T* p, int i) {
+  return ((const __attribute__((address_space(4))) T*)p)[i];
+}
+
+struct PyrHandPlain {
+  struct {
+    const float* lvl;
+    const float* in_mr;
+    int D;
+  } a;
+  static __device__ __forceinline__ void store_mom(double* p, double v) { *p = v; }
+  __device__ __forceinline__ float lvl_mean(int g, int k) const { return a.lvl[(g * a.D + k) * 2 + 0]; }
+  __device__ __forceinline__ float lvl_rstd(int g, int k) const { return a.lvl[(g * a.D + k) * 2 + 1]; }
+  __device__ __forceinline__ float in_mean(int g) const { return a.in_mr[2 * g]; }
+  __device__ __forceinline__ float in_rstd(int g) const { return a.in_mr[2 * g + 1]; }
+};
+
+
 template <bool MOMENTS, int CH, bool PERSIST = MOMENTS, bool SAVE = false>
 __global__ __launch_bounds__(256) void srf_pyramid_reg_kernel(PyrRegArgs a) {
   __shared__ float4 pyr_strip[MOMENTS ? 1 : 4 * 60 * (CH / 4 + 1)];
-  const int lane = threadIdx.x & 63;
-  const int L = a.L, D = a.D, C = a.C;
-  const int nchunks = L / CH;
+  const int C = a.C;
   const int wave = __builtin_amdgcn_readfirstlane(threadIdx.x >> 6);
   int row, row_end, tile, g, c;
   if (PERSIST) {
@@ -128,242 +145,346 @@
     tile = blockIdx.y * 4 + wave;
     if (tile >= a.tiles) return;
   }
-  const float* in_base = a.y1;
-  auto chunk_src = [&](int row_, int tile_) {
-    const int ci_ = min(max(tile_ * a.own - 2 + lane, 0), nchunks - 1);
-    return reinterpret_cast<const float4*>(in_base + (size_t)row_ * L + ci_ * CH);
+  using Hand = PyrHandPlain;
+  const Hand h{{a.lvl, a.in_mr, a.D}};
+#include "srf_pyramid_reg_body.inc"
+}
+
+typedef __attribute__((address_space(1))) unsigned srf_gu32;
+typedef __attribute__((address_space(1))) unsigned long long srf_gu64;
+#define SRF_PYR_WAIT_TICKS 20000000LL
+#define SRF_PYR_EPOCH 1u
+
+__device__ __forceinline__ unsigned srf_pyr_ld32(const unsigned* p) {
+  return __hip_atomic_load((srf_gu32*)p, __ATOMIC_RELAXED, __HIP_MEMORY_SCOPE_AGENT);
+}
+__device__ __forceinline__ void srf_pyr_granule_store(unsigned long long* p, float v) {
+  __hip_atomic_store((srf_gu64*)p, ((unsigned long long)SRF_PYR_EPOCH << 32) | (unsigned)__float_as_int(v), __ATOMIC_RELAXED,
+                     __HIP_MEMORY_SCOPE_AGENT);
+}
+__device__ __forceinline__ bool srf_pyr_spin_fail(unsigned* tmo, unsigned code, long long t0) {
+  if (srf_pyr_ld32(tmo) != 0) return true;
+  if (wall_clock64() - t0 > SRF_PYR_WAIT_TICKS) {
+    if ((threadIdx.x & 63) == 0) __hip_atomic_store((srf_gu32*)tmo, code, __ATOMIC_RELAXED, __HIP_MEMORY_SCOPE_AGENT);
+    return true;
+  }
+  __builtin_amdgcn_s_sleep(8);
+  return false;
+}
+
+struct PyrHandFused {
+  float st[12];
+  static __device__ __forceinline__ void store_mom(double* p, double v) {
+    __hip_atomic_store((srf_gu64*)p, (unsigned long long)__double_as_longlong(v), __ATOMIC_RELAXED, __HIP_MEMORY_SCOPE_AGENT);
+  }
+  __device__ __forceinline__ float lvl_mean(int, int k) const { return k < SRF_PYR_FUSED_MAX_D ? st[2 * k] : 0.f; }
+  __device__ __forceinline__ float lvl_rstd(int, int k) const { return k < SRF_PYR_FUSED_MAX_D ? st[2 * k + 1] : 0.f; }
+  __device__ __forceinline__ float in_mean(int) const { return st[SRF_PYR_GRANULE_IN]; }
+  __device__ __forceinline__ float in_rstd(int) const { return st[SRF_PYR_GRANULE_IN + 1]; }
+};
+
+__device__ __forceinline__ unsigned srf_pyr_div(unsigned n, unsigned long long magic) {
+  return (unsigned)(((unsigned long long)n * magic) >> 32);
+}
+
+struct PyrFusedFin {
+  const double* mom;
+  const double* in_sums;
+  double in_inv_count;
+  float* in_mr;
+  float* lvl;
+  const float* w[SRF_PYR_FUSED_MAX_D];
+  const float* bias[SRF_PYR_FUSED_MAX_D];
+  const float* gamma[SRF_PYR_FUSED_MAX_D];
+  const float* beta[SRF_PYR_FUSED_MAX_D];
+  int C, L, D, preread;
+  unsigned* ctl;
+  unsigned long long* gp;
+};
+__device__ __forceinline__ void srf_pyramid_fused_finalize(const PyrFusedFin a, int g, double* lds, unsigned* ctl_cache,
+                                                           int wave) {
+  const int tid = threadIdx.x, lane = tid & 63, C = a.C, D = a.D;
+  double* kap = lds;
+  double* g0 = lds + SRF_PYR_FUSED_MAX_C;
+  double* g1 = lds + 2 * SRF_PYR_FUSED_MAX_C;
+  double* gl = lds + 3 * SRF_PYR_FUSED_MAX_C;
+  double* red = lds + 4 * SRF_PYR_FUSED_MAX_C;
+  unsigned* tmo = a.ctl + SRF_PYR_CTL_TIMEOUT;
+  unsigned long long* gp = a.gp;
+  const double* mbase = a.mom + (size_t)g * C * D * 5;
+  auto load_level = [&](double (&mo)[2][5], int k) {
+#pragma unroll
+    for (int i = 0; i < 2; ++i) {
+      const int c = min(tid + 256 * i, C - 1);
+      const double* m = mbase + ((size_t)c * D + k) * 5;
+#pragma unroll
+      for (int e = 0; e < 5; ++e) mo[i][e] = m[e];
+    }
   };
-  float s1[6], s2[6];
-  int cur_g = -1;
-  float in_mean = 0.f, in_rstd = 1.f;
-  float4 pre[CH / 4];
-  {
-    const float4* src = chunk_src(row, tile);
-#pragma unroll
-    for (int i = 0; i < CH / 4; ++i) pre[i] = src[i];
-  }
-  for (;;) {
-  int nrow = row, ntile = tile + 1;
-  if (ntile == a.tiles) {
-    ntile = 0;
-    nrow = row + 1;
-  }
-  const bool last_task = !PERSIST || nrow >= row_end;
-  const int ci = tile * a.own - 2 + lane;
-  const bool valid = ci >= 0 && ci < nchunks;
-  const bool own = valid && lane >= 2 && lane < 2 + a.own;
-
-  LvCoef lc[SRF_MAX_DEPTH];
-#pragma unroll
-  for (int k = 0; k < SRF_MAX_DEPTH; ++k) {
-    if (k < D && (CH >> k) >= 1) {
-#pragma unroll
-      for (int t = 0; t < 5; ++t) lc[k].w[t] = a.w[k][c * 5 + t];
-      lc[k].b = (MOMENTS && k > 0) ? 0.f : a.bias[k][c];
-      if (MOMENTS) {
-        lc[k].a = 1.f;
-        lc[k].c = 0.f;
-      } else {
-        const float m = a.lvl[(g * D + k) * 2 + 0], r = a.lvl[(g * D + k) * 2 + 1];
-        lc[k].a = a.gamma[k][c] * r;
-        lc[k].c = a.beta[k][c] - m * lc[k].a;
+  if (a.preread) {
+    double pre[2][5];
+    load_level(pre, 0);
+    asm volatile("" ::"v"(pre[0][0]), "v"(pre[1][4]));
+  }
+  if (wave == 0) {
+    const long long t0 = wall_clock64();
+    const unsigned code = (2u << 24) | (unsigned)g;
+    bool ok = true;
+    while (srf_pyr_ld32(a.ctl + SRF_PYR_CTL_COUNTERS + g) != (unsigned)C) {
+      if (srf_pyr_spin_fail(tmo, code, t0)) {
+        ok = false;
+        break;
       }
     }
-  }
-
-  float x0[CH];
-  {
-    float sc = 1.f, sh = 0.f;
-    if (a.in_norm.sums) {
-      if (PERSIST) {
-        if (g != cur_g) {
-          srf_finalize_stats(a.in_norm.sums, g, a.in_inv_count, in_mean, in_rstd);
-          cur_g = g;
-        }
-      } else {
-        in_mean = a.in_mr[2 * g];
-        in_rstd = a.in_mr[2 * g + 1];
+    if (ok) {
+      __builtin_amdgcn_fence(__ATOMIC_ACQUIRE, "agent");
+      asm volatile("s_waitcnt vmcnt(0)" ::: "memory");
+    }
+    if (lane == 0) ctl_cache[1] = ok ? 1u : 0u;
+  }
+  __syncthreads();
+  if (ctl_cache[1] == 0) {
+    if (tid < 2 * D) a.lvl[(size_t)g * D * 2 + tid] = __builtin_nanf("");
+    return;
+  }
+  if (wave == 0) {
+    float m = 0.f, r = 1.f;
+    if (a.in_sums) srf_finalize_stats(a.in_sums, g, a.in_inv_count, m, r);
+    if (lane == 0) {
+      srf_pyr_granule_store(gp + SRF_PYR_GRANULE_IN, m);
+      srf_pyr_granule_store(gp + SRF_PYR_GRANULE_IN + 1, r);
+      if (a.in_sums && a.in_mr) {
+        a.in_mr[2 * g] = m;
+        a.in_mr[2 * g + 1] = r;
       }
-      sc = a.in_norm.gamma[c] * in_rstd;
-      sh = a.in_norm.beta[c] - in_mean * sc;
-    }
-    const bool act = a.in_norm.prelu != nullptr;
-    const float slope = act ? a.in_norm.prelu[0] : 1.f;
-    float o[CH];
-#pragma unroll
-    for (int i = 0; i < CH / 4; ++i) {
-      const float4 v = pre[i];
-      o[4 * i + 0] = v.x;
-      o[4 * i + 1] = v.y;
-      o[4 * i + 2] = v.z;
-      o[4 * i + 3] = v.w;
-    }
-    const float scm = valid ? sc : 0.f, shm = valid ? sh : 0.f;
-#pragma unroll
-    for (int i = 0; i < CH; ++i) {
-      float v = fmaf(o[i], scm, shm);
-      if (act) v = srf_prelu(v, slope);
-      o[i] = v;
-    }
-    srf_conv_s1<CH>(o, x0, lc[0].w, lc[0].b);
-    if (SAVE && a.lv_out[0])
-      srf_pyr_store_chunks<CH>(pyr_strip + (threadIdx.x >> 6) * (60 * (CH / 4 + 1)), x0, own, a.lv_out[0] + (size_t)row * L,
-                               tile * a.own, min(a.own, nchunks - tile * a.own), lane);
-    const float vmask = valid ? 1.f : 0.f;
-    if (MOMENTS) {
-#pragma unroll
-      for (int i = 0; i < CH; ++i) x0[i] *= vmask;
-    } else {
-      srf_affine_mask<CH>(x0, lc[0].a, lc[0].c, valid);
-    }
-  }
-
-  if (PERSIST) {
-    const float4* src = chunk_src(last_task ? row : nrow, last_task ? tile : ntile);
-#pragma unroll
-    for (int i = 0; i < CH / 4; ++i) pre[i] = src[i];
-  }
-
-  float x1[CH / 2], x2[CH / 4], x3[CH / 8], x4[CH / 16], x5[CH / 32 > 0 ? CH / 32 : 1];
-  srf_zero(x1);
-  srf_zero(x2);
-  srf_zero(x3);
-  srf_zero(x4);
-  srf_zero(x5);
-  if (!PERSIST || tile == 0) {
-#pragma unroll
-    for (int k = 0; k < 6; ++k) s1[k] = s2[k] = 0.f;
-  }
-  double* mrow = a.mom + (size_t)row * D * 5;
-  if (MOMENTS && own) {
-    srf_acc_moments<CH>(x0, s1[0], s2[0]);
-    srf_pyr_edges<CH>(mrow, x0, ci, nchunks);
-  }
-  if (D > 1) {
-    srf_conv_s2<CH>(x0, x1, lc[1].w, lc[1].b);
-    if (SAVE && own) srf_pyr_store_level<CH / 2>(a.lv_out[1] + (size_t)row * (L >> 1) + (size_t)ci * (CH / 2), x1);
-    srf_affine_mask<CH / 2>(x1, lc[1].a, lc[1].c, valid);
-    if (MOMENTS && own) {
-      srf_acc_moments<CH / 2>(x1, s1[1], s2[1]);
-      srf_pyr_edges<CH / 2>(mrow + 5, x1, ci, nchunks);
-    }
-  }
-  if (D > 2) {
-    srf_conv_s2<CH / 2>(x1, x2, lc[2].w, lc[2].b);
-    if (SAVE && own) srf_pyr_store_level<CH / 4>(a.lv_out[2] + (size_t)row * (L >> 2) + (size_t)ci * (CH / 4), x2);
-    srf_affine_mask<CH / 4>(x2, lc[2].a, lc[2].c, valid);
-    if (MOMENTS && own) {
-      srf_acc_moments<CH / 4>(x2, s1[2], s2[2]);
-      srf_pyr_edges<CH / 4>(mrow + 10, x2, ci, nchunks);
-    }
-  }
-  if (D > 3) {
-    srf_conv_s2<CH / 4>(x2, x3, lc[3].w, lc[3].b);
-    if (SAVE && own) srf_pyr_store_level<CH / 8>(a.lv_out[3] + (size_t)row * (L >> 3) + (size_t)ci * (CH / 8), x3);
-    srf_affine_mask<CH / 8>(x3, lc[3].a, lc[3].c, valid);
-    if (MOMENTS && own) {
-      srf_acc_moments<CH / 8>(x3, s1[3], s2[3]);
-      srf_pyr_edges<CH / 8>(mrow + 15, x3, ci, nchunks);
-    }
-  }
-  if (D > 4) {
-    srf_conv_s2<CH / 8>(x3, x4, lc[4].w, lc[4].b);
-    if (SAVE && own) srf_pyr_store_level<CH / 16>(a.lv_out[4] + (size_t)row * (L >> 4) + (size_t)ci * (CH / 16), x4);
-    srf_affine_mask<CH / 16>(x4, lc[4].a, lc[4].c, valid);
-    if (MOMENTS && own) {
-      srf_acc_moments<CH / 16>(x4, s1[4], s2[4]);
-      srf_pyr_edges<CH / 16>(mrow + 20, x4, ci, nchunks);
-    }
-  }
-  if constexpr (CH >= 32) {
-    if (D > 5) {
-      srf_conv_s2<CH / 16>(x4, x5, lc[5].w, lc[5].b);
-      if (SAVE && own) srf_pyr_store_level<CH / 32>(a.lv_out[5] + (size_t)row * (L >> 5) + (size_t)ci * (CH / 32), x5);
-      srf_affine_mask<CH / 32>(x5, lc[5].a, lc[5].c, valid);
-      if (MOMENTS && own) {
-        srf_acc_moments<CH / 32>(x5, s1[5], s2[5]);
-        srf_pyr_edges<CH / 32>(mrow + 25, x5, ci, nchunks);
+    }
+  }
+  double alpha[2] = {1.0, 1.0};
+#pragma unroll
+  for (int i = 0; i < 2; ++i) kap[tid + 256 * i] = g0[tid + 256 * i] = g1[tid + 256 * i] = gl[tid + 256 * i] = 0.0;
+  double mo[2][5];
+  load_level(mo, 0);
+#pragma unroll
+  for (int k = 0; k < SRF_PYR_FUSED_MAX_D; ++k) {
+    if (k >= D) break;
+    const int Lk = a.L >> k;
+    double s = 0.0, q = 0.0;
+#pragma unroll
+    for (int i = 0; i < 2; ++i) {
+      const int c = tid + 256 * i;
+      if (c < C) {
+        const PyrFinState t{alpha[i], kap[c], g0[c], g1[c], gl[c]};
+        srf_pyr_fin_accum(t, mo[i], Lk, s, q);
       }
     }
-  }
-
-  if (MOMENTS) {
-#pragma unroll
-    for (int k = 0; k < 6; ++k) {
-      if (PERSIST && tile != a.tiles - 1) break;
-      if (k < D) {
-        const float r1 = srf_dpp_wave_sum(s1[k]);
-        const float r2 = srf_dpp_wave_sum(s2[k]);
-        if (lane == 63) {
-          if (PERSIST) {
-            mrow[k * 5 + 0] = (double)r1;
-            mrow[k * 5 + 1] = (double)r2;
-          } else {
-            atomicAdd(&mrow[k * 5 + 0], (double)r1);
-            atomicAdd(&mrow[k * 5 + 1], (double)r2);
-          }
+    s = srf_dpp_wave_sum(s);
+    q = srf_dpp_wave_sum(q);
+    if (lane == 63) {
+      red[wave * 2] = s;
+      red[wave * 2 + 1] = q;
+    }
+    __syncthreads();
+    float mean_f, rstd_f;
+    double ts, tq;
+    srf_pyr_fin_level(red, C, Lk, mean_f, rstd_f, ts, tq);
+    if (tid == 0) {
+      srf_pyr_granule_store(gp + 2 * k, mean_f);
+      srf_pyr_granule_store(gp + 2 * k + 1, rstd_f);
+      a.lvl[((size_t)g * D + k) * 2 + 0] = mean_f;
+      a.lvl[((size_t)g * D + k) * 2 + 1] = rstd_f;
+    }
+    if (k + 1 < D) {
+#pragma unroll
+      for (int i = 0; i < 2; ++i) {
+        const int c = tid + 256 * i;
+        if (c < C) {
+          float w[5];
+#pragma unroll
+          for (int t5 = 0; t5 < 5; ++t5) w[t5] = a.w[k + 1][c * 5 + t5];
+          PyrFinState t{alpha[i], kap[c], g0[c], g1[c], gl[c]};
+          srf_pyr_fin_advance(t, a.gamma[k][c], a.beta[k][c], w, a.bias[k + 1][c], mean_f, rstd_f);
+          alpha[i] = t.alpha;
+          kap[c] = t.kap;
+          g0[c] = t.g0;
+          g1[c] = t.g1;
+          gl[c] = t.gl;
         }
       }
-    }
+      load_level(mo, k + 1);
+    }
+    __syncthreads();
+  }
+  if (tid == 0)
+    for (int k = D; k < SRF_PYR_FUSED_MAX_D; ++k) {
+      srf_pyr_granule_store(gp + 2 * k, 0.f);
+      srf_pyr_granule_store(gp + 2 * k + 1, 0.f);
+    }
+}
+
+template <int CH>
+__global__ __launch_bounds__(256, 7) void srf_pyramid_fused_kernel(PyrRegArgs a, PyrFusedArgs f) {
+  __shared__ float4 pyr_strip[4 * 60 * (CH / 4 + 1)];
+  __shared__ unsigned ctl_cache[4];
+  static_assert(sizeof(double) * (4 * SRF_PYR_FUSED_MAX_C + 8) <= sizeof(float4) * 4 * 60 * (CH / 4 + 1), "finalize state");
+  const int lane = threadIdx.x & 63;
+  const int wave = __builtin_amdgcn_readfirstlane(threadIdx.x >> 6);
+  if (threadIdx.x == 0)
+    ctl_cache[0] = __hip_atomic_fetch_add((srf_gu32*)(f.ctl + f.ticket_word), 1u, __ATOMIC_RELAXED, __HIP_MEMORY_SCOPE_AGENT);
+  __syncthreads();
+  const unsigned t = __builtin_amdgcn_readfirstlane(ctl_cache[0]);
+  const unsigned dA = f.a1 + f.aF, dB = dA + f.a2;
+  unsigned s, r;
+  if (t < f.a1) {
+    s = 0;
+    r = t;
+  } else if (t < f.TA) {
+    const unsigned u = t - f.a1, j = srf_pyr_div(u, f.mA);
+    s = j + 1;
+    r = u - j * dA;
+  } else if (t < f.TB) {
+    const unsigned u = t - f.TA, j = srf_pyr_div(u, f.mB);
+    s = f.K + j;
+    r = u - j * dB;
+  } else if (t < f.TC) {
+    s = f.G;
+    r = t - f.TB + f.a1;
   } else {
-    float ms = 0.f, mq = 0.f;
-    float outv[CH];
-#pragma unroll
-    for (int i = 0; i < CH; ++i) {
-      float t = 0.f;
-      bool have = false;
-      if (D > 5 && CH >= 32) {
-        t = x5[i >> 5];
-        have = true;
+    const unsigned u = t - f.TC, j = srf_pyr_div(u, f.m2);
+    s = f.G + 1 + j;
+    r = u - j * f.a2 + dA;
+  }
+  const int role = r < f.a1 ? 0 : (r < dA ? 1 : 2);
+  const int es = (int)s - (role == 0 ? 0 : (role == 1 ? 1 : f.K));
+  const int ex = f.descending ? f.G - 1 - es : es;
+  PyrHandFused h;
+#pragma unroll
+  for (int i = 0; i < 12; ++i) h.st[i] = 0.f;
+
+  if (role == 0) {
+    const int nc = a.C;
+    int g = ex, c = (int)r * 4 + wave;
+    if (c < nc) {
+      constexpr bool MOMENTS = true, PERSIST = true, SAVE = false;
+      using Hand = PyrHandFused;
+      int row = g * nc + c, row_end = row + 1, tile = 0;
+#include "srf_pyramid_reg_body.inc"
+    }
+    asm volatile("s_waitcnt vmcnt(0)" ::: "memory");
+    __syncthreads();
+    if (threadIdx.x == 0)
+      __hip_atomic_fetch_add((srf_gu32*)(f.ctl + SRF_PYR_CTL_COUNTERS + ex), (unsigned)min(4, nc - (int)r * 4), __ATOMIC_RELAXED,
+                             __HIP_MEMORY_SCOPE_AGENT);
+  } else if (role == 1) {
+    PyrFusedFin ff;
+    ff.mom = a.mom;
+    ff.in_sums = a.in_norm.sums;
+    ff.in_inv_count = a.in_inv_count;
+    ff.in_mr = const_cast<float*>(a.in_mr);
+    ff.lvl = const_cast<float*>(a.lvl);
+#pragma unroll
+    for (int k = 0; k < SRF_PYR_FUSED_MAX_D; ++k) {
+      ff.w[k] = a.w[k];
+      ff.bias[k] = a.bias[k];
+      ff.gamma[k] = a.gamma[k];
+      ff.beta[k] = a.beta[k];
+    }
+    ff.C = a.C;
+    ff.L = a.L;
+    ff.D = a.D;
+    ff.ctl = f.ctl;
+    ff.gp = f.gran + (size_t)ex * SRF_PYR_GRANULES;
+    ff.preread = f.preread;
+    srf_pyramid_fused_finalize(ff, ex, reinterpret_cast<double*>(pyr_strip), ctl_cache, wave);
+  } else {
+    const int nc = a.C;
+    const unsigned idx = r - dA, tgi = srf_pyr_div(idx, f.mC);
+    int g = ex, c = (int)(idx - tgi * (unsigned)nc);
+    int tile = (int)tgi * 4 + wave;
+    if (tile >= a.tiles) return;
+    unsigned long long* gp = f.gran + (size_t)ex * SRF_PYR_GRANULES;
+    const int gi = lane < 12 ? lane : 0;
+    if (f.preread) {
+      const unsigned long long x = gp[gi];
+      asm volatile("" ::"v"(x));
+    }
+    const long long t0 = wall_clock64();
+    unsigned long long x;
+    bool ok = true;
+    for (;;) {
+      x = __hip_atomic_load((srf_gu64*)(gp + gi), __ATOMIC_RELAXED, __HIP_MEMORY_SCOPE_AGENT);
+      if (__all((unsigned)(x >> 32) == SRF_PYR_EPOCH)) break;
+      if (srf_pyr_spin_fail(f.ctl + SRF_PYR_CTL_TIMEOUT, (3u << 24) | (unsigned)ex, t0)) {
+        ok = false;
+        break;
       }
-      if (D > 4) {
-        const float v = x4[i >> 4];
-        t = have ? v + t : v;
-        have = true;
-      }
-      if (D > 3) {
-        const float v = x3[i >> 3];
-        t = have ? v + t : v;
-        have = true;
-      }
-      if (D > 2) {
-        const float v = x2[i >> 2];
-        t = have ? v + t : v;
-        have = true;
-      }
-      if (D > 1) {
-        const float v = x1[i >> 1];
-        t = have ? v + t : v;
-        have = true;
-      }
-      const float v = have ? x0[i] + t : x0[i];
-      outv[i] = v;
-      ms += v;
-      mq = fmaf(v, v, mq);
-    }
-    if (!own) {
-      ms = 0.f;
-      mq = 0.f;
-    }
-    srf_pyr_store_chunks<CH>(pyr_strip + wave * (60 * (CH / 4 + 1)), outv, own, a.merged + (size_t)row * L, tile * a.own,
-                             min(a.own, nchunks - tile * a.own), lane);
-    if (a.out_sums) {
-      const double ds = srf_dpp_wave_sum((double)ms), dq = srf_dpp_wave_sum((double)mq);
-      if (lane == 63) {
-        double* dst = srf_stat_slot(a.out_sums, g, c * a.tiles + tile);
-        atomicAdd(dst, ds);
-        atomicAdd(dst + 1, dq);
-      }
-    }
-  }
-  if (last_task) break;
-  if (ntile == 0 && ++c == C) {
-    c = 0;
-    ++g;
-  }
-  row = nrow;
-  tile = ntile;
-  }
+    }
+    int row = g * nc + c, row_end = row + 1;
+    if (!ok) {
+      const int first = tile * a.own, cnt = min(a.own, a.L / CH - first);
+      float* dst = a.merged + (size_t)row * a.L + (size_t)first * CH;
+      for (int i = lane; i < cnt * CH; i += 64) dst[i] = __builtin_nanf("");
+      return;
+    }
+#pragma unroll
+    for (int i = 0; i < 12; ++i) h.st[i] = __int_as_float(__builtin_amdgcn_readlane((int)(unsigned)x, i));
+    constexpr bool MOMENTS = false, PERSIST = false, SAVE = false;
+    using Hand = PyrHandFused;
+#include "srf_pyramid_reg_body.inc"
+  }
+}
+
+static unsigned long long pyr_magic(unsigned d) { return d ? (1ULL << 32) / d + 1 : 0; }
+
+static void pyr_fused_tasks(int C, int L, unsigned* a1, unsigned* a2) {
+  const int nchunks = L / 16, tiles = (nchunks + 59) / 60;
+  *a1 = (unsigned)((C + 3) / 4);
+  *a2 = (unsigned)C * (unsigned)((tiles + 3) / 4);
+}
+
+bool srf_pyramid_fused_supported(int groups, int C, int L, int D) {
+  if (!srf_dbg2(SRF_DBG2_PYR_ONE_LAUNCH) || srf_dbg2(SRF_DBG2_PYR_THREE_LAUNCHES)) return false;
+  if (srf_dbg(SRF_DBG_PYR_NO_REG | SRF_DBG_PYR_PASS1_NONPERSISTENT)) return false;
+  if (D > SRF_PYR_FUSED_MAX_D || C > SRF_PYR_FUSED_MAX_C || !srf_pyramid_reg_supported(L, D)) return false;
+  unsigned a1, a2;
+  pyr_fused_tasks(C, L, &a1, &a2);
+  const unsigned long long per = (unsigned long long)a1 + 1 + a2, total = per * (unsigned)groups;
+  return groups <= 65535 && total < (1ULL << 31) && total * per < (1ULL << 32);
+}
+
+#define SRF_PYR_DEFAULT_LAG 3
+
+int srf_pyramid_fused_launch(PyrRegArgs a, void* ctl, int groups, int role_mask, bool zero_ctl, hipStream_t st) {
+  const int nchunks = a.L / 16;
+  a.tiles = (nchunks + 59) / 60;
+  a.own = (nchunks + a.tiles - 1) / a.tiles;
+  a.rows = groups * a.C;
+  a.rpw = 1;
+  PyrFusedArgs f;
+  f.ctl = reinterpret_cast<unsigned*>(ctl);
+  f.gran = reinterpret_cast<unsigned long long*>(reinterpret_cast<char*>(ctl) + srf_pyr_ctl_granule_off(groups));
+  f.ticket_word = SRF_PYR_CTL_TICKET + (role_mask == 2 ? 1 : (role_mask == 4 ? 2 : 0));
+  f.G = groups;
+  const int lag = (srf_debug_flags2() & SRF_DBG2_PYR_LAG_MASK) >> SRF_DBG2_PYR_LAG_SHIFT;
+  f.K = lag ? lag : SRF_PYR_DEFAULT_LAG;
+  if (f.K > groups) f.K = groups;
+  f.descending = srf_dbg2(SRF_DBG2_PYR_ASCENDING) ? 0 : 1;
+  f.preread = srf_dbg2(SRF_DBG2_PYR_PREREAD_HANDOFF) ? 1 : 0;
+  unsigned a1, a2;
+  pyr_fused_tasks(a.C, a.L, &a1, &a2);
+  f.a1 = (role_mask & 1) ? a1 : 0;
+  f.aF = (role_mask & 2) ? 1 : 0;
+  f.a2 = (role_mask & 4) ? a2 : 0;
+  const unsigned dA = f.a1 + f.aF, dB = dA + f.a2;
+  f.TA = f.a1 + (unsigned)(f.K - 1) * dA;
+  f.TB = f.TA + (unsigned)(groups - f.K) * dB;
+  f.TC = f.TB + f.aF + f.a2;
+  f.mA = pyr_magic(dA);
+  f.mB = pyr_magic(dB);
+  f.m2 = pyr_magic(f.a2);
+  f.mC = pyr_magic((unsigned)a.C);
+  if (zero_ctl) SRF_CHECK_HIP(hipMemsetAsync(ctl, 0, srf_pyr_ctl_bytes(groups), st));
+  hipLaunchKernelGGL(srf_pyramid_fused_kernel<16>, dim3((unsigned)groups * dB), dim3(256), 0, st, a, f);
+  return SRF_OK;
 }
 
 bool srf_pyramid_reg_supported(int L, int D) {
diff --git a/sudo_rm_rf_amd/csrc/srf_pyramid_reg_body.inc b/sudo_rm_rf_amd/csrc/srf_pyramid_reg_body.inc
--- /dev/null
+++ b/sudo_rm_rf_amd/csrc/srf_pyramid_reg_body.inc
@@ -0,0 +1,241 @@
+{
+  const int lane = threadIdx.x & 63;
+  const int L = a.L, D = a.D, C = a.C;
+  const int nchunks = L / CH;
+  const float* in_base = a.y1;
+  auto chunk_src = [&](int row_, int tile_) {
+    const int ci_ = min(max(tile_ * a.own - 2 + lane, 0), nchunks - 1);
+    return reinterpret_cast<const float4*>(in_base + (size_t)row_ * L + ci_ * CH);
+  };
+  float s1[6], s2[6];
+  int cur_g = -1;
+  float in_mean = 0.f, in_rstd = 1.f;
+  float4 pre[CH / 4];
+  {
+    const float4* src = chunk_src(row, tile);
+#pragma unroll
+    for (int i = 0; i < CH / 4; ++i) pre[i] = src[i];
+  }
+  for (;;) {
+  int nrow = row, ntile = tile + 1;
+  if (ntile == a.tiles) {
+    ntile = 0;
+    nrow = row + 1;
+  }
+  const bool last_task = !PERSIST || nrow >= row_end;
+  const int ci = tile * a.own - 2 + lane;
+  const bool valid = ci >= 0 && ci < nchunks;
+  const bool own = valid && lane >= 2 && lane < 2 + a.own;
+
+  LvCoef lc[SRF_MAX_DEPTH];
+#pragma unroll
+  for (int k = 0; k < SRF_MAX_DEPTH; ++k) {
+    if (k < D && (CH >> k) >= 1) {
+#pragma unroll
+      for (int t = 0; t < 5; ++t) lc[k].w[t] = srf_ldc(a.w[k], c * 5 + t);
+      lc[k].b = (MOMENTS && k > 0) ? 0.f : srf_ldc(a.bias[k], c);
+      if (MOMENTS) {
+        lc[k].a = 1.f;
+        lc[k].c = 0.f;
+      } else {
+        const float m = h.lvl_mean(g, k), r = h.lvl_rstd(g, k);
+        lc[k].a = srf_ldc(a.gamma[k], c) * r;
+        lc[k].c = srf_ldc(a.beta[k], c) - m * lc[k].a;
+      }
+    }
+  }
+
+  float x0[CH];
+  {
+    float sc = 1.f, sh = 0.f;
+    if (a.in_norm.sums) {
+      if (PERSIST) {
+        if (g != cur_g) {
+          srf_finalize_stats(a.in_norm.sums, g, a.in_inv_count, in_mean, in_rstd);
+          cur_g = g;
+        }
+      } else {
+        in_mean = h.in_mean(g);
+        in_rstd = h.in_rstd(g);
+      }
+      sc = srf_ldc(a.in_norm.gamma, c) * in_rstd;
+      sh = srf_ldc(a.in_norm.beta, c) - in_mean * sc;
+    }
+    const bool act = a.in_norm.prelu != nullptr;
+    const float slope = act ? srf_ldc(a.in_norm.prelu, 0) : 1.f;
+    float o[CH];
+#pragma unroll
+    for (int i = 0; i < CH / 4; ++i) {
+      const float4 v = pre[i];
+      o[4 * i + 0] = v.x;
+      o[4 * i + 1] = v.y;
+      o[4 * i + 2] = v.z;
+      o[4 * i + 3] = v.w;
+    }
+    const float scm = valid ? sc : 0.f, shm = valid ? sh : 0.f;
+#pragma unroll
+    for (int i = 0; i < CH; ++i) {
+      float v = fmaf(o[i], scm, shm);
+      if (act) v = srf_prelu(v, slope);
+      o[i] = v;
+    }
+    srf_conv_s1<CH>(o, x0, lc[0].w, lc[0].b);
+    if (SAVE && a.lv_out[0])
+      srf_pyr_store_chunks<CH>(pyr_strip + (threadIdx.x >> 6) * (60 * (CH / 4 + 1)), x0, own, a.lv_out[0] + (size_t)row * L,
+                               tile * a.own, min(a.own, nchunks - tile * a.own), lane);
+    const float vmask = valid ? 1.f : 0.f;
+    if (MOMENTS) {
+#pragma unroll
+      for (int i = 0; i < CH; ++i) x0[i] *= vmask;
+    } else {
+      srf_affine_mask<CH>(x0, lc[0].a, lc[0].c, valid);
+    }
+  }
+
+  if (PERSIST) {
+    const float4* src = chunk_src(last_task ? row : nrow, last_task ? tile : ntile);
+#pragma unroll
+    for (int i = 0; i < CH / 4; ++i) pre[i] = src[i];
+  }
+
+  float x1[CH / 2], x2[CH / 4], x3[CH / 8], x4[CH / 16], x5[CH / 32 > 0 ? CH / 32 : 1];
+  srf_zero(x1);
+  srf_zero(x2);
+  srf_zero(x3);
+  srf_zero(x4);
+  srf_zero(x5);
+  if (!PERSIST || tile == 0) {
+#pragma unroll
+    for (int k = 0; k < 6; ++k) s1[k] = s2[k] = 0.f;
+  }
+  double* mrow = a.mom + (size_t)row * D * 5;
+  if (MOMENTS && own) {
+    srf_acc_moments<CH>(x0, s1[0], s2[0]);
+    srf_pyr_edges<CH, Hand>(mrow, x0, ci, nchunks);
+  }
+  if (D > 1) {
+    srf_conv_s2<CH>(x0, x1, lc[1].w, lc[1].b);
+    if (SAVE && own) srf_pyr_store_level<CH / 2>(a.lv_out[1] + (size_t)row * (L >> 1) + (size_t)ci * (CH / 2), x1);
+    srf_affine_mask<CH / 2>(x1, lc[1].a, lc[1].c, valid);
+    if (MOMENTS && own) {
+      srf_acc_moments<CH / 2>(x1, s1[1], s2[1]);
+      srf_pyr_edges<CH / 2, Hand>(mrow + 5, x1, ci, nchunks);
+    }
+  }
+  if (D > 2) {
+    srf_conv_s2<CH / 2>(x1, x2, lc[2].w, lc[2].b);
+    if (SAVE && own) srf_pyr_store_level<CH / 4>(a.lv_out[2] + (size_t)row * (L >> 2) + (size_t)ci * (CH / 4), x2);
+    srf_affine_mask<CH / 4>(x2, lc[2].a, lc[2].c, valid);
+    if (MOMENTS && own) {
+      srf_acc_moments<CH / 4>(x2, s1[2], s2[2]);
+      srf_pyr_edges<CH / 4, Hand>(mrow + 10, x2, ci, nchunks);
+    }
+  }
+  if (D > 3) {
+    srf_conv_s2<CH / 4>(x2, x3, lc[3].w, lc[3].b);
+    if (SAVE && own) srf_pyr_store_level<CH / 8>(a.lv_out[3] + (size_t)row * (L >> 3) + (size_t)ci * (CH / 8), x3);
+    srf_affine_mask<CH / 8>(x3, lc[3].a, lc[3].c, valid);
+    if (MOMENTS && own) {
+      srf_acc_moments<CH / 8>(x3, s1[3], s2[3]);
+      srf_pyr_edges<CH / 8, Hand>(mrow + 15, x3, ci, nchunks);
+    }
+  }
+  if (D > 4) {
+    srf_conv_s2<CH / 8>(x3, x4, lc[4].w, lc[4].b);
+    if (SAVE && own) srf_pyr_store_level<CH / 16>(a.lv_out[4] + (size_t)row * (L >> 4) + (size_t)ci * (CH / 16), x4);
+    srf_affine_mask<CH / 16>(x4, lc[4].a, lc[4].c, valid);
+    if (MOMENTS && own) {
+      srf_acc_moments<CH / 16>(x4, s1[4], s2[4]);
+      srf_pyr_edges<CH / 16, Hand>(mrow + 20, x4, ci, nchunks);
+    }
+  }
+  if constexpr (CH >= 32) {
+    if (D > 5) {
+      srf_conv_s2<CH / 16>(x4, x5, lc[5].w, lc[5].b);
+      if (SAVE && own) srf_pyr_store_level<CH / 32>(a.lv_out[5] + (size_t)row * (L >> 5) + (size_t)ci * (CH / 32), x5);
+      srf_affine_mask<CH / 32>(x5, lc[5].a, lc[5].c, valid);
+      if (MOMENTS && own) {
+        srf_acc_moments<CH / 32>(x5, s1[5], s2[5]);
+        srf_pyr_edges<CH / 32, Hand>(mrow + 25, x5, ci, nchunks);
+      }
+    }
+  }
+
+  if (MOMENTS) {
+#pragma unroll
+    for (int k = 0; k < 6; ++k) {
+      if (PERSIST && tile != a.tiles - 1) break;
+      if (k < D) {
+        const float r1 = srf_dpp_wave_sum(s1[k]);
+        const float r2 = srf_dpp_wave_sum(s2[k]);
+        if (lane == 63) {
+          if (PERSIST) {
+            Hand::store_mom(mrow + k * 5 + 0, (double)r1);
+            Hand::store_mom(mrow + k * 5 + 1, (double)r2);
+          } else {
+            atomicAdd(&mrow[k * 5 + 0], (double)r1);
+            atomicAdd(&mrow[k * 5 + 1], (double)r2);
+          }
+        }
+      }
+    }
+  } else {
+    float ms = 0.f, mq = 0.f;
+    float outv[CH];
+#pragma unroll
+    for (int i = 0; i < CH; ++i) {
+      float t = 0.f;
+      bool have = false;
+      if (D > 5 && CH >= 32) {
+        t = x5[i >> 5];
+        have = true;
+      }
+      if (D > 4) {
+        const float v = x4[i >> 4];
+        t = have ? v + t : v;
+        have = true;
+      }
+      if (D > 3) {
+        const float v = x3[i >> 3];
+        t = have ? v + t : v;
+        have = true;
+      }
+      if (D > 2) {
+        const float v = x2[i >> 2];
+        t = have ? v + t : v;
+        have = true;
+      }
+      if (D > 1) {
+        const float v = x1[i >> 1];
+        t = have ? v + t : v;
+        have = true;
+      }
+      const float v = have ? x0[i] + t : x0[i];
+      outv[i] = v;
+      ms += v;
+      mq = fmaf(v, v, mq);
+    }
+    if (!own) {
+      ms = 0.f;
+      mq = 0.f;
+    }
+    srf_pyr_store_chunks<CH>(pyr_strip + wave * (60 * (CH / 4 + 1)), outv, own, a.merged + (size_t)row * L, tile * a.own,
+                             min(a.own, nchunks - tile * a.own), lane);
+    if (a.out_sums) {
+      const double ds = srf_dpp_wave_sum((double)ms), dq = srf_dpp_wave_sum((double)mq);
+      if (lane == 63) {
+        double* dst = srf_stat_slot(a.out_sums, g, c * a.tiles + tile);
+        atomicAdd(dst, ds);
+        atomicAdd(dst + 1, dq);
+      }
+    }
+  }
+  if (last_task) break;
+  if (ntile == 0 && ++c == C) {
+    c = 0;
+    ++g;
+  }
+  row = nrow;
+  tile = ntile;
+  }
+}
diff --git a/sudo_rm_rf_amd/ops.py b/sudo_rm_rf_amd/ops.py
--- a/sudo_rm_rf_amd/ops.py
+++ b/sudo_rm_rf_amd/ops.py
@@ -209,7 +209,7 @@
     return y
 
 
-def pyramid(y1, in_sums, in_gamma, in_beta, in_prelu, weights, biases, gammas, betas, out_sums=None):
+def pyramid(y1, in_sums, in_gamma, in_beta, in_prelu, weights, biases, gammas, betas, out_sums=None, scratch=None):
     dev = _chk(y1, in_sums, in_gamma, in_beta, in_prelu, *weights, *biases, *gammas, *betas, out_sums)
     groups, Cc, L = y1.shape
     D = len(weights)
@@ -217,7 +217,11 @@
     if not lib.srf_pyramid_supported(Cc, L, D):
         raise _lib.SrfError("srf_pyramid: unsupported shape C=%d L=%d D=%d" % (Cc, L, D))
     merged = torch.empty_like(y1)
-    scratch = torch.empty(lib.srf_pyramid_scratch_bytes(groups, Cc, L, D), dtype=torch.uint8, device=dev)
+    need = lib.srf_pyramid_scratch_bytes(groups, Cc, L, D)
+    if scratch is None:
+        scratch = torch.empty(need, dtype=torch.uint8, device=dev)
+    elif scratch.dtype != torch.uint8 or scratch.numel() < need or scratch.device != dev:
+        raise RuntimeError("pyramid: scratch must be a uint8 tensor of >= %d bytes on %s" % (need, dev))
     arr = lambda ts: (C.c_void_p * D)(*[t.data_ptr() for t in ts])
     n = _lib.make_norm(in_sums, in_gamma, in_beta, in_prelu)
     rc = lib.srf_pyramid(_lib.ptr(y1), _lib.ptr(merged), C.byref(n), arr(weights), arr(biases), arr(gammas),
@@ -555,6 +559,9 @@
         set_debug_flags(prev)
 
 
+from ._diag import DebugFlag2, debug_flags2, set_debug_flags2
+
+
 def set_kernel_mode(mode):
     _lib.load().srf_set_kernel_mode(int(mode))
 
```

Measured after the change: 22420. About the same (-0.0%).
